# speechcatcher-asr/statecatcher

Measured on AMD Instinct MI355X. Metric: audio-frames/sec (LucyRNN+CTC, 80-d fbank, T=1500), whole job, higher is better.
Workload: dtype bf16

## Files before the change

include/statecatcher.h:

```cpp
#ifndef STATECATCHER_H
#define STATECATCHER_H

#include <stddef.h>
#include <stdint.h>

#ifdef __cplusplus
extern "C" {
#endif

#define SC_EINVAL (-1)

#define SC_F32 0
#define SC_BF16 1
#define SC_F16 2

int sc_abi_version(void);

const char* sc_last_error(void);


int sc_lucy_scan_chunk(void);

int64_t sc_lucy_scan_ckpt_numel(int B, int T, int D);

int sc_lucy_scan_fwd(const void* gates, int gates_dtype, const float* gate_bias,
                     const float* h0, const float* s0,
                     void* out, float* s_out, float* h_out, int B, int T, int D,
                     int64_t stride_g_bt, int64_t stride_g_td, int64_t stride_g_cd,
                     int64_t stride_g_cb, int64_t stride_o_bt, int64_t stride_o_bd, float* ckpt,
                     void* stream);

int sc_lucy_scan_fwd_split(const void* gates, int gates_dtype, const float* gate_bias,
                           const float* h0, const float* s0, void* out, void* out_dup, void* out_lo,
                           float* s_out, float* h_out, int B, int T, int D,
                           int64_t stride_g_bt, int64_t stride_g_td, int64_t stride_g_cd,
                           int64_t stride_g_cb, int64_t stride_o_bt, int64_t stride_o_bd,
                           float* ckpt, void* stream);

int sc_lucy_scan_fwd_ln(const void* gates, int gates_dtype, const float* gate_bias,
                        const float* h0, const float* s0, void* out, void* out_dup, void* out_lo,
                        float* s_out, float* h_out, int B, int T, int D,
                        int64_t stride_g_bt, int64_t stride_g_td, int64_t stride_g_cd,
                        int64_t stride_g_cb, int64_t stride_o_bt, int64_t stride_o_bd,
                        float* ckpt, const float* ln_r, const float* ln_rec_in, float* ln_stat,
                        float* ln_rec_out, float ln_eps, void* stream);

int sc_lucy_scan_bwd(const void* gates, int gates_dtype, const float* gate_bias, const float* ckpt,
                     const void* dout, const float* ds_last,
                     void* dgates, float* dh0, float* ds0, float* dbias, int B, int T, int D,
                     int64_t stride_g_bt, int64_t stride_g_td, int64_t stride_g_cd,
                     int64_t stride_g_cb, int64_t stride_d_bt, int64_t stride_d_bd,
                     int64_t stride_dg_bt, int64_t stride_dg_td, int64_t stride_dg_cd,
                     int64_t stride_dg_cb, void* stream);

int sc_lucy_scan_bwd_ln(const void* gates, int gates_dtype, const float* gate_bias,
                        const float* ckpt, const void* dout, const float* ds_last, void* dgates,
                        float* dh0, float* ds0, float* dbias, int B, int T, int D,
                        int64_t stride_g_bt, int64_t stride_g_td, int64_t stride_g_cd,
                        int64_t stride_g_cb, int64_t stride_d_bt, int64_t stride_d_bd,
                        int64_t stride_dg_bt, int64_t stride_dg_td, int64_t stride_dg_cd,
                        int64_t stride_dg_cb, const float* ln_r, const float* ln_stat,
                        void* stream);


int sc_decay_scan_fwd(const void* kv, const void* decay, void* out, int dtype,
                      const float* init, int B, int T, int D,
                      int64_t stride_b, int64_t stride_t, int64_t stride_d, void* stream);

int sc_decay_scan_bwd(const void* decay, const void* s_all, const void* dout, void* dkv,
                      void* ddecay, int dtype, const float* init, float* dinit,
                      int B, int T, int D, int64_t stride_b, int64_t stride_t, int64_t stride_d,
                      void* stream);


int sc_layernorm_supported(int dtype, int D);
int sc_layernorm_fwd(const void* x, int dtype, const float* gamma, const float* beta, void* y,
                     float* mean, float* rstd, int64_t rows, int D, float eps, void* stream);

int64_t sc_layernorm_bwd_workspace_numel(int64_t rows, int D);

int sc_layernorm_bwd(const void* x, const void* dy, int dtype, const float* gamma,
                     const float* mean, const float* rstd, void* dx, float* dgamma_dbeta,
                     float* workspace, int64_t rows, int D, void* stream);

typedef struct {
  const float* w;
  const float* gamma;
  const float* beta;
  const float* bias;
  float* shift;
  float* bias_out;
  float* rowsum;
  int64_t ld, rows, D;
} sc_ln_fold_job;
int sc_ln_fold_prep(const sc_ln_fold_job* jobs, int njobs, void* stream);

int sc_ln_fold_bwd(const void* g, const void* h, int dtype, const float* stat, void* dh,
                   int64_t rows, int D, void* stream);

int64_t sc_ln_fold_wgrad_workspace_numel(int rows, int D);

int sc_ln_fold_wgrad(const float* M, const float* w, int64_t ld, const float* gamma,
                     const float* beta, const float* dbias, int rows, int D, float* dw,
                     float* dgamma_dbeta, float* workspace, void* stream);


size_t sc_ctc_workspace_bytes(int B, int T, int max_target_len);

int sc_ctc_fwd(const void* x, int x_dtype, int is_logits, int B, int T, int V,
               int64_t stride_b, int64_t stride_t,
               const int64_t* targets, int64_t target_stride, int max_target_len,
               const int64_t* in_lens, const int64_t* tgt_lens, int blank,
               float* nll, void* workspace, size_t workspace_bytes, void* stream);

int sc_ctc_bwd(const void* x, int x_dtype, int is_logits, int B, int T, int V,
               int64_t stride_b, int64_t stride_t,
               const int64_t* targets, int64_t target_stride, int max_target_len,
               const int64_t* in_lens, const int64_t* tgt_lens, int blank,
               const float* nll, const float* scale, void* grad, int grad_dtype,
               const void* workspace, size_t workspace_bytes, void* stream);

int sc_ctc_fwd_ex(const void* x, int x_dtype, int is_logits, int B, int T, int V,
                  int64_t stride_b, int64_t stride_t,
                  const int64_t* targets, int64_t target_stride, int max_target_len,
                  const int64_t* in_lens, const int64_t* tgt_lens, int blank,
                  const float* ex, int64_t ex_stride_b, int64_t ex_stride_t,
                  float* nll, void* workspace, size_t workspace_bytes, void* stream);
int sc_ctc_bwd_ex(const void* x, int x_dtype, int is_logits, int B, int T, int V,
                  int64_t stride_b, int64_t stride_t,
                  const int64_t* targets, int64_t target_stride, int max_target_len,
                  const int64_t* in_lens, const int64_t* tgt_lens, int blank,
                  const float* ex, int64_t ex_stride_b, int64_t ex_stride_t,
                  const float* nll, const float* scale, void* grad, int grad_dtype,
                  const void* workspace, size_t workspace_bytes, void* stream);

int sc_ctc_split_rows(const float* w, int64_t ldw, const float* bias, int V, int K,
                      const int64_t* targets, int64_t target_stride, int max_target_len,
                      int blank, void* out, float* bias_out, int B, void* stream);

int sc_ctc_mean(const float* nll, const int64_t* tgt_lens, int B, float* loss, float* factor,
                void* stream);


int sc_ctc_greedy_decode(const void* log_probs, int dtype, int B, int T, int V,
                         int64_t stride_b, int64_t stride_t, const int64_t* lengths, int blank,
                         int32_t* tokens, int32_t* counts, void* stream);

int sc_ctc_greedy_step(const void* logits, int dtype, int B, int V, int64_t stride_b,
                       const float* mask, int blank, int32_t* prev, int32_t* emit,
                       int64_t emit_stride, void* stream);
int sc_ctc_greedy_frames(const void* logits, int dtype, int F, int B, int V, int64_t stride_f,
                         int64_t stride_b, const float* mask, int64_t mask_f, int blank,
                         int32_t* prev, int32_t* emit, int64_t emit_f, int64_t emit_b,
                         void* stream);


int sc_lucy_step_supported(int dtype, int D);

int sc_lucy_step_ln(const void* x, int dtype, const float* w, const float* b, float eps, void* y,
                    int B, int D, void* stream);

int sc_lucy_step_cell(int mode, const void* g, int dtype, int64_t g_stride, const void* u,
                      const void* hp, const float* lnz_w, const float* lnz_b, const float* lnh_w,
                      const float* lnh_b, float eps, float* h, float* s, void* out,
                      const float* mask, int B, int D, void* stream);

int sc_lucy_frame_gemm(int epi, const float* x, int64_t ldx, int K, const float* ln_w,
                       const float* ln_b, const void* st_in, int nst_in, float eps, const void* w,
                       int w_dtype, int64_t ldw, const float* bias, int B, int N, float* y,
                       int64_t ldy, void* st_out, float* z, void* st_z, float* s,
                       const float* mask, void* stream);
int sc_lucy_frame_cellb(const float* z, const void* st_z, int nst_z, const float* hp,
                        const void* st_h, int nst_h, const float* lnz_w, const float* lnz_b,
                        const float* lnh_w, const float* lnh_b, float eps, float* h, float* out,
                        int64_t ldo, const float* mask, int B, int D, void* stream);

typedef struct sc_frame_gemm_job {
  const float* x;
  int64_t ldx;
  int K;
  const float* ln_w;
  const float* ln_b;
  const void* st_in;
  int nst_in;
  const void* w;
  int64_t ldw;
  const float* bias;
  int B, N;
  float* y;
  int64_t ldy;
  void* st_out;
  float* z;
  void* st_z;
  float* s;
  const float* mask;
} sc_frame_gemm_job;
int sc_lucy_frame_gemm_multi(int epi, int w_dtype, float eps, const sc_frame_gemm_job* jobs,
                             int njobs, void* stream);
typedef struct sc_frame_cell_job {
  const float* z;
  const void* st_z;
  int nst_z;
  const float* hp;
  const void* st_h;
  int nst_h;
  const float *lnz_w, *lnz_b, *lnh_w, *lnh_b;
  float* h;
  float* out;
  int64_t ldo;
  const float* mask;
  int B, D;
} sc_frame_cell_job;
int sc_lucy_frame_cellb_multi(float eps, const sc_frame_cell_job* jobs, int njobs, void* stream);


size_t sc_colsum_workspace_bytes(int64_t M, int64_t N);
int sc_colsum(const void* x, int dtype, int64_t M, int64_t N, int64_t ld, int64_t perm_a,
              int64_t perm_b, float* out, void* workspace, size_t workspace_bytes, void* stream);


int sc_gemm_wgrad_splits(int L, int I, int J);
int sc_gemm_wgrad_bf16(const void* A, int64_t lda, const void* B, int64_t ldb, float* part, int L,
                       int I, int J, int S, void* stream);

int sc_gemm_tn_bf16(const void* A, int64_t lda, const void* B, int64_t ldb, void* C, int64_t ldc,
                    int M, int N, int K, int tile_m, void* stream);

int sc_gemm_tn_ln_bf16(const void* H, int64_t ldh, const void* Wpp, int64_t ldw, void* C,
                       int64_t ldc, int M, int N, int K, const float* r, void* stat, float eps,
                       void* stream);


typedef struct {
  float* p;
  const float* g;
  float* m;
  float* v;
  int64_t n;
} sc_adam_tensor;
int64_t sc_adam_parts(const sc_adam_tensor* t, int nt);
int sc_adam_sumsq(const sc_adam_tensor* t, int nt, float* part, void* stream);
int sc_adam_step(const sc_adam_tensor* t, int nt, const float* part, int64_t nparts,
                 double max_norm, double lr, double beta1, double beta2, double eps,
                 double weight_decay, int decoupled, double step_size, double bc2_sqrt,
                 float* norm_out, void* stream);

typedef struct {
  const float* src;
  void* dst;
  void* dst_t;
  int64_t rows, cols, cols_pad, ld_src, block_d;
  const float* col_scale;
  const float* row_shift;
} sc_image_job;
int sc_weight_images(const sc_image_job* jobs, int njobs, void* stream);


int sc_xlstm_part_rows(int64_t rows);
int sc_rmsnorm_fwd(const void* x, const float* w, void* y, float* rstd, int64_t rows, int D,
                   float eps, void* stream);
int sc_rmsnorm_bwd(const void* x, const void* dy, const float* w, const float* rstd, void* dx,
                   float* part, int64_t rows, int D, void* stream);
int sc_rmsnorm_add_fwd(const void* x, const void* r, void* s, const float* w, void* y, float* rstd,
                       int64_t rows, int D, float eps, void* stream);
int sc_rmsnorm_add_bwd(const void* s, const void* dy, const void* dres, const float* w,
                       const float* rstd, void* dx, float* part, int64_t rows, int D, void* stream);
int sc_mhln_gate_fwd(const void* h, const void* o, int64_t ldo, const float* w, void* out,
                     float* mean, float* rstd, int B, int T, int NH, int DH, float eps,
                     void* stream);
int sc_mhln_gate_bwd(const void* h, const void* o, int64_t ldo, const float* w, const float* mean,
                     const float* rstd, const void* dy, int64_t ldy, void* dh, void* dgo,
                     int64_t lddo, float* part, int B, int T, int NH, int DH, void* stream);
int sc_mhln_gate_fwd_h16(const void* h, const void* o, int64_t ldo, const float* w, void* out,
                         float* mean, float* rstd, int B, int T, int NH, int DH, float eps,
                         void* stream);
int sc_mhln_gate_bwd_h16(const void* h, const void* o, int64_t ldo, const float* w,
                         const float* mean, const float* rstd, const void* dy, int64_t ldy,
                         void* dh, void* dgo, int64_t lddo, float* part, int B, int T, int NH,
                         int DH, void* stream);
int sc_swiglu_fwd(const void* a, void* y, int64_t rows, int F, void* stream);
int sc_swiglu_bwd(const void* a, const void* dy, void* da, int64_t rows, int F, void* stream);


int64_t sc_fbank_frames(int64_t n_samples);
size_t sc_fbank_workspace_bytes(void);

int sc_fbank(const float* audio, int B, int64_t n_samples, int64_t audio_stride, int kind,
             float sample_rate, float* out, void* workspace, size_t workspace_bytes, void* stream);


int sc_mlstm_supported(int dtype, int DQ, int DV);

int64_t sc_mlstm_chunk_state_numel(int BH, int T, int DQ, int DV);

int sc_mlstm_fwd(const void* q, const void* k, const void* v, int dtype, const float* igate,
                 const float* fgate, const float* c0, const float* n0, const float* m0, int BH,
                 int T, int DQ, int DV, float eps, void* h, void* states_C, float* states_n,
                 float* states_m, float* c_last, float* m_rows, float* den_rows,
                 const int64_t* layout, void* stream);

int sc_mlstm_bwd(const void* q, const void* k, const void* v, int dtype, const float* igate,
                 const float* fgate, const void* h, const void* dh, const float* dcT,
                 const float* dnT, const void* states_C, const float* states_n,
                 const float* states_m, const float* m_rows, const float* den_rows, int BH, int T,
                 int DQ, int DV, float eps, float* dstates_C, float* dstates_n, void* dq,
                 void* dk, void* dv, float* qdq, float* kdk, const int64_t* layout,
                 void* stream);

int sc_mlstm_fwd_io(const void* q, const void* k, const void* v, int dtype, int io_dtype,
                    const float* igate, const float* fgate, const float* c0, const float* n0,
                    const float* m0, int BH, int T, int DQ, int DV, float eps, void* h,
                    void* states_C, float* states_n, float* states_m, float* c_last,
                    float* m_rows, float* den_rows, const int64_t* layout, void* stream);
int sc_mlstm_bwd_io(const void* q, const void* k, const void* v, int dtype, int io_dtype,
                    const float* igate, const float* fgate, const void* h, const void* dh,
                    const float* dcT, const float* dnT, const void* states_C,
                    const float* states_n, const float* states_m, const float* m_rows,
                    const float* den_rows, int BH, int T, int DQ, int DV, float eps,
                    float* dstates_C, float* dstates_n, void* dq, void* dk, void* dv,
                    float* qdq, float* kdk, const int64_t* layout, void* stream);

int sc_mlstm_gate_bwd(const float* qdq, const float* kdk, const float* fgate, int BH, int T,
                      float* dfgate, const void* a, void* da, int NH, int64_t ld, int io, int fo,
                      float cap, void* stream);


size_t sc_rnnt_workspace_bytes(int B, int T, int max_labels);

int sc_rnnt_fwd(const void* x, int x_dtype, int is_logits, int B, int T, int max_labels, int V,
                int64_t stride_b, int64_t stride_t, int64_t stride_u, const int64_t* row_offsets,
                const int64_t* labels, int64_t label_stride, const int64_t* frames_lengths,
                const int64_t* labels_lengths, int blank, float* nll, void* workspace,
                size_t workspace_bytes, void* stream);

int sc_rnnt_bwd(const void* x, int x_dtype, int is_logits, int B, int T, int max_labels, int V,
                int64_t stride_b, int64_t stride_t, int64_t stride_u, const int64_t* row_offsets,
                const int64_t* labels, int64_t label_stride, const int64_t* frames_lengths,
                const int64_t* labels_lengths, int blank, const float* scale, void* grad,
                int grad_dtype, const void* workspace, size_t workspace_bytes, void* stream);

int sc_rnnt_joint_geometry(int B, int T, int max_labels, int V, int* t_blocks, int* u_splits,
                           int* slices);
int sc_rnnt_joint_fwd(const float* enc, const float* pred, const void* W, const float* bias, int B,
                      int T, int max_labels, int V, int J, const int64_t* labels,
                      int64_t label_stride, const int64_t* frames_lengths,
                      const int64_t* labels_lengths, int blank, float* nll, void* workspace,
                      size_t workspace_bytes, void* stream);
int sc_rnnt_joint_bwd(const float* enc, const float* pred, const void* W, const float* bias, int B,
                      int T, int max_labels, int V, int J, const int64_t* labels,
                      int64_t label_stride, const int64_t* frames_lengths,
                      const int64_t* labels_lengths, int blank, const float* scale, float* d_enc,
                      float* d_pred, float* dW, float* db, const void* workspace,
                      size_t workspace_bytes, void* stream);

int sc_rnnt_greedy_decode(const void* enc_p, const void* pred_tab, const void* W, int dtype,
                          const float* bias, int B, int T, int V, int J, int64_t stride_b,
                          int64_t stride_t, const int64_t* lengths, const float* mask,
                          int64_t mask_b, int64_t mask_t, int blank, int max_symbols,
                          int32_t* prev, int32_t* tokens, int32_t* frames, int cap,
                          int32_t* counts, void* stream);

#ifdef __cplusplus
}
#endif
#endif
```

statecatcher_amd/_lib.py:

```python
import ctypes
import os

import torch

LIB_NAME = "libstatecatcher_hip.so"
LIB_PATH = os.environ.get("SC_LIB_PATH") or os.path.join(os.path.dirname(os.path.abspath(__file__)),
                                                         LIB_NAME)

SC_F32, SC_BF16, SC_F16 = 0, 1, 2
_DTYPE = {torch.float32: SC_F32, torch.bfloat16: SC_BF16, torch.float16: SC_F16}

_c = ctypes
_i32, _i64, _vp, _fp = _c.c_int, _c.c_int64, _c.c_void_p, _c.c_void_p
ABI_VERSION = 14

_SIGS = {
    "sc_abi_version": (_i32, []),
    "sc_gemm_wgrad_splits": (_i32, [_i32, _i32, _i32]),
    "sc_gemm_wgrad_bf16": (_i32, [_vp, _i64, _vp, _i64, _fp, _i32, _i32, _i32, _i32, _vp]),
    "sc_gemm_tn_bf16": (_i32, [_vp, _i64, _vp, _i64, _vp, _i64, _i32, _i32, _i32, _i32, _vp]),
    "sc_gemm_tn_ln_bf16": (_i32, [_vp, _i64, _vp, _i64, _vp, _i64, _i32, _i32, _i32, _fp, _vp,
                                 _c.c_float, _vp]),
    "sc_last_error": (_c.c_char_p, []),
    "sc_lucy_scan_chunk": (_i32, []),
    "sc_lucy_scan_ckpt_numel": (_i64, [_i32, _i32, _i32]),
    "sc_lucy_scan_fwd": (_i32, [_vp, _i32, _fp, _fp, _fp, _vp, _fp, _fp, _i32, _i32, _i32,
                               _i64, _i64, _i64, _i64, _i64, _i64, _fp, _vp]),
    "sc_lucy_scan_fwd_split": (_i32, [_vp, _i32, _fp, _fp, _fp, _vp, _vp, _vp, _fp, _fp, _i32, _i32,
                                     _i32, _i64, _i64, _i64, _i64, _i64, _i64, _fp, _vp]),
    "sc_lucy_scan_bwd": (_i32, [_vp, _i32, _fp, _fp, _vp, _fp, _vp, _fp, _fp, _fp, _i32, _i32, _i32,
                               _i64, _i64, _i64, _i64, _i64, _i64, _i64, _i64, _i64, _i64,
                               _vp]),
    "sc_lucy_scan_fwd_ln": (_i32, [_vp, _i32, _fp, _fp, _fp, _vp, _vp, _vp, _fp, _fp, _i32, _i32,
                                  _i32, _i64, _i64, _i64, _i64, _i64, _i64, _fp, _fp, _fp, _fp, _fp,
                                  _c.c_float, _vp]),
    "sc_lucy_scan_bwd_ln": (_i32, [_vp, _i32, _fp, _fp, _vp, _fp, _vp, _fp, _fp, _fp, _i32, _i32,
                                  _i32, _i64, _i64, _i64, _i64, _i64, _i64, _i64, _i64, _i64, _i64,
                                  _fp, _fp, _vp]),
    "sc_ln_fold_prep": (_i32, [_vp, _i32, _vp]),
    "sc_ln_fold_bwd": (_i32, [_vp, _vp, _i32, _fp, _vp, _i64, _i32, _vp]),
    "sc_ln_fold_wgrad_workspace_numel": (_i64, [_i32, _i32]),
    "sc_ln_fold_wgrad": (_i32, [_fp, _fp, _i64, _fp, _fp, _fp, _i32, _i32, _fp, _fp, _fp, _vp]),
    "sc_decay_scan_fwd": (_i32, [_vp, _vp, _vp, _i32, _fp, _i32, _i32, _i32, _i64, _i64, _i64, _vp]),
    "sc_decay_scan_bwd": (_i32, [_vp, _vp, _vp, _vp, _vp, _i32, _fp, _fp, _i32, _i32, _i32,
                                _i64, _i64, _i64, _vp]),
    "sc_layernorm_supported": (_i32, [_i32, _i32]),
    "sc_layernorm_fwd": (_i32, [_vp, _i32, _fp, _fp, _vp, _fp, _fp, _i64, _i32, _c.c_float, _vp]),
    "sc_layernorm_bwd_workspace_numel": (_i64, [_i64, _i32]),
    "sc_layernorm_bwd": (_i32, [_vp, _vp, _i32, _fp, _fp, _fp, _vp, _fp, _fp, _i64, _i32, _vp]),
    "sc_ctc_workspace_bytes": (_c.c_size_t, [_i32, _i32, _i32]),
    "sc_ctc_fwd": (_i32, [_vp, _i32, _i32, _i32, _i32, _i32, _i64, _i64, _vp, _i64, _i32, _vp, _vp,
                         _i32, _fp, _vp, _c.c_size_t, _vp]),
    "sc_ctc_bwd": (_i32, [_vp, _i32, _i32, _i32, _i32, _i32, _i64, _i64, _vp, _i64, _i32, _vp, _vp,
                         _i32, _fp, _fp, _vp, _i32, _vp, _c.c_size_t, _vp]),
    "sc_ctc_fwd_ex": (_i32, [_vp, _i32, _i32, _i32, _i32, _i32, _i64, _i64, _vp, _i64, _i32, _vp,
                            _vp, _i32, _fp, _i64, _i64, _fp, _vp, _c.c_size_t, _vp]),
    "sc_ctc_bwd_ex": (_i32, [_vp, _i32, _i32, _i32, _i32, _i32, _i64, _i64, _vp, _i64, _i32, _vp,
                            _vp, _i32, _fp, _i64, _i64, _fp, _fp, _vp, _i32, _vp, _c.c_size_t,
                            _vp]),
    "sc_ctc_split_rows": (_i32, [_fp, _i64, _fp, _i32, _i32, _vp, _i64, _i32, _i32, _vp, _fp,
                                 _i32, _vp]),
    "sc_ctc_greedy_decode": (_i32, [_vp, _i32, _i32, _i32, _i32, _i64, _i64, _vp, _i32, _vp, _vp, _vp]),
    "sc_colsum_workspace_bytes": (_c.c_size_t, [_i64, _i64]),
    "sc_colsum": (_i32, [_vp, _i32, _i64, _i64, _i64, _i64, _i64, _fp, _vp, _c.c_size_t, _vp]),
    "sc_fbank_frames": (_i64, [_i64]),
    "sc_fbank_workspace_bytes": (_c.c_size_t, []),
    "sc_fbank": (_i32, [_vp, _i32, _i64, _i64, _i32, _c.c_float, _fp, _vp, _c.c_size_t, _vp]),
    "sc_ctc_mean": (_i32, [_fp, _vp, _i32, _fp, _fp, _vp]),
    "sc_ctc_greedy_step": (_i32, [_vp, _i32, _i32, _i32, _i64, _fp, _i32, _vp, _vp, _i64, _vp]),
    "sc_lucy_step_supported": (_i32, [_i32, _i32]),
    "sc_lucy_step_ln": (_i32, [_vp, _i32, _fp, _fp, _c.c_float, _vp, _i32, _i32, _vp]),
    "sc_lucy_step_cell": (_i32, [_i32, _vp, _i32, _i64, _vp, _vp, _fp, _fp, _fp, _fp, _c.c_float,
                                 _fp, _fp, _vp, _fp, _i32, _i32, _vp]),
    "sc_lucy_frame_gemm": (_i32, [_i32, _fp, _i64, _i32, _fp, _fp, _vp, _i32, _c.c_float, _vp, _i32,
                                  _i64, _fp, _i32, _i32, _fp, _i64, _vp, _fp, _vp, _fp, _fp, _vp]),
    "sc_lucy_frame_cellb": (_i32, [_fp, _vp, _i32, _fp, _vp, _i32, _fp, _fp, _fp, _fp, _c.c_float,
                                   _fp, _fp, _i64, _fp, _i32, _i32, _vp]),
    "sc_lucy_frame_gemm_multi": (_i32, [_i32, _i32, _c.c_float, _vp, _i32, _vp]),
    "sc_lucy_frame_cellb_multi": (_i32, [_c.c_float, _vp, _i32, _vp]),
    "sc_ctc_greedy_frames": (_i32, [_vp, _i32, _i32, _i32, _i32, _i64, _i64, _fp, _i64, _i32, _vp,
                                    _vp, _i64, _i64, _vp]),
    "sc_mlstm_supported": (_i32, [_i32, _i32, _i32]),
    "sc_mlstm_chunk_state_numel": (_i64, [_i32, _i32, _i32, _i32]),
    "sc_mlstm_fwd": (_i32, [_vp, _vp, _vp, _i32, _fp, _fp, _fp, _fp, _fp, _i32, _i32, _i32, _i32,
                           _c.c_float, _vp, _vp, _fp, _fp, _fp, _fp, _fp, _vp, _vp]),
    "sc_mlstm_bwd": (_i32, [_vp, _vp, _vp, _i32, _fp, _fp, _vp, _vp, _fp, _fp, _vp, _fp, _fp, _fp,
                           _fp, _i32, _i32, _i32, _i32, _c.c_float, _fp, _fp, _vp, _vp, _vp, _fp,
                           _fp, _vp, _vp]),
    "sc_mlstm_fwd_io": (_i32, [_vp, _vp, _vp, _i32, _i32, _fp, _fp, _fp, _fp, _fp, _i32, _i32, _i32,
                              _i32, _c.c_float, _vp, _vp, _fp, _fp, _fp, _fp, _fp, _vp, _vp]),
    "sc_mlstm_bwd_io": (_i32, [_vp, _vp, _vp, _i32, _i32, _fp, _fp, _vp, _vp, _fp, _fp, _vp, _fp, _fp,
                              _fp, _fp, _i32, _i32, _i32, _i32, _c.c_float, _fp, _fp, _vp, _vp, _vp,
                              _fp, _fp, _vp, _vp]),
    "sc_mlstm_gate_bwd": (_i32, [_fp, _fp, _fp, _i32, _i32, _fp, _vp, _vp, _i32, _i64, _i32, _i32,
                                _c.c_float, _vp]),
    "sc_xlstm_part_rows": (_i32, [_i64]),
    "sc_rmsnorm_fwd": (_i32, [_vp, _fp, _vp, _fp, _i64, _i32, _c.c_float, _vp]),
    "sc_rmsnorm_bwd": (_i32, [_vp, _vp, _fp, _fp, _vp, _fp, _i64, _i32, _vp]),
    "sc_rmsnorm_add_fwd": (_i32, [_vp, _vp, _vp, _fp, _vp, _fp, _i64, _i32, _c.c_float, _vp]),
    "sc_rmsnorm_add_bwd": (_i32, [_vp, _vp, _vp, _fp, _fp, _vp, _fp, _i64, _i32, _vp]),
    "sc_mhln_gate_fwd": (_i32, [_vp, _vp, _i64, _fp, _vp, _fp, _fp, _i32, _i32, _i32, _i32,
                                _c.c_float, _vp]),
    "sc_mhln_gate_bwd": (_i32, [_vp, _vp, _i64, _fp, _fp, _fp, _vp, _i64, _vp, _vp, _i64, _fp,
                                _i32, _i32, _i32, _i32, _vp]),
    "sc_mhln_gate_fwd_h16": (_i32, [_vp, _vp, _i64, _fp, _vp, _fp, _fp, _i32, _i32, _i32, _i32,
                                _c.c_float, _vp]),
    "sc_mhln_gate_bwd_h16": (_i32, [_vp, _vp, _i64, _fp, _fp, _fp, _vp, _i64, _vp, _vp, _i64, _fp,
                                _i32, _i32, _i32, _i32, _vp]),
    "sc_swiglu_fwd": (_i32, [_vp, _vp, _i64, _i32, _vp]),
    "sc_swiglu_bwd": (_i32, [_vp, _vp, _vp, _i64, _i32, _vp]),
    "sc_adam_parts": (_i64, [_vp, _i32]),
    "sc_adam_sumsq": (_i32, [_vp, _i32, _fp, _vp]),
    "sc_adam_step": (_i32, [_vp, _i32, _fp, _i64, _c.c_double, _c.c_double, _c.c_double,
                           _c.c_double, _c.c_double, _c.c_double, _i32, _c.c_double, _c.c_double,
                           _fp, _vp]),
    "sc_weight_images": (_i32, [_vp, _i32, _vp]),
    "sc_rnnt_workspace_bytes": (_c.c_size_t, [_i32, _i32, _i32]),
    "sc_rnnt_joint_geometry": (_i32, [_i32, _i32, _i32, _i32, _vp, _vp, _vp]),
    "sc_rnnt_joint_fwd": (_i32, [_fp, _fp, _vp, _fp, _i32, _i32, _i32, _i32, _i32, _vp, _i64, _vp,
                                 _vp, _i32, _fp, _vp, _c.c_size_t, _vp]),
    "sc_rnnt_joint_bwd": (_i32, [_fp, _fp, _vp, _fp, _i32, _i32, _i32, _i32, _i32, _vp, _i64, _vp,
                                 _vp, _i32, _fp, _fp, _fp, _fp, _fp, _vp, _c.c_size_t, _vp]),
    "sc_rnnt_fwd": (_i32, [_vp, _i32, _i32, _i32, _i32, _i32, _i32, _i64, _i64, _i64, _vp, _vp, _i64,
                          _vp, _vp, _i32, _fp, _vp, _c.c_size_t, _vp]),
    "sc_rnnt_bwd": (_i32, [_vp, _i32, _i32, _i32, _i32, _i32, _i32, _i64, _i64, _i64, _vp, _vp, _i64,
                          _vp, _vp, _i32, _fp, _vp, _i32, _vp, _c.c_size_t, _vp]),
    "sc_rnnt_greedy_decode": (_i32, [_vp, _vp, _vp, _i32, _fp, _i32, _i32, _i32, _i32, _i64, _i64,
                                     _vp, _fp, _i64, _i64, _i32, _i32, _vp, _vp, _vp, _i32, _vp,
                                     _vp]),
}
EXPORTED = tuple(_SIGS)


class AdamTensor(ctypes.Structure):
    _fields_ = [("p", _vp), ("g", _vp), ("m", _vp), ("v", _vp), ("n", _i64)]


class ImageJob(ctypes.Structure):
    _fields_ = [("src", _vp), ("dst", _vp), ("dst_t", _vp), ("rows", _i64), ("cols", _i64),
                ("cols_pad", _i64), ("ld_src", _i64), ("block_d", _i64), ("col_scale", _vp),
                ("row_shift", _vp)]


class LnFoldJob(ctypes.Structure):
    _fields_ = [("w", _vp), ("gamma", _vp), ("beta", _vp), ("bias", _vp), ("shift", _vp),
                ("bias_out", _vp), ("rowsum", _vp), ("ld", _i64), ("rows", _i64), ("D", _i64)]


class FrameGemmJob(ctypes.Structure):
    _fields_ = [("x", _vp), ("ldx", _i64), ("K", _i32), ("ln_w", _vp), ("ln_b", _vp),
                ("st_in", _vp), ("nst_in", _i32), ("w", _vp), ("ldw", _i64), ("bias", _vp),
                ("B", _i32), ("N", _i32), ("y", _vp), ("ldy", _i64), ("st_out", _vp), ("z", _vp),
                ("st_z", _vp), ("s", _vp), ("mask", _vp)]


class FrameCellJob(ctypes.Structure):
    _fields_ = [("z", _vp), ("st_z", _vp), ("nst_z", _i32), ("hp", _vp), ("st_h", _vp),
                ("nst_h", _i32), ("lnz_w", _vp), ("lnz_b", _vp), ("lnh_w", _vp), ("lnh_b", _vp),
                ("h", _vp), ("out", _vp), ("ldo", _i64), ("mask", _vp), ("B", _i32), ("D", _i32)]


_LIB = None


def load():
    global _LIB
    if _LIB is None:
        if not os.path.exists(LIB_PATH):
            raise RuntimeError(
                f"statecatcher HIP library not built: {LIB_PATH} missing "
                "(run `python -c 'import __graft_entry__ as g; g.build()'` or "
                "`make -C statecatcher_amd/csrc`)")
        lib = ctypes.CDLL(LIB_PATH)
        for name, (res, args) in _SIGS.items():
            fn = getattr(lib, name)
            fn.restype = res
            fn.argtypes = args
        if lib.sc_abi_version() != ABI_VERSION:
            raise RuntimeError("statecatcher ABI version mismatch")
        _LIB = lib
    return _LIB


def check(rc, what):
    if rc != 0:
        msg = load().sc_last_error().decode(errors="replace")
        if rc < 0:
            raise ValueError(f"{what}: {msg}")
        raise RuntimeError(f"{what}: HIP error {rc}: {msg}")


def dtype_code(t):
    try:
        return _DTYPE[t.dtype]
    except KeyError:
        raise TypeError(f"unsupported dtype {t.dtype}; expected float32, bfloat16 or float16") from None


def require_device(*tensors):
    for t in tensors:
        if t is not None and t.device.type != "cuda":
            raise RuntimeError(
                "statecatcher ops run only on a ROCm GPU (HIP); got a tensor on "
                f"{t.device}. There is no CPU fallback.")


def stream_of(t):
    return ctypes.c_void_p(torch.cuda.current_stream(t.device).cuda_stream)


def ptr(t):
    return ctypes.c_void_p(t.data_ptr()) if t is not None else None
```

statecatcher_amd/csrc/ctc.hip:

```cpp
#include "sc_common.h"

#ifndef SC_CTC_ABL
#define SC_CTC_ABL 0
#endif
#ifndef SC_CTC_KMAX
#define SC_CTC_KMAX 16
#endif
#ifndef SC_CTC_FLAGX
#define SC_CTC_FLAGX 0
#endif
#ifndef SC_CTC_WMV
#define SC_CTC_WMV 0
#endif
#ifndef SC_CTC_FLAG_SLEEP
#define SC_CTC_FLAG_SLEEP 1
#endif

namespace sc {

constexpr float kNegInf = -__builtin_huge_valf();

struct CtcWs {
  float* lse;
  double* lse64;
  float* lpe;
  float* alpha;
  float* beta;
  double* offA;
  double* offB;
  float* cst;
  double* ll2s;
  int* chain;
  int* first;
  float* ylin;
  int* flag;
  int* sharp;
};

static size_t align256(size_t x) { return (x + 255) & ~(size_t)255; }

static int states_per_lane(int S) { return (S + 63) / 64; }

static int lin_ppl(int Umax);

static size_t ws_layout(int B, int T, int Umax, CtcWs* w, void* base) {
  const int S = 2 * Umax + 1;
  const int Sp = 64 * states_per_lane(S);
  const bool lin = lin_ppl(Umax) > 0;
  const size_t ab = 4;
  const int Um = Umax > 0 ? Umax : 1;
  char* p = (char*)base;
  size_t off = 0;
  auto take = [&](size_t bytes) {
    char* r = p + off;
    off += align256(bytes);
    return (void*)r;
  };
  CtcWs t;
  t.lse = (float*)take((size_t)B * T * 4);
  t.lse64 = (double*)take((size_t)B * T * 8);
  t.lpe = (float*)take((size_t)B * T * Sp * 4);
  t.alpha = (float*)take((size_t)B * T * Sp * ab);
  t.beta = (float*)take((size_t)B * T * Sp * ab);
  t.offA = (double*)take((size_t)B * (T + 1) * 8);
  t.offB = (double*)take((size_t)B * (T + 1) * 8);
  t.cst = (float*)take((size_t)B * T * 4);
  t.ll2s = (double*)take((size_t)B * 8);
  t.chain = (int*)take((size_t)B * Um * 4);
  t.first = (int*)take((size_t)B * Um * 4);
  t.ylin = lin ? (float*)take((size_t)B * T * Sp * 4) : nullptr;
  t.flag = lin ? (int*)take((size_t)B * 4) : nullptr;
  t.sharp = (int*)take((size_t)B * 4);
  if (w) *w = t;
  return off;
}

__device__ __forceinline__ float lse2_b2(float a, float b) {
  const float m = fmaxf(a, b);
  if (m == kNegInf) return kNegInf;
  return m + log2_(exp2_(a - m) + exp2_(b - m));
}


struct CtcArgs {
  const void* x;
  int is_logits, B, T, V, S, Sp, Umax, blank;
  int kh;
  int lin;
  int64_t sb, stt;
  const int64_t* tg;
  int64_t tgs;
  const int64_t* in_lens;
  const int64_t* tgt_lens;
  float* nll;
  CtcWs ws;
  const float* scale;
  void* grad;
  const float* ex;
  int64_t exb, ext;
};

__device__ __forceinline__ int clampi(int64_t v, int lo, int hi) {
  return (int)(v < lo ? lo : (v > hi ? hi : v));
}

__device__ __forceinline__ int state_label(const int64_t* tg, int s, int blank, int V) {
  int lab = (s & 1) ? (int)tg[(s - 1) >> 1] : blank;
  return lab < 0 ? 0 : (lab >= V ? V - 1 : lab);
}

constexpr float kTiny = 120.0f;

template <int DT>
__global__ void __launch_bounds__(256) ctc_emit_kernel(CtcArgs a) {
  using E = Elem<DT>;
  using T = typename E::T;
  const int lane = threadIdx.x & 63;
  const int64_t row = (int64_t)blockIdx.x * 4 + (threadIdx.x >> 6);
  if (row >= (int64_t)a.B * a.T) return;
  const int b = (int)(row / a.T), t = (int)(row % a.T);
  if (t >= clampi(a.in_lens[b], 0, a.T)) return;
  const T* p = (const T*)a.x + (int64_t)b * a.sb + (int64_t)t * a.stt;
  const int Sb = 2 * clampi(a.tgt_lens[b], 0, a.Umax) + 1;
  const int64_t* tg = a.tg + (int64_t)b * a.tgs;
  const float* exr = a.ex ? a.ex + (int64_t)b * a.exb + (int64_t)t * a.ext : nullptr;
  constexpr int kGx = 8;
  auto state_logit = [&](int s) {
    return exr ? exr[(s & 1) ? (s + 1) >> 1 : 0] : E::ld(p[state_label(tg, s, a.blank, a.V)]);
  };
  const bool inreg = a.Sp <= 64 * kGx;
  float xs[kGx];
  if (inreg) {
    if (exr) {
#pragma unroll
      for (int j = 0; j < kGx; ++j) {
        const int s = min(lane + 64 * j, Sb - 1);
        xs[j] = exr[(s & 1) ? (s + 1) >> 1 : 0];
      }
    } else {
      int lab[kGx];
#pragma unroll
      for (int j = 0; j < kGx; ++j) lab[j] = state_label(tg, min(lane + 64 * j, Sb - 1), a.blank, a.V);
#pragma unroll
      for (int j = 0; j < kGx; ++j) xs[j] = E::ld(p[lab[j]]);
    }
  }
  float lse = 0.0f;
  if (a.is_logits) {
    float m = kNegInf, l = 0.0f;
    constexpr int N = Vec16<DT>::N;
    if ((a.V % N) == 0 && ((uintptr_t)p & 15) == 0) {
      for (int c = lane; c < a.V / N; c += 64) {
        float xv[N];
        Vec16<DT>::ld(p + N * c, xv);
        float cm = xv[0];
#pragma unroll
        for (int k = 1; k < N; ++k) cm = fmaxf(cm, xv[k]);
        const float mn = fmaxf(m, cm);
        float cs = 0.0f;
#pragma unroll
        for (int k = 0; k < N; ++k) cs += fexp(xv[k] - mn);
        l = l * fexp(m - mn) + cs;
        m = mn;
      }
    } else {
      for (int v = lane; v < a.V; v += 64) {
        const float xv = E::ld(p[v]);
        const float mn = fmaxf(m, xv);
        l = l * fexp(m - mn) + fexp(xv - mn);
        m = mn;
      }
    }
    const float M = wave_max_dpp(m);
    l = wave_sum_dpp(m == kNegInf ? 0.0f : l * fexp(m - M));
    lse = M + flog(l);
    if (lane == 0) {
      a.ws.lse[row] = lse;
      a.ws.lse64[row] = (double)M + (double)flog(l);
    }
  }
  float* out = a.ws.lpe + row * a.Sp;
  auto lp2x = [&](float xl) { return fmaxf((xl - lse) * kLog2e, -1e30f); };
  auto lp2 = [&](int s) { return lp2x(state_logit(s)); };
  float c = -1e30f;
  if (inreg) {
#pragma unroll
    for (int j = 0; j < kGx; ++j)
      if (lane + 64 * j < Sb) c = fmaxf(c, lp2x(xs[j]));
  } else {
    for (int s = lane; s < Sb; s += 64) c = fmaxf(c, lp2(s));
  }
  c = wave_max_dpp(c);
  if (!(c > -1e29f)) c = 0.0f;
  bool tiny = false;
  auto put = [&](int s, float e) {
    out[s] = e;
    if (a.lin) {
      tiny |= e > -1e29f && e < -kTiny;
      a.ws.ylin[row * a.Sp + s] = e > -1e29f ? exp2_(e) : 0.0f;
    }
  };
  if (inreg) {
#pragma unroll
    for (int j = 0; j < kGx; ++j) {
      const int s = lane + 64 * j;
      if (s < a.Sp) put(s, s < Sb ? fmaxf(lp2x(xs[j]) - c, -1e30f) : -1e30f);
    }
  } else {
    for (int s = lane; s < a.Sp; s += 64) put(s, s < Sb ? fmaxf(lp2(s) - c, -1e30f) : -1e30f);
  }
  if (lane == 0) a.ws.cst[row] = c;
  if (a.lin && __ballot(tiny) && lane == 0) a.ws.flag[b] = 1;
}

__global__ void __launch_bounds__(256) ctc_chain_kernel(CtcArgs a) {
  __shared__ int lt[1024];
  const int b = blockIdx.x;
  const int lane = threadIdx.x & 63;
  const int Ub = clampi(a.tgt_lens[b], 0, a.Umax);
  const int64_t* tg = a.tg + (int64_t)b * a.tgs;
  const int Um = a.Umax > 0 ? a.Umax : 1;
  for (int u = threadIdx.x; u < Ub; u += blockDim.x) lt[u] = (int)tg[u];
  __syncthreads();
  if (blockIdx.y == 0 && threadIdx.x == 0) a.ws.sharp[b] = 0;
  const int u = blockIdx.y * 4 + (threadIdx.x >> 6);
  if (u >= Um) return;
  int nxt = -1, first = 0;
  if (u < Ub) {
    const int lab = lt[u];
    for (int q0 = u + 1; q0 < Ub; q0 += 64) {
      const int q = q0 + lane;
      const unsigned long long hit = __ballot(q < Ub && lt[q] == lab);
      if (hit) {
        nxt = q0 + __ffsll(hit) - 1;
        break;
      }
    }
    first = 1;
    for (int q0 = 0; q0 < u; q0 += 64) {
      const int q = q0 + lane;
      if (__ballot(q < u && lt[q] == lab)) {
        first = 0;
        break;
      }
    }
  }
  if (lane == 0) {
    a.ws.chain[(int64_t)b * Um + u] = nxt;
    a.ws.first[(int64_t)b * Um + u] = first;
  }
}

__device__ __forceinline__ float shr1(float v) {
  return __int_as_float(__builtin_amdgcn_update_dpp(__float_as_int(-1e30f), __float_as_int(v),
                                                     0x138, 0xf, 0xf, false));
}
__device__ __forceinline__ float shl1(float v) {
  return __int_as_float(__builtin_amdgcn_update_dpp(__float_as_int(-1e30f), __float_as_int(v),
                                                     0x130, 0xf, 0xf, false));
}

constexpr float kDead = -1e30f;
constexpr float kDrift = 512.0f;
__device__ __forceinline__ float lse3_live(float a, float b, float c) {
  const float m = fmaxf(fmaxf(a, b), c);
  if (SC_CTC_ABL & 4) return m;
  const float md = __builtin_amdgcn_fmed3f(a, b, c);
  const float lo = fminf(fminf(a, b), c);
  return m + log2_(1.0f + exp2_(md - m) + exp2_(lo - m));
}

constexpr int kAbP = 16;

#ifndef SC_CTC_V2
#define SC_CTC_V2 1
#endif
__device__ __forceinline__ float vmin(float a, float b) {
  float r;
  asm("v_min_f32 %0, %1, %2" : "=v"(r) : "v"(a), "v"(b));
  return r;
}
__device__ __forceinline__ float vmax3(float a, float b, float c) {
  float r;
  asm("v_max3_f32 %0, %1, %2, %3" : "=v"(r) : "v"(a), "v"(b), "v"(c));
  return r;
}
__device__ __forceinline__ float vmin3(float a, float b, float c) {
  float r;
  asm("v_min3_f32 %0, %1, %2, %3" : "=v"(r) : "v"(a), "v"(b), "v"(c));
  return r;
}
__device__ __forceinline__ float shr1z(float v) {
  return __int_as_float(__builtin_amdgcn_mov_dpp(__float_as_int(v), 0x138, 0xf, 0xf, true));
}
__device__ __forceinline__ float shl1z(float v) {
  return __int_as_float(__builtin_amdgcn_mov_dpp(__float_as_int(v), 0x130, 0xf, 0xf, true));
}
typedef float f2v __attribute__((ext_vector_type(2)));
__device__ __forceinline__ f2v lse23(float a2, float b2, float a3, float b3, float c3, f2v e) {
  const float m2 = vmax(a2, b2), l2 = vmin(a2, b2);
  const float m3 = vmax3(a3, b3, c3), d3 = __builtin_amdgcn_fmed3f(a3, b3, c3);
  const float l3 = vmin3(a3, b3, c3);
  const f2v me = f2v{m2, m3} + e;
  const f2v s = f2v{1.0f, 1.0f} + f2v{exp2_(l2 - m2), exp2_(d3 - m3)};
  return me + f2v{log2_(s.x), log2_(s.y + exp2_(l3 - m3))};
}


__device__ __forceinline__ float lse2_live(float a, float b) {
  const float m = fmaxf(a, b);
  if (SC_CTC_ABL & 4) return m;
  return m + log2_(1.0f + exp2_(fminf(a, b) - m));
}

template <int K, bool BETA>
__device__ __forceinline__ void ab_run(const CtcArgs& a, int b, int Tb, int Ub) {
  constexpr int OW = 64 - K;
  constexpr int kAbP = K > 16 ? K : 16;
  const int tid = threadIdx.x;
  const int lane = tid & 63;
  const int w = uniform(tid >> 6);
  const int nw = blockDim.x >> 6;
  const int p = BETA ? w * OW + lane : w * OW + lane - K;
  const bool own = BETA ? (lane < OW) : (lane >= K);
  const bool liveB = p >= 0 && p <= Ub;
  const bool liveL = p >= 0 && p < Ub;
  const int64_t* tg = a.tg + (int64_t)b * a.tgs;
  bool skip = false;
  if (liveL) {
    const int lab = (int)tg[p];
    if (!BETA) {
      skip = p >= 1 && lab != a.blank && lab != (int)tg[p - 1];
    } else if (p + 1 < Ub) {
      const int l2 = (int)tg[p + 1];
      skip = l2 != a.blank && l2 != lab;
    }
  }
  extern __shared__ __attribute__((aligned(16))) float2 full2[];
  __shared__ __attribute__((aligned(16))) float wmax[16];
  __shared__ int xflag[16];
  if (SC_CTC_FLAGX) {
    if (tid < 16) xflag[tid] = 0;
    lds_barrier();
  }
  const int nst = nw * OW;
  const int pc = p < 0 ? 0 : (2 * p >= a.Sp ? a.Sp / 2 - 1 : p);
  const float2* lrow = (const float2*)(a.ws.lpe + (int64_t)b * a.T * a.Sp) + pc;
  const int64_t rs = a.Sp / 2;
  constexpr uint32_t kDrop = 0x80000000u;
  const uint32_t rowb = (uint32_t)(a.Sp * 4);
  const __amdgpu_buffer_rsrc_t ors = __builtin_amdgcn_make_buffer_rsrc(
      (BETA ? a.ws.beta : a.ws.alpha) + (int64_t)b * a.T * a.Sp, 0, (int)(rowb * (uint32_t)a.T),
      0x00020000);
  const uint32_t ovo = (own && 2 * p < a.Sp) ? (uint32_t)(8 * pc) : kDrop;
  double* offn = (BETA ? a.ws.offB : a.ws.offA) + (int64_t)b * (a.T + 1);
  if (tid == 0) offn[0] = 0.0;
  auto tstep = [&](int i) { return BETA ? Tb - 1 - i : i; };
  float2 bufA[kAbP], bufB[kAbP];
#if SC_CTC_V2
  const __amdgpu_buffer_rsrc_t ers = __builtin_amdgcn_make_buffer_rsrc(
      a.ws.lpe + (int64_t)b * a.T * a.Sp, 0, (int)(rowb * (uint32_t)a.T), 0x00020000);
  const uint32_t evo = (p >= 0 && 2 * p < a.Sp) ? (uint32_t)(8 * p) : kDrop;
  auto load = [&](float2 (&buf)[kAbP], int i0) {
#pragma unroll
    for (int j = 0; j < kAbP; ++j)
      buf[j] = __builtin_bit_cast(float2, __builtin_amdgcn_raw_buffer_load_b64(
                                              ers, evo, (uint32_t)tstep(min(i0 + j, Tb - 1)) * rowb, 0));
  };
#else
  auto load = [&](float2 (&buf)[kAbP], int i0) {
#pragma unroll
    for (int j = 0; j < kAbP; ++j) buf[j] = lrow[(int64_t)tstep(min(i0 + j, Tb - 1)) * rs];
  };
#endif
  auto emit = [&](int t, float vB, float vL) {
    __builtin_amdgcn_raw_buffer_store_b64(
        __builtin_bit_cast(__attribute__((ext_vector_type(2))) unsigned, make_float2(vB, vL)), ors,
        ovo, (uint32_t)t * rowb, 0);
  };
  float vB = kDead, vL = kDead;
  double off = 0.0;
  int exch = 0;
  auto body = [&](const float2 (&buf)[kAbP], int i0) __attribute__((always_inline)) {
#pragma unroll
    for (int j = 0; j < kAbP; ++j) {
      const int i = i0 + j;
      if (i >= Tb) break;
#if SC_CTC_V2
      if (i == 0) {
        vB = (liveB && p == (BETA ? Ub : 0)) ? buf[j].x : kDead;
        vL = (liveL && p == (BETA ? Ub - 1 : 0)) ? buf[j].y : kDead;
      } else if (!BETA) {
        const float lp = shr1z(vL);
        const f2v r = lse23(vB, lp, vL, vB, skip ? lp : kDead, f2v{buf[j].x, buf[j].y});
        vB = r.x;
        vL = r.y;
      } else {
        const float bn = shl1z(vB);
        const float ln = shl1z(vL);
        const f2v r = lse23(vB, vL, vL, bn, skip ? ln : kDead, f2v{buf[j].x, buf[j].y});
        vB = r.x;
        vL = r.y;
      }
#else
      const float eB = liveB ? buf[j].x : kDead;
      const float eL = liveL ? buf[j].y : kDead;
      if (i == 0) {
        vB = (liveB && p == (BETA ? Ub : 0)) ? eB : kDead;
        vL = (liveL && p == (BETA ? Ub - 1 : 0)) ? eL : kDead;
      } else if (!BETA) {
        const float lp = shr1(vL);
        const float nB = lse2_live(vB, lp) + eB;
        vL = lse3_live(vL, vB, skip ? lp : kDead) + eL;
        vB = nB;
      } else {
        const float bn = shl1(vB);
        const float ln = shl1(vL);
        const float nB = lse2_live(vB, vL) + eB;
        vL = lse3_live(vL, bn, skip ? ln : kDead) + eL;
        vB = nB;
      }
#endif
      if (!(SC_CTC_ABL & 1) && j % K == K - 1) {
        const int par = exch & 1;
        const bool norm = par == 1;
        if (own) full2[par * nst + p] = make_float2(vB, vL);
        if (SC_CTC_FLAGX && !norm) {
          lds_read_wait();
          if (lane == 0)
            __hip_atomic_store(&xflag[w], exch + 1, __ATOMIC_RELEASE, __HIP_MEMORY_SCOPE_WORKGROUP);
          const int nb = BETA ? w + 1 : w - 1;
          if (nb >= 0 && nb < nw) {
            while (__hip_atomic_load(&xflag[nb], __ATOMIC_ACQUIRE, __HIP_MEMORY_SCOPE_WORKGROUP) <= exch)
              if (SC_CTC_FLAG_SLEEP) __builtin_amdgcn_s_sleep(1);
          }
          if (!own) {
            const bool has = p >= 0 && p < nst;
            const float2 q = has ? full2[par * nst + p] : make_float2(kDead, kDead);
            vB = q.x;
            vL = q.y;
          }
          ++exch;
          if (!(SC_CTC_ABL & 2)) emit(tstep(i), vB, vL);
          continue;
        }
        if (norm) {
          float m = own ? fmaxf(vB, vL) : kDead;
#if SC_CTC_V2
          m = wave_max_dpp(m);
#else
#pragma unroll
          for (int o = 32; o > 0; o >>= 1) m = fmaxf(m, __shfl_xor(m, o));
#endif
          if (lane == 0) wmax[w] = m;
        }
        lds_barrier();
        if (!own) {
          const bool has = p >= 0 && p < nst;
          const float2 q = has ? full2[par * nst + p] : make_float2(kDead, kDead);
          vB = q.x;
          vL = q.y;
        }
        if (norm) {
          float m = kDead;
#if SC_CTC_WMV
#pragma unroll
          for (int q4 = 0; q4 < 16; q4 += 4) {
            if (q4 < nw) {
              const float4 wm = *(const float4*)&wmax[q4];
              m = fmaxf(m, q4 + 0 < nw ? wm.x : kDead);
              m = fmaxf(m, q4 + 1 < nw ? wm.y : kDead);
              m = fmaxf(m, q4 + 2 < nw ? wm.z : kDead);
              m = fmaxf(m, q4 + 3 < nw ? wm.w : kDead);
            }
          }
#else
          for (int q = 0; q < nw; ++q) m = fmaxf(m, wmax[q]);
#endif
          if (m > 0.5f * kDead) {
            vB -= m;
            vL -= m;
            off += (double)m;
// ... 94 lines not shown
  const int64_t* tg = a.tg + (int64_t)b * a.tgs;
  const int npairs = a.Sp / 2;
  double skip[PPL];
  uint32_t vo[PPL];
  constexpr uint32_t kDrop = 0x80000000u;
#pragma unroll
  for (int j = 0; j < PPL; ++j) {
    const int p = lane * PPL + j;
    bool sk = false;
    if (p < Ub) {
      const int lab = (int)tg[p];
      if (!BETA) {
        sk = p >= 1 && lab != a.blank && lab != (int)tg[p - 1];
      } else if (p + 1 < Ub) {
        const int l2 = (int)tg[p + 1];
        sk = l2 != a.blank && l2 != lab;
      }
    }
    skip[j] = sk ? 1.0 : 0.0;
    vo[j] = p < npairs ? (uint32_t)(8 * p) : kDrop;
  }
  const uint32_t rowb = (uint32_t)(a.Sp * 4);
  const __amdgpu_buffer_rsrc_t ers = __builtin_amdgcn_make_buffer_rsrc(
      a.ws.ylin + (int64_t)b * a.T * a.Sp, 0, (int)(rowb * (uint32_t)a.T), 0x00020000);
  double* offn = (BETA ? a.ws.offB : a.ws.offA) + (int64_t)b * (a.T + 1);
  if (lane == 0) offn[0] = 0.0;
  auto tstep = [&](int i) { return BETA ? Tb - 1 - i : i; };
  f2v bufA[kLinC][PPL], bufB[kLinC][PPL];
  auto load = [&](f2v (&buf)[kLinC][PPL], int i0) {
#pragma unroll
    for (int s = 0; s < kLinC; ++s) {
      const uint32_t so = (uint32_t)tstep(min(i0 + s, Tb - 1)) * rowb;
#pragma unroll
      for (int j = 0; j < PPL; ++j)
        buf[s][j] = (SC_CTC_ABL & 16) ? f2v{0.5f, 0.25f}
                                      : __builtin_bit_cast(f2v, __builtin_amdgcn_raw_buffer_load_b64(ers, vo[j], so, 0));
    }
  };
  double vB[PPL], vL[PPL];
#pragma unroll
  for (int j = 0; j < PPL; ++j) vB[j] = vL[j] = 0.0;
  double off = 0.0;
  bool fail = false;
  auto body = [&](const f2v (&buf)[kLinC][PPL], int ci) __attribute__((always_inline)) {
    d2v* slot = slots + (size_t)(ci & 1) * kLinC * PPL * 64;
#pragma unroll
    for (int s = 0; s < kLinC; ++s) {
      const int i = ci * kLinC + s;
      if (i >= Tb) break;
      if (i == 0) {
#pragma unroll
        for (int j = 0; j < PPL; ++j) {
          const int p = lane * PPL + j;
          vB[j] = (p <= Ub && p == (BETA ? Ub : 0)) ? (double)buf[s][j].x : 0.0;
          vL[j] = (p < Ub && p == (BETA ? Ub - 1 : 0)) ? (double)buf[s][j].y : 0.0;
        }
      } else if (!BETA) {
        double prevL[PPL];
        prevL[0] = dpp_shr1d(vL[PPL - 1]);
#pragma unroll
        for (int j = 1; j < PPL; ++j) prevL[j] = vL[j - 1];
#pragma unroll
        for (int j = 0; j < PPL; ++j) {
          const double nb = (vB[j] + prevL[j]) * (double)buf[s][j].x;
          const double nl = __builtin_fma(skip[j], prevL[j], vL[j] + vB[j]) * (double)buf[s][j].y;
          vB[j] = nb;
          vL[j] = nl;
        }
      } else {
        double nB[PPL], nL[PPL];
        nB[PPL - 1] = dpp_shl1d(vB[0]);
        nL[PPL - 1] = dpp_shl1d(vL[0]);
#pragma unroll
        for (int j = 0; j + 1 < PPL; ++j) {
          nB[j] = vB[j + 1];
          nL[j] = vL[j + 1];
        }
#pragma unroll
        for (int j = 0; j < PPL; ++j) {
          const double nb = (vB[j] + vL[j]) * (double)buf[s][j].x;
          const double nl = __builtin_fma(skip[j], nL[j], vL[j] + nB[j]) * (double)buf[s][j].y;
          vB[j] = nb;
          vL[j] = nl;
        }
      }
      if (!(SC_CTC_ABL & 8) && (i + 1) % kAb1R == 0) {
        double m = 0.0;
#pragma unroll
        for (int j = 0; j < PPL; ++j) m = fmax(m, fmax(vB[j], vL[j]));
        int e = 0;
        (void)frexp(m, &e);
        const float E = wave_max_dpp(m > 0.0 ? (float)e : -1e9f);
        if (E < -1e8f) {
          fail = true;
          return;
        }
        const int ie = (int)E;
#pragma unroll
        for (int j = 0; j < PPL; ++j) {
          vB[j] = ldexp(vB[j], -ie);
          vL[j] = ldexp(vL[j], -ie);
        }
        off += (double)ie;
        if (lane == 0) offn[(i + 1) / kAb1R] = off;
      }
#pragma unroll
      for (int j = 0; j < PPL; ++j) slot[(s * PPL + j) * 64 + lane] = d2v{vB[j], vL[j]};
    }
  };
  const int nch = (Tb + kLinC - 1) / kLinC;
  load(bufA, 0);
  for (int ci = 0; ci < nch; ++ci) {
    if (!fail) {
      if ((ci & 1) == 0) {
        if (ci + 1 < nch) load(bufB, (ci + 1) * kLinC);
        body(bufA, ci);
      } else {
        if (ci + 1 < nch) load(bufA, (ci + 1) * kLinC);
        body(bufB, ci);
      }
    }
    if (lane == 0) *fail_lds = fail ? 1 : 0;
    __syncthreads();
  }
  if (fail) return false;
  if (!BETA) {
    double c = 0.0;
#pragma unroll
    for (int j = 0; j < PPL; ++j) {
      const int p = lane * PPL + j;
      if (p == Ub) c += vB[j];
      if (p == Ub - 1) c += vL[j];
    }
    double cs = 0.0;
    for (int t = lane; t < Tb; t += 64) cs += (double)a.ws.cst[(int64_t)b * a.T + t];
#pragma unroll
    for (int o = 32; o > 0; o >>= 1) {
      c += __shfl_xor(c, o);
      cs += __shfl_xor(cs, o);
    }
    if (!(c > 0.0)) return false;
    if (lane == 0) {
      const double ll2s = log2(c) + off;
      a.ws.ll2s[b] = ll2s;
      a.nll[b] = (float)(-(ll2s + cs) * 0.6931471805599453);
    }
  }
  return true;
}

template <int PPL, bool BETA>
__device__ __forceinline__ void lin_consume(const CtcArgs& a, int b, int Tb, const d2v* slots,
                                            const int* fail_lds) {
  const int lane = threadIdx.x & 63, half = (threadIdx.x >> 6) - 1;
  const int npairs = a.Sp / 2;
  constexpr uint32_t kDrop = 0x80000000u;
  uint32_t vo[PPL];
#pragma unroll
  for (int j = 0; j < PPL; ++j) {
    const int p = lane * PPL + j;
    vo[j] = p < npairs ? (uint32_t)(8 * p) : kDrop;
  }
  const uint32_t rowb = (uint32_t)(a.Sp * 4);
  const __amdgpu_buffer_rsrc_t ors = __builtin_amdgcn_make_buffer_rsrc(
      (BETA ? a.ws.beta : a.ws.alpha) + (int64_t)b * a.T * a.Sp, 0, (int)(rowb * (uint32_t)a.T),
      0x00020000);
  const int nch = (Tb + kLinC - 1) / kLinC;
  bool stop = false;
  auto consume = [&](int ci) {
    const d2v* slot = slots + (size_t)(ci & 1) * kLinC * PPL * 64;
#pragma unroll
    for (int s2 = 0; s2 < kLinC / 2; ++s2) {
      const int s = half * (kLinC / 2) + s2, i = ci * kLinC + s;
      if (i >= Tb) break;
      const uint32_t so = (uint32_t)(BETA ? Tb - 1 - i : i) * rowb;
#pragma unroll
      for (int j = 0; j < PPL; ++j) {
        const d2v v = slot[(s * PPL + j) * 64 + lane];
        if (!(SC_CTC_ABL & 2))
          __builtin_amdgcn_raw_buffer_store_b64(
              __builtin_bit_cast(__attribute__((ext_vector_type(2))) unsigned, f2v{log2d(v.x), log2d(v.y)}),
              ors, vo[j], so, 0);
      }
    }
  };
  for (int ci = 0; ci < nch; ++ci) {
    __syncthreads();
    if (!stop) stop = *fail_lds != 0;
    if (!stop) consume(ci);
  }
}

template <int PPL>
__global__ void __launch_bounds__(192) ctc_lin_kernel(CtcArgs a) {
  __shared__ d2v slots[2 * kLinC * PPL * 64];
  __shared__ int fail_lds;
  const bool is_beta = blockIdx.x >= a.B;
  const int b = is_beta ? blockIdx.x - a.B : blockIdx.x;
  const int Tb = clampi(a.in_lens[b], 0, a.T);
  const int Ub = clampi(a.tgt_lens[b], 0, a.Umax);
  const int w = uniform(threadIdx.x >> 6);
  if (Tb == 0) {
    if (!is_beta && threadIdx.x == 0) {
      a.nll[b] = (Ub == 0) ? 0.0f : __builtin_huge_valf();
      a.ws.ll2s[b] = (Ub == 0) ? 0.0 : -__builtin_huge_val();
    }
    return;
  }
  const bool tiny = a.ws.flag[b] != 0;
  bool lin = !tiny;
  if (lin) {
    if (w == 0) {
      lin = is_beta ? lin_produce<PPL, true>(a, b, Tb, Ub, slots, &fail_lds)
                    : lin_produce<PPL, false>(a, b, Tb, Ub, slots, &fail_lds);
    } else {
      if (is_beta) lin_consume<PPL, true>(a, b, Tb, slots, &fail_lds);
      else lin_consume<PPL, false>(a, b, Tb, slots, &fail_lds);
      __builtin_amdgcn_s_waitcnt(0);
    }
    __syncthreads();
  }
  if (!lin && threadIdx.x == 0) a.ws.sharp[b] = 1;
}


constexpr int kXDeadE = -(1 << 29);
constexpr int kX64P = 16;
constexpr double kLog2eD = 1.4426950408889634;

struct Xv {
  double m;
  int e;
};
__device__ __forceinline__ Xv xnorm(double m, int e) {
  int x;
  const double mm = frexp(m, &x);
  return m > 0.0 ? Xv{mm, e + x} : Xv{0.0, kXDeadE};
}
__device__ __forceinline__ Xv xadd2(Xv a, Xv b) {
  const int E = max(a.e, b.e);
  return Xv{ldexp(a.m, a.e - E) + ldexp(b.m, b.e - E), E};
}
__device__ __forceinline__ Xv xadd3(Xv a, Xv b, Xv c) {
  const int E = max(max(a.e, b.e), c.e);
  return Xv{ldexp(a.m, a.e - E) + ldexp(b.m, b.e - E) + ldexp(c.m, c.e - E), E};
}
template <bool RIGHT>
__device__ __forceinline__ Xv xdpp(Xv v) {
  constexpr int ctl = RIGHT ? 0x138 : 0x130;
  const int lo = __builtin_amdgcn_update_dpp(0, __double2loint(v.m), ctl, 0xf, 0xf, false);
  const int hi = __builtin_amdgcn_update_dpp(0, __double2hiint(v.m), ctl, 0xf, 0xf, false);
  const int e = __builtin_amdgcn_update_dpp(kXDeadE, v.e, ctl, 0xf, 0xf, false);
  return Xv{__hiloint2double(hi, lo), e};
}
__device__ __forceinline__ Xv xemit(float x, double q, bool live) {
  const double e2 = (double)x * kLog2eD - q;
  if (!live || !(e2 > -1e300)) return Xv{0.0, kXDeadE};
  const double k = floor(e2);
  return xnorm((double)exp2_((float)(e2 - k)), (int)k);
}

template <int PPL, int DT, bool BETA>
__device__ __forceinline__ void x64_run(const CtcArgs& a, int b, int Tb, int Ub) {
  using E = Elem<DT>;
  const int lane = threadIdx.x;
  const int64_t* tg = a.tg + (int64_t)b * a.tgs;
  const int npairs = a.Sp / 2;
  bool skip[PPL], liveB[PPL], liveL[PPL];
  uint32_t cB[PPL], cL[PPL];
  uint32_t vo[PPL];
  constexpr uint32_t kDrop = 0x80000000u;
  const bool ex = a.ex != nullptr;
  const uint32_t esz = ex ? 4u : (uint32_t)sizeof(typename E::T);
#pragma unroll
  for (int j = 0; j < PPL; ++j) {
    const int p = lane * PPL + j;
    skip[j] = false;
    liveB[j] = p <= Ub;
    liveL[j] = p < Ub;
    int lab = a.blank;
    if (p < Ub) {
      lab = (int)tg[p];
      if (!BETA) {
        skip[j] = p >= 1 && lab != a.blank && lab != (int)tg[p - 1];
      } else if (p + 1 < Ub) {
        const int l2 = (int)tg[p + 1];
        skip[j] = l2 != a.blank && l2 != lab;
      }
    }
    lab = lab < 0 ? 0 : (lab >= a.V ? a.V - 1 : lab);
    cB[j] = ex ? 0u : (uint32_t)a.blank * esz;
    cL[j] = ex ? (uint32_t)(p < Ub ? 1 + p : 0) * 4u : (uint32_t)lab * esz;
    vo[j] = p < npairs ? (uint32_t)(8 * p) : kDrop;
  }
  const void* xb = ex ? (const void*)(a.ex + (int64_t)b * a.exb)
                      : (const void*)((const typename E::T*)a.x + (int64_t)b * a.sb);
  const uint32_t xrow = ex ? (uint32_t)a.ext * 4u : (uint32_t)a.stt * esz;
  const Buf<float> xf(xb);
  const Buf<typename E::T> xe(xb);
  auto ldx = [&](uint32_t col, uint32_t so) -> uint32_t {
    return ex ? __float_as_uint(xf.ld(col, so)) : xe.ldw(col, so);
  };
  auto cvt = [&](uint32_t w) { return ex ? __uint_as_float(w) : E::ldw(w); };
  const uint32_t rowb = (uint32_t)(a.Sp * 4);
  const __amdgpu_buffer_rsrc_t ors = __builtin_amdgcn_make_buffer_rsrc(
      (BETA ? a.ws.beta : a.ws.alpha) + (int64_t)b * a.T * a.Sp, 0, (int)(rowb * (uint32_t)a.T),
      0x00020000);
  double* offn = (BETA ? a.ws.offB : a.ws.offA) + (int64_t)b * (a.T + 1);
  const double* lse64 = a.ws.lse64 + (int64_t)b * a.T;
  const float* cst = a.ws.cst + (int64_t)b * a.T;
  if (lane == 0) offn[0] = 0.0;
  auto tstep = [&](int i) { return BETA ? Tb - 1 - i : i; };
  uint32_t wA[kX64P][PPL][2], wB[kX64P][PPL][2];
  double qA, qB;
  auto load = [&](uint32_t (&w)[kX64P][PPL][2], double& q, int i0) {
#pragma unroll
    for (int s = 0; s < kX64P; ++s) {
      const uint32_t so = (uint32_t)tstep(min(i0 + s, Tb - 1)) * xrow;
#pragma unroll
      for (int j = 0; j < PPL; ++j) {
        w[s][j][0] = ldx(cB[j], so);
        w[s][j][1] = ldx(cL[j], so);
      }
    }
    const int t = tstep(min(i0 + (lane & (kX64P - 1)), Tb - 1));
    q = (a.is_logits ? lse64[t] * kLog2eD : 0.0) + (double)cst[t];
  };
  Xv vB[PPL], vL[PPL];
#pragma unroll
  for (int j = 0; j < PPL; ++j) vB[j] = vL[j] = Xv{0.0, kXDeadE};
  const Xv dead{0.0, kXDeadE};
  auto body = [&](const uint32_t (&w)[kX64P][PPL][2], double qv, int i0) __attribute__((always_inline)) {
#pragma unroll
    for (int s = 0; s < kX64P; ++s) {
      const int i = i0 + s;
      if (i >= Tb) break;
      const double q = __hiloint2double(__builtin_amdgcn_readlane(__double2hiint(qv), s),
                                        __builtin_amdgcn_readlane(__double2loint(qv), s));
      Xv eB[PPL], eL[PPL];
#pragma unroll
      for (int j = 0; j < PPL; ++j) {
        eB[j] = xemit(cvt(w[s][j][0]), q, liveB[j]);
        eL[j] = xemit(cvt(w[s][j][1]), q, liveL[j]);
      }
      if (i == 0) {
#pragma unroll
        for (int j = 0; j < PPL; ++j) {
          const int p = lane * PPL + j;
          vB[j] = p == (BETA ? Ub : 0) ? eB[j] : dead;
          vL[j] = p == (BETA ? Ub - 1 : 0) ? eL[j] : dead;
        }
      } else if (!BETA) {
        Xv prevL[PPL];
        prevL[0] = xdpp<true>(vL[PPL - 1]);
#pragma unroll
        for (int j = 1; j < PPL; ++j) prevL[j] = vL[j - 1];
#pragma unroll
        for (int j = 0; j < PPL; ++j) {
          const Xv nb = xadd2(vB[j], prevL[j]);
          const Xv nl = xadd3(vL[j], vB[j], skip[j] ? prevL[j] : dead);
          vB[j] = xnorm(nb.m * eB[j].m, nb.e + eB[j].e);
          vL[j] = xnorm(nl.m * eL[j].m, nl.e + eL[j].e);
        }
      } else {
        Xv nB[PPL], nL[PPL];
        nB[PPL - 1] = xdpp<false>(vB[0]);
        nL[PPL - 1] = xdpp<false>(vL[0]);
#pragma unroll
        for (int j = 0; j + 1 < PPL; ++j) {
          nB[j] = vB[j + 1];
          nL[j] = vL[j + 1];
        }
#pragma unroll
        for (int j = 0; j < PPL; ++j) {
          const Xv nb = xadd2(vB[j], vL[j]);
          const Xv nl = xadd3(vL[j], nB[j], skip[j] ? nL[j] : dead);
          vB[j] = xnorm(nb.m * eB[j].m, nb.e + eB[j].e);
          vL[j] = xnorm(nl.m * eL[j].m, nl.e + eL[j].e);
        }
      }
      int mx = kXDeadE;
#pragma unroll
      for (int j = 0; j < PPL; ++j) mx = max(mx, max(vB[j].e, vL[j].e));
      const int O = (int)wave_max_dpp((float)mx);
      const bool alive = O > kXDeadE / 2;
      if (lane == 0) offn[i + 1] = alive ? (double)O : 0.0;
      const uint32_t so = (uint32_t)tstep(i) * rowb;
#pragma unroll
      for (int j = 0; j < PPL; ++j) {
        const float rb = vB[j].m > 0.0 ? (float)(vB[j].e - O) + log2_((float)vB[j].m) : kDead;
        const float rl = vL[j].m > 0.0 ? (float)(vL[j].e - O) + log2_((float)vL[j].m) : kDead;
        __builtin_amdgcn_raw_buffer_store_b64(
            __builtin_bit_cast(__attribute__((ext_vector_type(2))) unsigned, f2v{rb, rl}), ors,
            vo[j], so, 0);
      }
    }
  };
  load(wA, qA, 0);
  for (int i0 = 0; i0 < Tb; i0 += 2 * kX64P) {
    load(wB, qB, i0 + kX64P);
    body(wA, qA, i0);
    if (i0 + kX64P >= Tb) break;
    load(wA, qA, i0 + 2 * kX64P);
    body(wB, qB, i0 + kX64P);
  }
  if (!BETA) {
    Xv c = dead;
#pragma unroll
    for (int j = 0; j < PPL; ++j) {
      const int p = lane * PPL + j;
      if (p == Ub) c = xadd2(c, vB[j]);
      if (p == Ub - 1) c = xadd2(c, vL[j]);
    }
    double cs = 0.0;
    for (int t = lane; t < Tb; t += 64) cs += (double)cst[t];
#pragma unroll
    for (int o = 32; o > 0; o >>= 1) {
      const Xv co{__shfl_xor(c.m, o), __shfl_xor(c.e, o)};
      c = xadd2(c, co);
      cs += __shfl_xor(cs, o);
    }
    if (lane == 0) {
      const bool deadP = !(c.m > 0.0);
      const double ll2s = (double)c.e + log2(c.m);
      a.ws.ll2s[b] = deadP ? -__builtin_huge_val() : ll2s;
      a.nll[b] = deadP ? __builtin_huge_valf() : (float)(-(ll2s + cs) * 0.6931471805599453);
    }
  }
}

template <int PPL, int DT>
__global__ void __launch_bounds__(64) ctc_x64_kernel(CtcArgs a) {
  const bool is_beta = blockIdx.x >= a.B;
  const int b = is_beta ? blockIdx.x - a.B : blockIdx.x;
  if (a.ws.sharp[b] == 0) return;
  const int Tb = clampi(a.in_lens[b], 0, a.T);
  const int Ub = clampi(a.tgt_lens[b], 0, a.Umax);
  if (Tb == 0) return;
  if (threadIdx.x == 0) a.ws.sharp[b] = 2;
  if (is_beta) x64_run<PPL, DT, true>(a, b, Tb, Ub);
  else x64_run<PPL, DT, false>(a, b, Tb, Ub);
}

static int x64_ppl(int Umax) {
  const int ppl = (Umax + 1 + 63) / 64;
  return ppl <= 4 ? ppl : 0;
}

static int lin_ppl(int Umax) {
  static const bool on = [] {
    const char* e = getenv("SC_CTC_LIN");
    return e && e[0] == '1';
  }();
  const int ppl = (Umax + 1 + 63) / 64;
  return (on && ppl <= 4) ? ppl : 0;
}

static int ab_halo_k(int Umax) {
  auto waves = [&](int K) { return (Umax + 1 + (64 - K) - 1) / (64 - K); };
  for (int K : {SC_CTC_KMAX, 4, 2, 1})
    if (waves(K) <= 16) {
      if (SC_CTC_KMAX == 16 && K == 16 && waves(24) == waves(16)) return 24;
      return K;
    }
  return 0;
}

__device__ __forceinline__ void wave_lds_sync() {
  __builtin_amdgcn_fence(__ATOMIC_RELEASE, "wavefront");
  __builtin_amdgcn_wave_barrier();
  __builtin_amdgcn_fence(__ATOMIC_ACQUIRE, "wavefront");
}

template <int DT, int GT>
__global__ void __launch_bounds__(256) ctc_grad_kernel(CtcArgs a) {
  using E = Elem<DT>;
  using G = Elem<GT>;
  extern __shared__ __attribute__((aligned(16))) float lcab_all[];
  const int lane = threadIdx.x & 63, w = threadIdx.x >> 6;
  const int64_t row = (int64_t)blockIdx.x * (blockDim.x >> 6) + w;
  if (row >= (int64_t)a.B * a.T) return;
  float* lcab = lcab_all + w * (a.V + 4);
  const int b = (int)(row / a.T), t = (int)(row % a.T);
  const int Tb = clampi(a.in_lens[b], 0, a.T);
  typename G::T* g = (typename G::T*)a.grad + row * a.V;
  const float sc = a.scale[b];
  const bool gvec = (a.V & 7) == 0 && ((uintptr_t)g & 15) == 0;
  if (t >= Tb || sc == 0.0f) {
    if (gvec) {
      const float z[8] = {0.f, 0.f, 0.f, 0.f, 0.f, 0.f, 0.f, 0.f};
      for (int c = lane; c < (a.V >> 3); c += 64) {
        if constexpr (Vec16<GT>::N == 8) {
          Vec16<GT>::st(g + 8 * c, z);
        } else {
          Vec16<GT>::st(g + 8 * c, *(const float(*)[4])&z[0]);
          Vec16<GT>::st(g + 8 * c + 4, *(const float(*)[4])&z[4]);
        }
      }
    } else {
      for (int v = lane; v < a.V; v += 64) g[v] = G::st(0.0f);
    }
    return;
  }
  const int Ub = clampi(a.tgt_lens[b], 0, a.Umax);
  const int Sb = 2 * Ub + 1;
  const int Um = a.Umax > 0 ? a.Umax : 1;
  const int64_t* tg = a.tg + (int64_t)b * a.tgs;
  for (int v = lane; v < a.V; v += 64) lcab[v] = kNegInf;
  wave_lds_sync();
  const float* exr = a.ex ? a.ex + (int64_t)b * a.exb + (int64_t)t * a.ext : nullptr;
  const float* al = a.ws.alpha + ((int64_t)b * a.T + t) * a.Sp;
  const float* be = a.ws.beta + ((int64_t)b * a.T + t) * a.Sp;
  const int per = a.ws.sharp[b] == 2 ? 1 : 2 * a.kh;
  const float koff = (float)(a.ws.offA[(int64_t)b * (a.T + 1) + (t + 1) / per] +
                             a.ws.offB[(int64_t)b * (a.T + 1) + (Tb - t) / per] +
                             (double)a.ws.cst[(int64_t)b * a.T + t] - a.ws.ll2s[b]);
  const int* chain = a.ws.chain + (int64_t)b * Um;
  const int* first = a.ws.first + (int64_t)b * Um;
  const float lse = a.is_logits ? a.ws.lse[(int64_t)b * a.T + t] : 0.0f;
  const float lse_lo = a.is_logits ? (float)(a.ws.lse64[(int64_t)b * a.T + t] - (double)lse) : 0.0f;
  auto exact_grad = [&](float logit, float occ2) {
    const float lp2 = ((logit - lse) - lse_lo) * kLog2e;
    return (exp2_(lp2) - exp2_(occ2 + koff - lp2)) * sc;
  };
  float m = kNegInf, l = 0.0f;
  for (int s = lane; s < Sb; s += 64) {
    const int lab = (s & 1) ? (int)tg[(s - 1) >> 1] : a.blank;
    const float val = al[s] + be[s];
    if (lab == a.blank) {
      const float mn = fmaxf(m, val);
      if (mn != kNegInf) {
        l = l * exp2_(m - mn) + exp2_(val - mn);
        m = mn;
      }
    } else {
      const int u = (s - 1) >> 1;
      if (first[u]) {
        float acc = val;
        for (int q = chain[u]; q >= 0; q = chain[q])
          acc = lse2_b2(acc, al[2 * q + 1] + be[2 * q + 1]);
        if (lab >= 0 && lab < a.V) lcab[lab] = exr ? exact_grad(exr[1 + u], acc) : acc;
      }
    }
  }
  {
    const float M = wave_max_dpp(m);
    l = wave_sum_dpp(m == kNegInf ? 0.0f : l * exp2_(m - M));
    m = M;
  }
  if (lane == 0 && a.blank >= 0 && a.blank < a.V) {
    const float ob = (m == kNegInf) ? kNegInf : m + log2_(l);
    lcab[a.blank] = exr ? exact_grad(exr[0], ob) : ob;
  }
  wave_lds_sync();
  const typename E::T* xr = (const typename E::T*)a.x + (int64_t)b * a.sb + (int64_t)t * a.stt;
  if (gvec && ((uintptr_t)xr & 15) == 0) {
    for (int c = lane; c < (a.V >> 3); c += 64) {
      float xv[8], gv[8];
      if constexpr (Vec16<DT>::N == 8) {
        Vec16<DT>::ld(xr + 8 * c, xv);
      } else {
        Vec16<DT>::ld(xr + 8 * c, *(float(*)[4])&xv[0]);
        Vec16<DT>::ld(xr + 8 * c + 4, *(float(*)[4])&xv[4]);
      }
      const float4 l0 = *(const float4*)&lcab[8 * c], l1 = *(const float4*)&lcab[8 * c + 4];
      const float lc[8] = {l0.x, l0.y, l0.z, l0.w, l1.x, l1.y, l1.z, l1.w};
#pragma unroll
      for (int k = 0; k < 8; ++k) {
        const float lp2 = ((xv[k] - lse) - lse_lo) * kLog2e;
        gv[k] = (exp2_(lp2) - exp2_(lc[k] + koff - lp2)) * sc;
        if (a.ex && lc[k] != kNegInf) gv[k] = lc[k];
      }
      if constexpr (Vec16<GT>::N == 8) {
        Vec16<GT>::st(g + 8 * c, gv);
      } else {
        Vec16<GT>::st(g + 8 * c, *(float(*)[4])&gv[0]);
        Vec16<GT>::st(g + 8 * c + 4, *(float(*)[4])&gv[4]);
      }
    }
    return;
  }
  for (int v = lane; v < a.V; v += 64) {
    const float lp2 = ((E::ld(xr[v]) - lse) - lse_lo) * kLog2e;
    const float lc = lcab[v];
    const float gv = (a.ex && lc != kNegInf) ? lc : (exp2_(lp2) - exp2_(lc + koff - lp2)) * sc;
    g[v] = G::st(gv);
  }
}

static void launch_ab(const CtcArgs& a, hipStream_t st);

template <int DT>
static void launch_fwd(const CtcArgs& a, hipStream_t st) {
  const int64_t rows = (int64_t)a.B * a.T;
  if (a.lin) zero_async(a.ws.flag, (size_t)a.B * sizeof(int), st);
  hipLaunchKernelGGL((ctc_emit_kernel<DT>), dim3((unsigned)((rows + 3) / 4)), dim3(256), 0, st, a);
  hipLaunchKernelGGL(ctc_chain_kernel, dim3(a.B, ((a.Umax > 0 ? a.Umax : 1) + 3) / 4), dim3(256), 0,
                     st, a);
  switch (a.lin ? lin_ppl(a.Umax) : 0) {
    case 1: hipLaunchKernelGGL((ctc_lin_kernel<1>), dim3(2 * a.B), dim3(192), 0, st, a); break;
    case 2: hipLaunchKernelGGL((ctc_lin_kernel<2>), dim3(2 * a.B), dim3(192), 0, st, a); break;
    case 3: hipLaunchKernelGGL((ctc_lin_kernel<3>), dim3(2 * a.B), dim3(192), 0, st, a); break;
    case 4: hipLaunchKernelGGL((ctc_lin_kernel<4>), dim3(2 * a.B), dim3(192), 0, st, a); break;
    default: launch_ab(a, st); break;
  }
  switch (x64_ppl(a.Umax)) {
    case 1: hipLaunchKernelGGL((ctc_x64_kernel<1, DT>), dim3(2 * a.B), dim3(64), 0, st, a); break;
    case 2: hipLaunchKernelGGL((ctc_x64_kernel<2, DT>), dim3(2 * a.B), dim3(64), 0, st, a); break;
    case 3: hipLaunchKernelGGL((ctc_x64_kernel<3, DT>), dim3(2 * a.B), dim3(64), 0, st, a); break;
    case 4: hipLaunchKernelGGL((ctc_x64_kernel<4, DT>), dim3(2 * a.B), dim3(64), 0, st, a); break;
    default: break;
  }
}

static void launch_ab(const CtcArgs& a, hipStream_t st) {
  const int K = a.kh;
  const int nw = (a.Umax + 1 + (64 - K) - 1) / (64 - K);
  const size_t sh = 2 * (size_t)nw * (64 - K) * sizeof(float2);
  switch (K) {
#if SC_CTC_KMAX == 16
    case 24: hipLaunchKernelGGL((ctc_ab_kernel<24>), dim3(2 * a.B), dim3(64 * nw), sh, st, a); break;
    case 16: hipLaunchKernelGGL((ctc_ab_kernel<16>), dim3(2 * a.B), dim3(64 * nw), sh, st, a); break;
#endif
    case 8: hipLaunchKernelGGL((ctc_ab_kernel<8>), dim3(2 * a.B), dim3(64 * nw), sh, st, a); break;
    case 4: hipLaunchKernelGGL((ctc_ab_kernel<4>), dim3(2 * a.B), dim3(64 * nw), sh, st, a); break;
    case 2: hipLaunchKernelGGL((ctc_ab_kernel<2>), dim3(2 * a.B), dim3(64 * nw), sh, st, a); break;
    default: hipLaunchKernelGGL((ctc_ab_kernel<1>), dim3(2 * a.B), dim3(64 * nw), sh, st, a); break;
  }
}

template <int DT, int GT>
static void launch_bwd(const CtcArgs& a, hipStream_t st) {
  const int R = 4 * (a.V + 4) * (int)sizeof(float) <= 65536 ? 4 : 1;
  hipLaunchKernelGGL((ctc_grad_kernel<DT, GT>), dim3((unsigned)(((int64_t)a.B * a.T + R - 1) / R)),
                     dim3(64 * R), R * (a.V + 4) * sizeof(float), st, a);
}

__global__ void __launch_bounds__(256) ctc_mean_kernel(const float* nll, const int64_t* tgt_lens,
                                                       int B, float* loss, float* factor) {
  __shared__ float part[256];
  float acc = 0.0f;
  for (int b = threadIdx.x; b < B; b += 256) {
    const float u = (float)(tgt_lens[b] > 1 ? tgt_lens[b] : 1);
    const float v = nll[b];
    const bool fin = !__builtin_isinf(v);
    acc += fin ? v / u : 0.0f;
    factor[b] = fin ? 1.0f / ((float)B * u) : 0.0f;
  }
  part[threadIdx.x] = acc;
  __syncthreads();
  for (int o = 128; o > 0; o >>= 1) {
    if ((int)threadIdx.x < o) part[threadIdx.x] += part[threadIdx.x + o];
    __syncthreads();
  }
  if (threadIdx.x == 0) *loss = part[0] / (float)B;
}

__global__ void __launch_bounds__(256) ctc_split_rows_kernel(const float* w, int64_t ldw,
                                                             const float* bias, int V, int K,
                                                             const int64_t* tg, int64_t tgs, int U1,
                                                             int blank, __bf16* out, float* bout,
                                                             int B) {
  const int lane = threadIdx.x & 63;
  const int64_t row = (int64_t)blockIdx.x * 4 + (threadIdx.x >> 6);
  if (row >= (int64_t)B * U1) return;
  const int b = (int)(row / U1), c = (int)(row % U1);
  int r = c == 0 ? blank : (int)tg[(int64_t)b * tgs + c - 1];
  r = r < 0 ? 0 : (r >= V ? V - 1 : r);
  const float* wr = w + (int64_t)r * ldw;
  __bf16* o = out + row * 3 * (int64_t)K;
  typedef __bf16 bf4 __attribute__((ext_vector_type(4)));
  for (int k = 4 * lane; k < K; k += 256) {
    const float4 v = *(const float4*)(wr + k);
    const bf4 hi = {(__bf16)v.x, (__bf16)v.y, (__bf16)v.z, (__bf16)v.w};
    const bf4 lo = {(__bf16)(v.x - (float)hi[0]), (__bf16)(v.y - (float)hi[1]),
                    (__bf16)(v.z - (float)hi[2]), (__bf16)(v.w - (float)hi[3])};
    *(bf4*)(o + k) = hi;
    *(bf4*)(o + K + k) = lo;
    *(bf4*)(o + 2 * K + k) = hi;
  }
  if (lane == 0) bout[row] = bias ? bias[r] : 0.0f;
}

}

using namespace sc;

extern "C" int sc_ctc_split_rows(const float* w, int64_t ldw, const float* bias, int V, int K,
                                 const int64_t* targets, int64_t target_stride, int max_target_len,
                                 int blank, void* out, float* bias_out, int B, void* stream) {
  clear_error();
  SC_REQUIRE(B >= 0 && V > 0 && K > 0 && max_target_len >= 0, "sc_ctc_split_rows: bad shape");
  if (B == 0) return 0;
  SC_REQUIRE(w && out && bias_out && (max_target_len == 0 || targets),
             "sc_ctc_split_rows: null pointer");
  SC_REQUIRE(K % 4 == 0 && ldw % 4 == 0 && (uintptr_t)w % 16 == 0 && (uintptr_t)out % 8 == 0,
             "sc_ctc_split_rows: rows must be 16-byte aligned (K %% 4, ldw %% 4)");
  SC_REQUIRE(blank >= 0 && blank < V, "sc_ctc_split_rows: blank outside [0, V)");
  const int U1 = max_target_len + 1;
  const int64_t rows = (int64_t)B * U1;
  hipLaunchKernelGGL(ctc_split_rows_kernel, dim3((unsigned)((rows + 3) / 4)), dim3(256), 0,
                     (hipStream_t)stream, w, ldw, bias, V, K, targets, target_stride, U1, blank,
                     (__bf16*)out, bias_out, B);
  return launch_status("sc_ctc_split_rows");
}

extern "C" size_t sc_ctc_workspace_bytes(int B, int T, int max_target_len) {
  if (B <= 0 || T <= 0 || max_target_len < 0) return 256;
  return ws_layout(B, T, max_target_len, nullptr, nullptr);
}

static int ctc_check(const void* x, int x_dtype, int B, int T, int V, int max_target_len,
                     const int64_t* targets, const int64_t* in_lens, const int64_t* tgt_lens,
                     int blank, const void* ws, size_t wsb, const char* who) {
  SC_REQUIRE(x_dtype == SC_F32 || x_dtype == SC_BF16 || x_dtype == SC_F16,
             "%s: unsupported dtype %d", who, x_dtype);
  SC_REQUIRE(B >= 0 && T >= 0 && V > 0 && max_target_len >= 0, "%s: bad shape", who);
  SC_REQUIRE(ab_halo_k(max_target_len) > 0,
             "%s: max target length %d exceeds %d", who, max_target_len, 16 * 63 - 1);
  SC_REQUIRE(blank >= 0 && blank < V, "%s: blank %d outside [0, %d)", who, blank, V);
  SC_REQUIRE((int64_t)B * T <= 0x7fffffff, "%s: B*T too large", who);
  if (B == 0 || T == 0) return 0;
  SC_REQUIRE(x && in_lens && tgt_lens && ws, "%s: null pointer", who);
  SC_REQUIRE(max_target_len == 0 || targets, "%s: null targets", who);
  const size_t need = ws_layout(B, T, max_target_len, nullptr, nullptr);
  SC_REQUIRE(wsb >= need, "%s: workspace %zu < %zu bytes", who, wsb, need);
  return 0;
}

static CtcArgs make_args(const void* x, int is_logits, int B, int T, int V, int64_t sb, int64_t st,
                         const int64_t* targets, int64_t tgs, int umax, const int64_t* in_lens,
                         const int64_t* tgt_lens, int blank, float* nll, const void* ws,
                         const float* scale, void* grad) {
  CtcArgs a;
  a.x = x;
  a.is_logits = is_logits;
  a.B = B;
  a.T = T;
  a.V = V;
  a.S = 2 * umax + 1;
  a.Sp = 64 * states_per_lane(a.S);
  a.Umax = umax;
  a.lin = lin_ppl(umax) > 0;
  a.kh = a.lin ? kAb1R / 2 : ab_halo_k(umax);
  a.blank = blank;
  a.sb = sb;
  a.stt = st;
  a.tg = targets;
  a.tgs = tgs;
  a.in_lens = in_lens;
  a.tgt_lens = tgt_lens;
  a.nll = nll;
  ws_layout(B, T, umax, &a.ws, (void*)ws);
  a.scale = scale;
  a.grad = grad;
  a.ex = nullptr;
  a.exb = a.ext = 0;
  return a;
}

static int ex_check(const float* ex, int64_t ex_stride_b, int64_t ex_stride_t, int is_logits,
                    int T, int max_target_len, const char* who) {
  if (!ex) return 0;
  SC_REQUIRE(is_logits, "%s: emission logits need is_logits = 1", who);
  SC_REQUIRE(ex_stride_t >= max_target_len + 1 && ex_stride_b >= (int64_t)T * ex_stride_t,
             "%s: emission logits rows of max_target_len + 1 = %d", who, max_target_len + 1);
  return 0;
}

extern "C" int sc_ctc_fwd_ex(const void* x, int x_dtype, int is_logits, int B, int T, int V,
                             int64_t stride_b, int64_t stride_t, const int64_t* targets,
                             int64_t target_stride, int max_target_len, const int64_t* in_lens,
                             const int64_t* tgt_lens, int blank, const float* ex,
                             int64_t ex_stride_b, int64_t ex_stride_t, float* nll, void* workspace,
                             size_t workspace_bytes, void* stream) {
  clear_error();
  int rc = ctc_check(x, x_dtype, B, T, V, max_target_len, targets, in_lens, tgt_lens, blank,
                     workspace, workspace_bytes, "sc_ctc_fwd");
  if (rc) return rc;
  if (B == 0) return 0;
  SC_REQUIRE(nll, "sc_ctc_fwd: null nll");
  SC_REQUIRE(T > 0, "sc_ctc_fwd: T == 0 is handled by the caller");
  if ((rc = ex_check(ex, ex_stride_b, ex_stride_t, is_logits, T, max_target_len, "sc_ctc_fwd_ex")))
    return rc;
  CtcArgs a = make_args(x, is_logits, B, T, V, stride_b, stride_t, targets, target_stride,
                        max_target_len, in_lens, tgt_lens, blank, nll, workspace, nullptr, nullptr);
  a.ex = ex;
  a.exb = ex_stride_b;
  a.ext = ex_stride_t;
  hipStream_t st = (hipStream_t)stream;
  switch (x_dtype) {
    case SC_F32: launch_fwd<SC_F32>(a, st); break;
    case SC_BF16: launch_fwd<SC_BF16>(a, st); break;
    default: launch_fwd<SC_F16>(a, st); break;
  }
  return launch_status("sc_ctc_fwd");
}

extern "C" int sc_ctc_fwd(const void* x, int x_dtype, int is_logits, int B, int T, int V,
                          int64_t stride_b, int64_t stride_t, const int64_t* targets,
                          int64_t target_stride, int max_target_len, const int64_t* in_lens,
                          const int64_t* tgt_lens, int blank, float* nll, void* workspace,
                          size_t workspace_bytes, void* stream) {
  return sc_ctc_fwd_ex(x, x_dtype, is_logits, B, T, V, stride_b, stride_t, targets, target_stride,
                       max_target_len, in_lens, tgt_lens, blank, nullptr, 0, 0, nll, workspace,
                       workspace_bytes, stream);
}

extern "C" int sc_ctc_bwd_ex(const void* x, int x_dtype, int is_logits, int B, int T, int V,
                             int64_t stride_b, int64_t stride_t, const int64_t* targets,
                             int64_t target_stride, int max_target_len, const int64_t* in_lens,
                             const int64_t* tgt_lens, int blank, const float* ex,
                             int64_t ex_stride_b, int64_t ex_stride_t, const float* nll,
                             const float* scale, void* grad, int grad_dtype, const void* workspace,
                             size_t workspace_bytes, void* stream) {
  clear_error();
  int rc = ctc_check(x, x_dtype, B, T, V, max_target_len, targets, in_lens, tgt_lens, blank,
                     workspace, workspace_bytes, "sc_ctc_bwd");
  if (rc) return rc;
  if (B == 0 || T == 0) return 0;
  SC_REQUIRE(grad_dtype == SC_F32 || grad_dtype == SC_BF16 || grad_dtype == SC_F16,
             "sc_ctc_bwd: unsupported grad dtype %d", grad_dtype);
  SC_REQUIRE(nll && scale && grad, "sc_ctc_bwd: null pointer");
  if ((rc = ex_check(ex, ex_stride_b, ex_stride_t, is_logits, T, max_target_len, "sc_ctc_bwd_ex")))
    return rc;
  CtcArgs a = make_args(x, is_logits, B, T, V, stride_b, stride_t, targets, target_stride,
                        max_target_len, in_lens, tgt_lens, blank, (float*)nll, workspace, scale,
                        grad);
  a.ex = ex;
  a.exb = ex_stride_b;
  a.ext = ex_stride_t;
  hipStream_t st = (hipStream_t)stream;
#define SC_CTC_BWD(DT)                                               \
  switch (grad_dtype) {                                              \
    case SC_F32: launch_bwd<DT, SC_F32>(a, st); break;               \
    case SC_BF16: launch_bwd<DT, SC_BF16>(a, st); break;             \
    default: launch_bwd<DT, SC_F16>(a, st); break;                   \
  }
  switch (x_dtype) {
    case SC_F32: SC_CTC_BWD(SC_F32) break;
    case SC_BF16: SC_CTC_BWD(SC_BF16) break;
    default: SC_CTC_BWD(SC_F16) break;
  }
#undef SC_CTC_BWD
  return launch_status("sc_ctc_bwd");
}

extern "C" int sc_ctc_bwd(const void* x, int x_dtype, int is_logits, int B, int T, int V,
                          int64_t stride_b, int64_t stride_t, const int64_t* targets,
                          int64_t target_stride, int max_target_len, const int64_t* in_lens,
                          const int64_t* tgt_lens, int blank, const float* nll,
                          const float* scale, void* grad, int grad_dtype, const void* workspace,
                          size_t workspace_bytes, void* stream) {
  return sc_ctc_bwd_ex(x, x_dtype, is_logits, B, T, V, stride_b, stride_t, targets, target_stride,
                       max_target_len, in_lens, tgt_lens, blank, nullptr, 0, 0, nll, scale, grad,
                       grad_dtype, workspace, workspace_bytes, stream);
}

extern "C" int sc_ctc_mean(const float* nll, const int64_t* tgt_lens, int B, float* loss,
                           float* factor, void* stream) {
  clear_error();
  SC_REQUIRE(B > 0, "sc_ctc_mean: B must be positive");
  SC_REQUIRE(nll && tgt_lens && loss && factor, "sc_ctc_mean: null pointer");
  hipLaunchKernelGGL(ctc_mean_kernel, dim3(1), dim3(256), 0, (hipStream_t)stream, nll, tgt_lens, B,
                     loss, factor);
  return launch_status("sc_ctc_mean");
}
```

statecatcher_amd/csrc/tn_gemm.hip:

```cpp

#include "sc_common.h"

namespace sc {
namespace {

typedef __bf16 b8v __attribute__((ext_vector_type(8)));
typedef __bf16 b2v __attribute__((ext_vector_type(2)));
typedef float f4v __attribute__((ext_vector_type(4)));
typedef int i4v __attribute__((ext_vector_type(4)));

#ifndef SC_TN_ABL
#define SC_TN_ABL 0
#endif
#ifndef SC_TNW_FENCE
#define SC_TNW_FENCE 1
#endif
#ifndef SC_TNW_IL
#define SC_TNW_IL 0
#endif
#ifndef SC_TNW_EPI
#define SC_TNW_EPI 1
#endif
#ifndef SC_TNW_AB
#define SC_TNW_AB 0
#endif

constexpr int kBK = 64;
constexpr int kRowB = 128;
constexpr int kTN = 256;
constexpr int kSlots = 2;

struct TnArgs {
  const __bf16* A;
  const __bf16* B;
  __bf16* C;
  int M, N, K, ntn, tiles;
  uint32_t lda, ldb, ldc;
  uint32_t cbytes;
  int gm;
};

__device__ __forceinline__ int swz(int r) { return (r ^ (r >> 2) ^ (r >> 4)) & 7; }

__device__ __forceinline__ i4v lds_read16(uint32_t byte) {
  return *(const __attribute__((address_space(3))) i4v*)(size_t)byte;
}

template <int MF, int SPI>
__global__ void __launch_bounds__(512) tn_kernel(TnArgs a) {
  constexpr int TM = 32 * MF;
  constexpr int NP = (TM + kTN) / 8;
  constexpr int NPW = NP / 8;
  static_assert(NP % 8 == 0, "pieces must split evenly over the 8 waves");
  constexpr int kSlotB = (TM + kTN) * kRowB;
  constexpr int NST = 2 * MF;
  extern __shared__ __attribute__((aligned(16))) unsigned char lds[];
  const int lane = threadIdx.x & 63;
  const int w = uniform(threadIdx.x >> 6);
  const int wm = w >> 2, wn = w & 3;
  const int fr = lane & 15, fq = lane >> 4;

  const int G = gridDim.x, bid = blockIdx.x;
  const int xcd = bid % 8, qq = G / 8, rr = G % 8;
  const int lid = (xcd < rr ? xcd * (qq + 1) : rr * (qq + 1) + (xcd - rr) * qq) + bid / 8;
  const int nks = a.K / kBK;
  const int ntw = lid < a.tiles ? (a.tiles - lid + G - 1) / G : 0;
  const int NH = ntw * nks;
  const uint32_t lds0 = lds_addr(lds);

  int prow[NPW];
  uint32_t pcol[NPW];
#pragma unroll
  for (int q = 0; q < NPW; ++q) {
    const int R = 8 * (NPW * w + q) + (lane >> 3);
    prow[q] = R < TM ? R : R - TM;
    pcol[q] = 8u * (uint32_t)((lane & 7) ^ swz(prow[q]));
  }
  int st_h = 0, st_ks = 0, st_tile = lid;
  int st_m0 = (st_tile / a.ntn) * TM, st_n0 = (st_tile % a.ntn) * kTN;
  auto stage = [&]() __attribute__((always_inline)) {
    const uint32_t sb = lds0 + (st_h % kSlots) * kSlotB;
    const uint32_t k0 = (uint32_t)st_ks * kBK;
#pragma unroll
    for (int q = 0; q < NPW; ++q) {
      const int g = NPW * w + q;
      if (8 * g < TM) {
        const uint32_t row = (uint32_t)min(st_m0 + prow[q], a.M - 1);
        dma_to_lds_s<16>(a.A, (row * a.lda + k0 + pcol[q]) * 2u, sb + g * 1024);
      } else {
        const uint32_t row = (uint32_t)(st_n0 + prow[q]);
        dma_to_lds_s<16>(a.B, (row * a.ldb + k0 + pcol[q]) * 2u, sb + g * 1024);
      }
    }
    ++st_h;
    if (++st_ks == nks) {
      st_ks = 0;
      st_tile += G;
      st_m0 = (st_tile / a.ntn) * TM;
      st_n0 = (st_tile % a.ntn) * kTN;
    }
  };

  uint32_t offB[4];
#pragma unroll
  for (int nf = 0; nf < 4; ++nf) {
    const int r = wn * 64 + (fr >> 2) * 16 + nf * 4 + (fr & 3);
    offB[nf] = (uint32_t)(TM * kRowB + r * kRowB + 16 * (fq ^ swz(r)));
  }
  uint32_t offA[MF];
#pragma unroll
  for (int mf = 0; mf < MF; ++mf) {
    const int r = wm * (TM / 2) + mf * 16 + fr;
    offA[mf] = (uint32_t)(r * kRowB + 16 * (fq ^ swz(r)));
  }
  auto load_frags = [&](uint32_t sb, int kk, i4v (&bf)[4], i4v (&af)[MF]) __attribute__((always_inline)) {
    const uint32_t x = 64u * kk;
#pragma unroll
    for (int nf = 0; nf < 4; ++nf) bf[nf] = lds_read16(sb + (offB[nf] ^ x));
#pragma unroll
    for (int mf = 0; mf < MF; ++mf) af[mf] = lds_read16(sb + (offA[mf] ^ x));
  };

  f4v acc[MF][4];
#pragma unroll
  for (int mf = 0; mf < MF; ++mf)
#pragma unroll
    for (int nf = 0; nf < 4; ++nf) acc[mf][nf] = f4v{0.f, 0.f, 0.f, 0.f};
  auto mfmas = [&](const i4v (&bf)[4], const i4v (&af)[MF]) __attribute__((always_inline)) {
#pragma unroll
    for (int mf = 0; mf < MF; ++mf)
#pragma unroll
      for (int nf = 0; nf < 4; ++nf)
        acc[mf][nf] = __builtin_amdgcn_mfma_f32_16x16x32_bf16(
            __builtin_bit_cast(b8v, bf[nf]), __builtin_bit_cast(b8v, af[mf]), acc[mf][nf], 0, 0, 0);
  };

  const __amdgpu_buffer_rsrc_t crs = __builtin_amdgcn_make_buffer_rsrc(a.C, 0, a.cbytes, 0x00020000);
  i4v outv[NST];
  int st_done = NST;
  uint32_t obase = 0;
  auto pack = [&](int tile) __attribute__((always_inline)) {
    const int m0 = (tile / a.ntn) * TM, n0 = (tile % a.ntn) * kTN;
    const uint32_t row = (uint32_t)(m0 + wm * (TM / 2) + fr);
    obase = (row * a.ldc + (uint32_t)(n0 + wn * 64 + fq * 16)) * 2u;
#pragma unroll
    for (int mf = 0; mf < MF; ++mf)
#pragma unroll
      for (int hlf = 0; hlf < 2; ++hlf) {
        i4v v;
#pragma unroll
        for (int d = 0; d < 4; ++d) {
          const int nf = 2 * hlf + (d >> 1), j = 2 * (d & 1);
          const b2v p = {(__bf16)acc[mf][nf][j], (__bf16)acc[mf][nf][j + 1]};
          v[d] = __builtin_bit_cast(int, p);
        }
        outv[2 * mf + hlf] = v;
      }
#pragma unroll
    for (int mf = 0; mf < MF; ++mf)
#pragma unroll
      for (int nf = 0; nf < 4; ++nf) acc[mf][nf] = f4v{0.f, 0.f, 0.f, 0.f};
    st_done = 0;
  };
  auto store_some = [&](int n) __attribute__((always_inline)) {
    const int lo = st_done, hi = min(NST, st_done + n);
#pragma unroll
    for (int s = 0; s < NST; ++s)
      if (s >= lo && s < hi) {
        const uint32_t off = obase + (uint32_t)((s >> 1) * 16) * a.ldc * 2u + (uint32_t)((s & 1) * 16);
        __builtin_amdgcn_raw_buffer_store_b128(outv[s], crs, off, 0, 0);
      }
    st_done = hi;
  };

  if (NH > 0) {
    stage();
    dma_wait();
    lds_barrier();
  }
  int cur_ks = 0, cur_tile = lid;
  i4v bf0[4], af0[MF], bf1[4], af1[MF];
  for (int h = 0; h < NH; ++h) {
    if (st_done < NST) store_some(SPI);
    if (st_h < NH && !(SC_TN_ABL & 2)) stage();
    const uint32_t sb = lds0 + (h % kSlots) * kSlotB;
    load_frags(sb, 0, bf0, af0);
    load_frags(sb, 1, bf1, af1);
    if (SC_TN_ABL & 1) {
#pragma unroll
      for (int mf = 0; mf < MF; ++mf)
        acc[mf][0][0] += (float)(bf0[mf & 3][0] ^ af1[mf][1]) + (float)(bf1[mf & 3][2] ^ af0[mf][3]);
    } else {
      mfmas(bf0, af0);
      mfmas(bf1, af1);
    }
    if (++cur_ks == nks) {
      pack(cur_tile);
      cur_ks = 0;
      cur_tile += G;
    }
    dma_wait();
    lds_barrier();
  }
  if (st_done < NST) store_some(NST);
}

constexpr int kHalfB = 128 * kRowB;

#ifndef SC_TN_WL
#define SC_TN_WL 0
#endif
constexpr int kTnWN = SC_TN_WL ? 2 : 4;
constexpr int kTnMF = 128 / (8 / kTnWN) / 16;
constexpr int kTnNF = 128 / kTnWN / 16;
struct FragA { i4v v[kTnMF][2]; };
struct FragB { i4v v[kTnNF][2]; };

__global__ void __launch_bounds__(512, 1) tn256_kernel(TnArgs a) {
  extern __shared__ __attribute__((aligned(16))) unsigned char lds[];
  const int lane = threadIdx.x & 63;
  const int w = uniform(threadIdx.x >> 6);
  const int wm = w / kTnWN, wn = w % kTnWN;
  const int l15 = lane & 15, l4 = lane >> 4;

  const int G = gridDim.x, bid = blockIdx.x;
  const int xcd = bid % 8, qq = G / 8, rr = G % 8;
  const int lid = (xcd < rr ? xcd * (qq + 1) : rr * (qq + 1) + (xcd - rr) * qq) + bid / 8;
  const int nkt = a.K / kBK;
  const int ntw = lid < a.tiles ? (a.tiles - lid + G - 1) / G : 0;
  const int NG = ntw * nkt;
  const uint32_t lds0 = lds_addr(lds);

  int drow[2];
  uint32_t dcol[2];
#pragma unroll
  for (int q = 0; q < 2; ++q) {
    const int r = 8 * (2 * w + q) + (lane >> 3);
    drow[q] = r;
    dcol[q] = 8u * (uint32_t)((lane & 7) ^ swz(r));
  }
  int dg = 0, dkt = 0, dtile = lid;
  int dm0 = (dtile / a.ntn) * 256, dn0 = (dtile % a.ntn) * 256;
  auto dma_half = [&](int h) __attribute__((always_inline)) {
    const uint32_t dst = lds0 + (uint32_t)(((dg & 1) * 4 + h) * kHalfB + 2 * w * 1024);
    const uint32_t k0 = (uint32_t)dkt * kBK;
#pragma unroll
    for (int q = 0; q < 2; ++q) {
      if (h < 2) {
        const uint32_t row = (uint32_t)min(dm0 + h * 128 + drow[q], a.M - 1);
        dma_to_lds_s<16>(a.A, (row * a.lda + k0 + dcol[q]) * 2u, dst + q * 1024);
      } else {
        const uint32_t row = (uint32_t)(dn0 + (h - 2) * 128 + drow[q]);
        dma_to_lds_s<16>(a.B, (row * a.ldb + k0 + dcol[q]) * 2u, dst + q * 1024);
      }
    }
  };
  auto dma_next = [&]() __attribute__((always_inline)) {
    ++dg;
    if (++dkt == nkt) {
      dkt = 0;
      dtile += G;
      dm0 = (dtile / a.ntn) * 256;
      dn0 = (dtile % a.ntn) * 256;
    }
  };

  uint32_t offA[kTnMF], offB[kTnNF];
#pragma unroll
  for (int mf = 0; mf < kTnMF; ++mf) {
    const int r = wm * 16 * kTnMF + mf * 16 + l15;
    offA[mf] = (uint32_t)(r * kRowB + 16 * (l4 ^ swz(r)));
  }
#pragma unroll
  for (int nf = 0; nf < kTnNF; ++nf) {
    const int r = wn * 16 * kTnNF + (l15 >> 2) * 4 * kTnNF + nf * 4 + (l15 & 3);
    offB[nf] = (uint32_t)(r * kRowB + 16 * (l4 ^ swz(r)));
  }
  auto half_base = [&](int buf, int h) __attribute__((always_inline)) {
    return lds0 + (uint32_t)((buf * 4 + h) * kHalfB);
  };
  auto read_A = [&](int buf, int qm, FragA& f) __attribute__((always_inline)) {
    const uint32_t hb = half_base(buf, qm);
#pragma unroll
    for (int kk = 0; kk < 2; ++kk)
#pragma unroll
      for (int mf = 0; mf < kTnMF; ++mf) f.v[mf][kk] = lds_read16(hb + (offA[mf] ^ (64u * kk)));
  };
  auto read_B = [&](int buf, int qn, FragB& f) __attribute__((always_inline)) {
    const uint32_t hb = half_base(buf, 2 + qn);
#pragma unroll
    for (int kk = 0; kk < 2; ++kk)
#pragma unroll
      for (int nf = 0; nf < kTnNF; ++nf) f.v[nf][kk] = lds_read16(hb + (offB[nf] ^ (64u * kk)));
  };

  f4v acc[4][kTnMF][kTnNF];
#pragma unroll
  for (int q = 0; q < 4; ++q)
#pragma unroll
    for (int mf = 0; mf < kTnMF; ++mf)
#pragma unroll
      for (int nf = 0; nf < kTnNF; ++nf) acc[q][mf][nf] = f4v{0.f, 0.f, 0.f, 0.f};
  auto quad = [&](f4v (&c)[kTnMF][kTnNF], const FragA& fa, const FragB& fb) __attribute__((always_inline)) {
    __builtin_amdgcn_s_setprio(1);
#pragma unroll
    for (int kk = 0; kk < 2; ++kk)
#pragma unroll
      for (int mf = 0; mf < kTnMF; ++mf)
#pragma unroll
        for (int nf = 0; nf < kTnNF; ++nf) {
          if (SC_TN_ABL & 1)
            c[mf][nf][0] += (float)(fb.v[nf][kk][0] ^ fa.v[mf][kk][1]);
          else
            c[mf][nf] = __builtin_amdgcn_mfma_f32_16x16x32_bf16(
                __builtin_bit_cast(b8v, fb.v[nf][kk]), __builtin_bit_cast(b8v, fa.v[mf][kk]),
                c[mf][nf], 0, 0, 0);
        }
    __builtin_amdgcn_s_setprio(0);
  };

  const __amdgpu_buffer_rsrc_t crs = __builtin_amdgcn_make_buffer_rsrc(a.C, 0, a.cbytes, 0x00020000);
  auto store_quad = [&](f4v (&c)[kTnMF][kTnNF], int m0, int n0, int qm, int qn) __attribute__((always_inline)) {
    if (SC_TN_ABL & 4) return;
    const uint32_t row = (uint32_t)(m0 + qm * 128 + wm * 16 * kTnMF + l15);
    const uint32_t col = (uint32_t)(n0 + qn * 128 + wn * 16 * kTnNF + l4 * 4 * kTnNF);
#pragma unroll
    for (int mf = 0; mf < kTnMF; ++mf) {
#pragma unroll
      for (int s2 = 0; s2 < kTnNF / 2; ++s2) {
        i4v v;
#pragma unroll
        for (int d = 0; d < 4; ++d) {
          const int nf = 2 * s2 + (d >> 1), j = 2 * (d & 1);
          const b2v p = {(__bf16)c[mf][nf][j], (__bf16)c[mf][nf][j + 1]};
          v[d] = __builtin_bit_cast(int, p);
        }
        __builtin_amdgcn_raw_buffer_store_b128(v, crs, ((row + 16u * mf) * a.ldc + col + 8u * s2) * 2u,
                                               0, 0);
      }
#pragma unroll
      for (int nf = 0; nf < kTnNF; ++nf) c[mf][nf] = f4v{0.f, 0.f, 0.f, 0.f};
    }
  };

  if (NG == 0) return;
#pragma unroll
  for (int g0 = 0; g0 < 2; ++g0)
    if (dg < NG) {
// ... 586 lines not shown
    for (int i = 0; i < 8; ++i)
#pragma unroll
      for (int j = 0; j < 8; ++j) asm volatile("" ::"a"(acc[i][j]));
    return;
  }
  const __amdgpu_buffer_rsrc_t crs = __builtin_amdgcn_make_buffer_rsrc(a.C, 0, a.cbytes, 0x00020000);
  const uint32_t col = (uint32_t)(n0 + wn * 128 + l4 * 32);
  float rr[32];
  if constexpr (LN) {
    const float inv = 1.0f / (float)a.K;
    const float m1 = (ls1a + ls1b) * inv;
    const float var = fmaxf((ls2a + ls2b) * inv - m1 * m1, 0.0f);
    const float2 sr = make_float2(rsq(var + ln.eps), lsh + m1);
    typedef float f2 __attribute__((ext_vector_type(2)));
    *(__attribute__((address_space(3))) f2*)(size_t)(lds0 + kStat + (uint32_t)t * 8u) = f2{sr.x, sr.y};
    if (n0 == 0 && m0 + t < a.M) ln.stat[m0 + t] = sr;
    lds_barrier();
    const uint32_t rb = lds0 + kR + (uint32_t)(wn * 128 + l4 * 32) * 4u;
#pragma unroll
    for (int q = 0; q < 8; ++q) {
      const i4v v = lds_read16(rb + 16u * q);
#pragma unroll
      for (int e = 0; e < 4; ++e) rr[4 * q + e] = __int_as_float(v[e]);
    }
  }
  const uint32_t blk = lds0 + (uint32_t)w * 32768u;
  if (SC_TNW_EPI && !LN) lds_barrier();
#pragma unroll
  for (int i = 0; i < 8; ++i) {
    const uint32_t row = (uint32_t)(m0 + wm * 128 + i * 16 + l15);
    typedef float f2 __attribute__((ext_vector_type(2)));
    f2 sr = {1.f, 0.f};
    if constexpr (LN)
      sr = *(const __attribute__((address_space(3))) f2*)(size_t)(
          lds0 + kStat + (uint32_t)(wm * 128 + i * 16 + l15) * 8u);
#pragma unroll
    for (int s4 = 0; s4 < 4; ++s4) {
      i4v v;
#pragma unroll
      for (int d = 0; d < 4; ++d) {
        const int j = 2 * s4 + (d >> 1), e = 2 * (d & 1);
        float c0 = acc[i][j][e], c1 = acc[i][j][e + 1];
        if constexpr (LN) {
          c0 = (c0 - sr.y * rr[4 * j + e]) * sr.x;
          c1 = (c1 - sr.y * rr[4 * j + e + 1]) * sr.x;
        }
        const b2v p = {(__bf16)c0, (__bf16)c1};
        v[d] = __builtin_bit_cast(int, p);
      }
      if (SC_TNW_EPI) {
        const uint32_t rl = (uint32_t)(i * 16 + l15), c = (uint32_t)(l4 * 4 + s4);
        *(__attribute__((address_space(3))) i4v*)(size_t)(blk + rl * 256u + 16u * (c ^ (rl & 15u))) = v;
      } else {
        __builtin_amdgcn_raw_buffer_store_b128(v, crs, (row * a.ldc + col + 8u * s4) * 2u, 0, 0);
      }
    }
  }
  if (SC_TNW_EPI) {
    lds_read_wait();
    const uint32_t ch = (uint32_t)(lane & 15);
#pragma unroll
    for (int it = 0; it < 32; ++it) {
      const uint32_t rl = (uint32_t)(4 * it + (lane >> 4));
      const i4v v = lds_read16(blk + rl * 256u + 16u * (ch ^ (rl & 15u)));
      const uint32_t row = (uint32_t)(m0 + wm * 128) + rl;
      __builtin_amdgcn_raw_buffer_store_b128(
          v, crs, (row * a.ldc + (uint32_t)(n0 + wn * 128) + 8u * ch) * 2u, 0, 0);
    }
  }
}

template <int NS, bool LN>
int launch_tnw32(const TnArgs& a, const TnLn& ln, hipStream_t st) {
  constexpr size_t lds = (size_t)NS * tnw32::kSlot + (LN ? 3072 : 0);
  static_assert(!LN || lds <= 160 * 1024, "LN needs a spare 3 KiB of LDS");
  static const bool ok = hipFuncSetAttribute((const void*)tnw32_kernel<NS, LN>,
                                             hipFuncAttributeMaxDynamicSharedMemorySize,
                                             (int)lds) == hipSuccess;
  (void)ok;
  const int npan = (a.M + 255) / 256;
  const int grid = 8 * ((npan + 7) / 8) * a.ntn;
  hipLaunchKernelGGL((tnw32_kernel<NS, LN>), dim3(grid), dim3(256), lds, st, a, ln);
  return 0;
}

#ifndef SC_TNR
#define SC_TNR 0
#endif
#if SC_TNR
template <bool LN>
__global__ void __launch_bounds__(256, 1) tnr_kernel(TnArgs a, TnLn ln) {
  using namespace tnw32;
  using tnw::Frag;
  extern __shared__ __attribute__((aligned(16))) unsigned char lds[];
  const int lane = threadIdx.x & 63;
  const int w = uniform(threadIdx.x >> 6);
  const int wm = w >> 1, wn = w & 1;
  const int l15 = lane & 15, l4 = lane >> 4;
  const int bid = blockIdx.x;
  const int npan = (a.M + 255) / 256;
  const int xcd = bid % 8, k = bid / 8;
  const int pq = npan / 8, pr = npan % 8;
  const int np = pq + (xcd < pr), p0 = xcd * pq + min(xcd, pr);
  if (k >= np * a.ntn) return;
  const int grp = k / (a.gm * a.ntn), first = grp * a.gm;
  const int gsz = min(a.gm, np - first), within = k - grp * a.gm * a.ntn;
  const int m0 = (p0 + first + within % gsz) * 256, n0 = (within / gsz) * 256;
  const int nst = a.K / 32;
  const uint32_t lds0 = lds_addr(lds);

  const int r0 = 64 * w + (lane >> 2);
  uint32_t voA[4], chq[4];
#pragma unroll
  for (int q = 0; q < 4; ++q) {
    chq[q] = 16u * (uint32_t)((lane & 3) ^ f64(r0 + 16 * q));
    voA[q] = (uint32_t)min(m0 + r0 + 16 * q, a.M - 1) * a.lda * 2u + chq[q];
  }
  const uint32_t voB0 = ((uint32_t)(n0 + r0) * a.ldb) * 2u;
  const __amdgpu_buffer_rsrc_t ra =
      __builtin_amdgcn_make_buffer_rsrc((void*)a.A, 0, (int)(a.M * a.lda * 2u), 0x00020000);
  const __amdgpu_buffer_rsrc_t rb =
      __builtin_amdgcn_make_buffer_rsrc((void*)a.B, 0, (int)((uint32_t)a.N * a.ldb * 2u), 0x00020000);
  struct Stg { i4v a[4], b[4]; };
  auto gload = [&](int st, Stg& g) __attribute__((always_inline)) {
    const uint32_t so = (uint32_t)st * 64u;
#pragma unroll
    for (int q = 0; q < 4; ++q)
      g.a[q] = __builtin_amdgcn_raw_buffer_load_b128(ra, voA[q], so, 0);
#pragma unroll
    for (int q = 0; q < 4; ++q)
      g.b[q] = __builtin_amdgcn_raw_buffer_load_b128(rb, voB0 + chq[q], so + 32u * q * a.ldb, 0);
  };
  const uint32_t wlane = (uint32_t)(w * 4 * 1024 + lane * 16);
  auto dswrite = [&](int st, const Stg& g) __attribute__((always_inline)) {
    const uint32_t sb = lds0 + (uint32_t)((st & 1) * kSlot) + wlane;
#pragma unroll
    for (int q = 0; q < 4; ++q)
      *(__attribute__((address_space(3))) i4v*)(size_t)(sb + q * 1024) = g.a[q];
#pragma unroll
    for (int q = 0; q < 4; ++q)
      *(__attribute__((address_space(3))) i4v*)(size_t)(sb + kHalf + q * 1024) = g.b[q];
  };
  uint32_t ox4[4], ow4[4];
  {
    const uint32_t bx = (uint32_t)((wm * 128 + l15) * kRow + 16 * ((l4 ^ (2 * ((l15 >> 3) & 1))) & 3));
    const int rw0 = wn * 128 + (l15 >> 2) * 32 + (l15 & 3);
    const uint32_t bw = (uint32_t)(kHalf + rw0 * kRow + 16 * ((l4 ^ (2 * ((l15 >> 2) & 1))) & 3));
#pragma unroll
    for (int g = 0; g < 4; ++g) {
      ox4[g] = bx ^ (16u * g);
      ow4[g] = bw ^ (16u * g);
    }
  }
  auto read = [&](int st, Frag& fx, Frag& fw) __attribute__((always_inline)) {
    const uint32_t sb = lds0 + (uint32_t)((st & 1) * kSlot);
#pragma unroll
    for (int f = 0; f < 8; ++f) fw.v[f] = lds_read16(sb + ow4[(2 * ((f >> 1) & 1)) ^ (f >> 2)] + 256u * f);
#pragma unroll
    for (int f = 0; f < 8; ++f) fx.v[f] = lds_read16(sb + ox4[f & 3] + 1024u * f);
  };
  f4v acc[8][8];
#pragma unroll
  for (int i = 0; i < 8; ++i)
#pragma unroll
    for (int j = 0; j < 8; ++j) acc[i][j] = f4v{0.f, 0.f, 0.f, 0.f};
  auto mfmas = [&](const Frag& fx, const Frag& fw, int i0, int i1) __attribute__((always_inline)) {
#pragma unroll
    for (int i = 0; i < 8; ++i) {
      if (i < i0 || i >= i1) continue;
#pragma unroll
      for (int j = 0; j < 8; ++j)
        acc[i][j] = __builtin_amdgcn_mfma_f32_16x16x32_bf16(
            __builtin_bit_cast(b8v, fw.v[j]), __builtin_bit_cast(b8v, fx.v[i]), acc[i][j], 0, 0, 0);
    }
  };
  constexpr uint32_t kR = 2u * kSlot, kStat = kR + 1024;
  const int t = threadIdx.x;
  float lsh = 0.f, ls1a = 0.f, ls1b = 0.f, ls2a = 0.f, ls2b = 0.f;
  const uint32_t statoff = (uint32_t)(t * kRow + 16 * f64(t));
  if constexpr (LN) {
    if (w == 0) {
      const i4v rv = __builtin_amdgcn_raw_buffer_load_b128(
          __builtin_amdgcn_make_buffer_rsrc((void*)ln.r, 0, (int)(a.N * 4), 0x00020000),
          (uint32_t)(n0 + 4 * lane) * 4u, 0, 0);
      *(__attribute__((address_space(3))) i4v*)(size_t)(lds0 + kR + (uint32_t)lane * 16u) = rv;
    }
  }
  auto stat_read = [&](int st, i4v (&rv)[4]) __attribute__((always_inline)) {
    if constexpr (LN) {
      const uint32_t sb = lds0 + (uint32_t)((st & 1) * kSlot);
#pragma unroll
      for (int c = 0; c < 4; ++c) rv[c] = lds_read16(sb + (statoff ^ (16u * c)));
    }
  };
  auto stat_acc = [&](int st, const i4v (&rv)[4]) __attribute__((always_inline)) {
    if constexpr (LN) {
      if (st == 0) lsh = __uint_as_float((uint32_t)rv[0][0] << 16);
#pragma unroll
      for (int c = 0; c < 4; ++c)
#pragma unroll
        for (int d = 0; d < 4; ++d) {
          const uint32_t u = (uint32_t)rv[c][d];
          const float x0 = __uint_as_float(u << 16) - lsh, x1 = __uint_as_float(u & 0xffff0000u) - lsh;
          ls1a += x0;
          ls1b += x1;
          ls2a = fmaf(x0, x0, ls2a);
          ls2b = fmaf(x1, x1, ls2b);
        }
    }
  };
  i4v sv[4];
  Stg S0, S1;
  Frag X, Xw, Y, Yw;
  gload(0, S0);
  gload(1, S1);
  dswrite(0, S0);
  if (2 < nst) gload(2, S0);
  dswrite(1, S1);
  if (3 < nst) gload(3, S1);
  lds_barrier();
  read(0, X, Xw);
  stat_read(0, sv);
  stat_acc(0, sv);
  auto step = [&](int s, Frag& F, Frag& Fw, Frag& N, Frag& Nw, Stg& G) __attribute__((always_inline)) {
    if (s + 1 < nst) {
      read(s + 1, N, Nw);
      stat_read(s + 1, sv);
    }
    __builtin_amdgcn_sched_barrier(0);
    mfmas(F, Fw, 0, 2);
    if (s + 1 < nst) stat_acc(s + 1, sv);
    __builtin_amdgcn_sched_barrier(0);
    if (s + 2 < nst) dswrite(s + 2, G);
    if (s + 4 < nst) gload(s + 4, G);
    __builtin_amdgcn_sched_barrier(0);
    mfmas(F, Fw, 2, 8);
    lds_barrier();
  };
  for (int s = 0; s < nst; s += 2) {
    step(s, X, Xw, Y, Yw, S0);
    step(s + 1, Y, Yw, X, Xw, S1);
  }
  const __amdgpu_buffer_rsrc_t crs = __builtin_amdgcn_make_buffer_rsrc(a.C, 0, a.cbytes, 0x00020000);
  const uint32_t col = (uint32_t)(n0 + wn * 128 + l4 * 32);
  float rr[32];
  if constexpr (LN) {
    const float inv = 1.0f / (float)a.K;
    const float m1 = (ls1a + ls1b) * inv;
    const float var = fmaxf((ls2a + ls2b) * inv - m1 * m1, 0.0f);
    const float2 sr = make_float2(rsq(var + ln.eps), lsh + m1);
    typedef float f2 __attribute__((ext_vector_type(2)));
    *(__attribute__((address_space(3))) f2*)(size_t)(lds0 + kStat + (uint32_t)t * 8u) = f2{sr.x, sr.y};
    if (n0 == 0 && m0 + t < a.M) ln.stat[m0 + t] = sr;
    lds_barrier();
    const uint32_t rb2 = lds0 + kR + (uint32_t)(wn * 128 + l4 * 32) * 4u;
#pragma unroll
    for (int q = 0; q < 8; ++q) {
      const i4v v = lds_read16(rb2 + 16u * q);
#pragma unroll
      for (int e = 0; e < 4; ++e) rr[4 * q + e] = __int_as_float(v[e]);
    }
  }
#pragma unroll
  for (int i = 0; i < 8; ++i) {
    const uint32_t row = (uint32_t)(m0 + wm * 128 + i * 16 + l15);
    typedef float f2 __attribute__((ext_vector_type(2)));
    f2 sr = {1.f, 0.f};
    if constexpr (LN)
      sr = *(const __attribute__((address_space(3))) f2*)(size_t)(
          lds0 + kStat + (uint32_t)(wm * 128 + i * 16 + l15) * 8u);
#pragma unroll
    for (int s4 = 0; s4 < 4; ++s4) {
      i4v v;
#pragma unroll
      for (int d = 0; d < 4; ++d) {
        const int j = 2 * s4 + (d >> 1), e = 2 * (d & 1);
        float c0 = acc[i][j][e], c1 = acc[i][j][e + 1];
        if constexpr (LN) {
          c0 = (c0 - sr.y * rr[4 * j + e]) * sr.x;
          c1 = (c1 - sr.y * rr[4 * j + e + 1]) * sr.x;
        }
        const b2v p = {(__bf16)c0, (__bf16)c1};
        v[d] = __builtin_bit_cast(int, p);
      }
      __builtin_amdgcn_raw_buffer_store_b128(v, crs, (row * a.ldc + col + 8u * s4) * 2u, 0, 0);
    }
  }
}

template <bool LN>
int launch_tnr(const TnArgs& a, const TnLn& ln, hipStream_t st) {
  constexpr size_t lds = 2 * (size_t)tnw32::kSlot + (LN ? 3072 : 0);
  static const bool ok = hipFuncSetAttribute((const void*)tnr_kernel<LN>,
                                             hipFuncAttributeMaxDynamicSharedMemorySize,
                                             (int)lds) == hipSuccess;
  (void)ok;
  const int npan = (a.M + 255) / 256;
  const int grid = 8 * ((npan + 7) / 8) * a.ntn;
  hipLaunchKernelGGL((tnr_kernel<LN>), dim3(grid), dim3(256), lds, st, a, ln);
  return 0;
}
#endif

int launch_tn256(const TnArgs& a, hipStream_t st) {
  constexpr size_t lds = 2 * 4 * (size_t)kHalfB;
  static const bool ok = hipFuncSetAttribute((const void*)tn256_kernel,
                                             hipFuncAttributeMaxDynamicSharedMemorySize,
                                             (int)lds) == hipSuccess;
  (void)ok;
  const int grid = a.tiles < 256 ? a.tiles : 256;
  hipLaunchKernelGGL(tn256_kernel, dim3(grid), dim3(512), lds, st, a);
  return 0;
}

int launch_tnpp(const TnArgs& a, hipStream_t st) {
  constexpr size_t lds = 2 * 4 * (size_t)kHalfB;
  static const bool ok = hipFuncSetAttribute((const void*)tnpp_kernel,
                                             hipFuncAttributeMaxDynamicSharedMemorySize,
                                             (int)lds) == hipSuccess;
  (void)ok;
  const int grid = a.tiles < 256 ? a.tiles : 256;
  hipLaunchKernelGGL(tnpp_kernel, dim3(grid), dim3(512), lds, st, a);
  return 0;
}

template <int MF, int SPI>
int launch_tn(const TnArgs& a, hipStream_t st) {
  auto kern = tn_kernel<MF, SPI>;
  constexpr size_t lds = (size_t)kSlots * (32 * MF + kTN) * kRowB;
  static const bool ok = hipFuncSetAttribute((const void*)kern,
                                             hipFuncAttributeMaxDynamicSharedMemorySize,
                                             (int)lds) == hipSuccess;
  (void)ok;
  const int grid = a.tiles < 256 ? a.tiles : 256;
  hipLaunchKernelGGL(kern, dim3(grid), dim3(512), lds, st, a);
  return 0;
}

}
}

using namespace sc;

extern "C" int sc_gemm_tn_bf16(const void* A, int64_t lda, const void* B, int64_t ldb, void* C,
                               int64_t ldc, int M, int N, int K, int tile_m, void* stream) {
  clear_error();
  SC_REQUIRE(A && B && C, "sc_gemm_tn_bf16: null pointer");
  SC_REQUIRE(M > 0 && N > 0 && K > 0, "sc_gemm_tn_bf16: empty shape M=%d N=%d K=%d", M, N, K);
  SC_REQUIRE(K % kBK == 0, "sc_gemm_tn_bf16: K=%d must be a multiple of 64 (zero-pad it)", K);
  SC_REQUIRE(N % kTN == 0, "sc_gemm_tn_bf16: N=%d must be a multiple of 256", N);
  SC_REQUIRE(tile_m == 0 || (SC_TNW_AB && tile_m >= 1 && tile_m <= 3) || tile_m == 128 ||
                 tile_m == 192 || tile_m == 256 || tile_m == 257,
             "sc_gemm_tn_bf16: tile_m=%d must be 0 (default 192), 128, 192, 256 or 257 (256, "
             "ping-pong schedule); 1 / 2 / 3 (one wave per SIMD) in SC_TNW_AB builds only",
             tile_m);
  SC_REQUIRE(lda >= K && ldb >= K && ldc >= N && lda % 8 == 0 && ldb % 8 == 0 && ldc % 8 == 0,
             "sc_gemm_tn_bf16: leading dimensions must cover the rows in 16-byte pieces");
  SC_REQUIRE((uintptr_t)A % 16 == 0 && (uintptr_t)B % 16 == 0 && (uintptr_t)C % 16 == 0,
             "sc_gemm_tn_bf16: operands must be 16-byte aligned");
  SC_REQUIRE((int64_t)M * lda * 2 < (1ll << 32) && (int64_t)N * ldb * 2 < (1ll << 32) &&
                 ((int64_t)M + 256) * ldc * 2 < (1ll << 32),
             "sc_gemm_tn_bf16: operands must be smaller than 4 GiB");
  const int tm = (tile_m == 257 || (tile_m >= 1 && tile_m <= 3)) ? 256 : tile_m ? tile_m : 192;
  const int ntn = N / kTN;
  const int64_t tiles = (int64_t)((M + tm - 1) / tm) * ntn;
  SC_REQUIRE(tiles < (1 << 30), "sc_gemm_tn_bf16: too many tiles");
  static const int gm = [] {
    const char* e = getenv("SC_TN_GM");
    const int v = e ? atoi(e) : 8;
    return v >= 1 ? v : 8;
  }();
  TnArgs a{(const __bf16*)A, (const __bf16*)B, (__bf16*)C, M, N, K, ntn, (int)tiles,
           (uint32_t)lda, (uint32_t)ldb, (uint32_t)ldc, (uint32_t)((int64_t)M * ldc * 2), gm};
  hipStream_t st = (hipStream_t)stream;
#if SC_TNW_AB
  if (tile_m == 1) {
    launch_tnw(a, st);
    return launch_status("sc_gemm_tn_bf16");
  }
  if (tile_m == 2 || tile_m == 3) {
#if SC_TNR
    launch_tnr<false>(a, TnLn{}, st);
#else
    if (tile_m == 2) launch_tnw32<5, false>(a, TnLn{}, st);
    else launch_tnw32<4, false>(a, TnLn{}, st);
#endif
    return launch_status("sc_gemm_tn_bf16");
  }
#endif
  if (tile_m == 257) {
    launch_tnpp(a, st);
    return launch_status("sc_gemm_tn_bf16");
  }
  if (tm == 256) {
    launch_tn256(a, st);
    return launch_status("sc_gemm_tn_bf16");
  }
  const int nks = K / kBK, nst = 2 * (tm / 32);
  const int spi = (nst + nks - 1) / nks;
  if (tm == 128) {
    if (spi <= 1) launch_tn<4, 1>(a, st);
    else if (spi <= 2) launch_tn<4, 2>(a, st);
    else if (spi <= 4) launch_tn<4, 4>(a, st);
    else launch_tn<4, 8>(a, st);
  } else {
    if (spi <= 1) launch_tn<6, 1>(a, st);
    else if (spi <= 2) launch_tn<6, 2>(a, st);
    else if (spi <= 4) launch_tn<6, 4>(a, st);
    else if (spi <= 6) launch_tn<6, 6>(a, st);
    else launch_tn<6, 12>(a, st);
  }
  return launch_status("sc_gemm_tn_bf16");
}

extern "C" int sc_gemm_tn_ln_bf16(const void* H, int64_t ldh, const void* Wpp, int64_t ldw, void* C,
                                  int64_t ldc, int M, int N, int K, const float* r, void* stat,
                                  float eps, void* stream) {
  clear_error();
  SC_REQUIRE(H && Wpp && C && r && stat, "sc_gemm_tn_ln_bf16: null pointer");
  SC_REQUIRE(M > 0 && N > 0 && K > 0 && K % 64 == 0 && N % 256 == 0,
             "sc_gemm_tn_ln_bf16: shape M=%d N=%d K=%d (K %% 64, N %% 256)", M, N, K);
  SC_REQUIRE(ldh >= K && ldw >= K && ldc >= N && ldh % 8 == 0 && ldw % 8 == 0 && ldc % 8 == 0,
             "sc_gemm_tn_ln_bf16: leading dimensions must cover the rows in 16-byte pieces");
  SC_REQUIRE(((uintptr_t)H | (uintptr_t)Wpp | (uintptr_t)C | (uintptr_t)r) % 16 == 0 &&
                 (uintptr_t)stat % 8 == 0,
             "sc_gemm_tn_ln_bf16: misaligned operand");
  SC_REQUIRE((int64_t)M * ldh * 2 < (1ll << 32) && (int64_t)N * ldw * 2 < (1ll << 32) &&
                 ((int64_t)M + 256) * ldc * 2 < (1ll << 32),
             "sc_gemm_tn_ln_bf16: operands must be smaller than 4 GiB");
  const int ntn = N / 256;
  const int64_t tiles = (int64_t)((M + 255) / 256) * ntn;
  TnArgs a{(const __bf16*)H, (const __bf16*)Wpp, (__bf16*)C, M, N, K, ntn, (int)tiles,
           (uint32_t)ldh, (uint32_t)ldw, (uint32_t)ldc, (uint32_t)((int64_t)M * ldc * 2), 8};
#if SC_TNR
  launch_tnr<true>(a, TnLn{r, (float2*)stat, eps}, (hipStream_t)stream);
#else
  launch_tnw32<4, true>(a, TnLn{r, (float2*)stat, eps}, (hipStream_t)stream);
#endif
  return launch_status("sc_gemm_tn_ln_bf16");
}
```

statecatcher_amd/ops.py:

```python
import ctypes
import os

import torch

from . import _lib
from ._lib import check, dtype_code, ptr, require_device, stream_of

LAUNCH_EVENTS = None


class _timed:

    def __init__(self, name, t, nbytes, flops=0):
        self.rec = LAUNCH_EVENTS is not None
        if self.rec:
            self.name, self.nbytes, self.flops = name, nbytes, flops
            self.stream = torch.cuda.current_stream(t.device)
            self.e0 = torch.cuda.Event(enable_timing=True)
            self.e1 = torch.cuda.Event(enable_timing=True)

    def __enter__(self):
        if self.rec:
            self.e0.record(self.stream)
        return self
# ... 400 lines not shown
        part = None
        if (USE_WGRAD_STREAM and ctx.needs_input_grad[0] and ctx.needs_input_grad[1]
                and dg2.is_cuda and dg2.dtype == torch.bfloat16 and xc.dtype == torch.bfloat16):
            main = torch.cuda.current_stream(dg2.device)
            side = _side_stream(dg2.device)
            side.wait_stream(main)
            with torch.cuda.stream(side):
                with _timed("gate_gemm_wgrad", dg2, 0):
                    part = wgrad_mfma_slabs(dg2, xc)
            if part is not None:
                dg2.record_stream(side)
                xc.record_stream(side)
        dx = None
        if ctx.needs_input_grad[0]:
            with _timed("gate_gemm_dgrad", dg2, 0):
                dx = torch.matmul(dg2, wt.t()) if wt is not None else proj_dgrad(dg2, wc)
            dx = dx.to(xdt)
        dw = None
        if part is not None:
            main.wait_stream(side)
            part.record_stream(main)
            dw = wgrad_slab_sum(part, bd)
            if dw.shape[1] != ctx.din:
                dw = dw[:, :ctx.din].contiguous()
            dw = dw.to(wdt)
        elif ctx.needs_input_grad[1]:
            with _timed("gate_gemm_wgrad", dg2, 0):
                dw = wgrad_splitk(dg2, xc, blocked_d=bd)
            if dw.shape[1] != ctx.din:
                dw = dw[:, :ctx.din].contiguous()
            dw = dw.to(wdt)
        db = colsum(dbias.view(dbias.shape[0], -1)).to(wdt) if dbias is not None else None
        return dx, dw, db, dh0.to(hdt), ds0.to(sdt), None, None, None, None, None, None


def lucy_cell(x, w, b, h0, s0, cdt=None, imgs=None, split_sink=None, rec_sink=None):
    B, T, Din = x.shape
    if cdt is None:
        cdt = torch.promote_types(x.dtype, w.dtype)
    return LucyCellFn.apply(x.reshape(B * T, Din), w, b, h0, s0, B, T, cdt, imgs, split_sink,
                            rec_sink)


LN_FOLD_MODE = int(os.environ.get("SC_LN_FOLD", "0") or 0)
USE_LN_FOLD = LN_FOLD_MODE in (1, 2)
_FOLD = WeakIdKeyDictionary()


def ln_fold_ok(D):
    return USE_LN_FOLD and D in (512, 1024)


def gemm_tn_ln(h2d, wpp, r_img, eps):
    M, K = h2d.shape
    N = wpp.shape[0]
    c = torch.empty(M, N, dtype=torch.bfloat16, device=h2d.device)
    stat = torch.empty(M, 2, dtype=torch.float32, device=h2d.device)
    rc = _lib.load().sc_gemm_tn_ln_bf16(ptr(h2d), h2d.stride(0), ptr(wpp), wpp.stride(0), ptr(c),
                                        c.stride(0), M, N, K, ptr(r_img), ptr(stat), float(eps),
                                        stream_of(h2d))
    check(rc, "sc_gemm_tn_ln_bf16")
    return c, stat


def fold_images(specs):
    out, preps, jobs, keep = [None] * len(specs), [], [], []
    for i, (w, b, g, be, bd, kp, want_t) in enumerate(specs):
        key = (w._version, w.data_ptr(), b._version, b.data_ptr(), g._version, g.data_ptr(),
               be._version, be.data_ptr(), bd, kp, bool(want_t))
        hit = _FOLD.get(w)
        if hit is not None and hit[0] == key:
            out[i] = hit[1]
            continue
        rows, cols = w.shape
        f32 = dict(dtype=torch.float32, device=w.device)
        shift, bprime, rowsum = (torch.empty(rows, **f32) for _ in range(3))
        preps.append(_lib.LnFoldJob(w.data_ptr(), g.data_ptr(), be.data_ptr(), b.data_ptr(),
                                    shift.data_ptr(), bprime.data_ptr(), rowsum.data_ptr(),
                                    w.stride(0), rows, cols))
        img = torch.empty(rows, kp, dtype=torch.bfloat16, device=w.device)
        img_t = torch.empty(cols, rows, dtype=torch.bfloat16, device=w.device) if want_t else None
        jobs.append(_lib.ImageJob(w.data_ptr(), img.data_ptr(),
                                  img_t.data_ptr() if img_t is not None else None, rows, cols, kp,
                                  w.stride(0), bd, g.data_ptr(), shift.data_ptr()))
        keep += [w, b, g, be, shift]
        r_img = torch.empty_like(rowsum) if bd and rows % (7 * 64) == 0 else None
        out[i] = (img, img_t, bprime, rowsum, r_img if r_img is not None else rowsum)
        _FOLD[w] = (key, out[i])
    if preps:
        require_device(*keep)
        lib = _lib.load()
        for k in range(0, len(preps), 16):
            part = preps[k:k + 16]
            check(lib.sc_ln_fold_prep((_lib.LnFoldJob * len(part))(*part), len(part),
                                      stream_of(keep[0])), "sc_ln_fold_prep")
        _image_jobs(jobs, keep)
        for o in out:
            if o is not None and o[4] is not o[3]:
                rows = o[3].numel()
                o[4].copy_(o[3].view(7, rows // (7 * 64), 64).transpose(0, 1).reshape(-1))
    return out


def ln_fold_bwd(g, h, stat):
    M, D = h.shape
    g = g.contiguous()
    dh = torch.empty_like(h)
    check(_lib.load().sc_ln_fold_bwd(ptr(g), ptr(h), dtype_code(h), ptr(stat), ptr(dh), M, D,
                                     stream_of(h)), "sc_ln_fold_bwd")
    return dh


def ln_fold_wgrad(Mw, w, gamma, beta, dbp):
    rows, D = Mw.shape
    lib = _lib.load()
    dw = torch.empty(rows, D, dtype=torch.float32, device=Mw.device)
    dgb = torch.empty(2, D, dtype=torch.float32, device=Mw.device)
    ws = torch.empty(lib.sc_ln_fold_wgrad_workspace_numel(rows, D), dtype=torch.float32,
                     device=Mw.device)
    g = gamma.detach().contiguous()
    be = beta.detach().contiguous()
    wd = w.detach()
    check(lib.sc_ln_fold_wgrad(ptr(Mw.contiguous()), ptr(wd), wd.stride(0), ptr(g), ptr(be),
                               ptr(dbp.contiguous()), rows, D, ptr(dw), ptr(dgb), ptr(ws),
                               stream_of(Mw)), "sc_ln_fold_wgrad")
    return dw, dgb[0], dgb[1]


class LucyCellLNFn(torch.autograd.Function):

    @staticmethod
    def forward(ctx, h2d, w, b, gamma, beta, h0, s0, B, T, fimgs, rec_in, eps, split_sink=None,
                rec_sink=None):
        ctx.set_materialize_grads(False)
        D = w.shape[0] // 7
        wg, wt, bprime, rowsum, r_img = fimgs
        need = any(ctx.needs_input_grad)
        if LN_FOLD_MODE == 2:
            with _timed("gate_gemm_fwd", h2d, 0):
                gates, stat = gemm_tn_ln(h2d, wg, r_img, eps)
            gates = gates.view(B, T, D // 64, 7, 64)
            stat = stat.view(B, T, 2)
            res = _scan_fwd(gates, h0, s0, need, bprime, want_h=True, split=split_sink is not None)
            rowsum = None
        else:
            with _timed("gate_gemm_fwd", h2d, 0):
                gates = proj_fwd(h2d, wg)
            gates = gates.view(B, T, D // 64, 7, 64)
            stat = torch.empty(B, T, 2, dtype=torch.float32, device=h2d.device)
            rec = None
            if rec_sink is not None:
                rec = torch.empty(B, T, D // 64, 2, dtype=torch.float32, device=h2d.device)
                rec_sink.append(rec)
            res = _scan_fwd(gates, h0, s0, need, bprime, want_h=True, split=split_sink is not None,
                            ln=(rowsum, rec_in, stat, rec, eps))
        gates, out, s_out, ckpt, h_out = res[:5]
        if len(res) > 5:
            split_sink.append(res[5])
        if need:
            ctx.save_for_backward(h2d, wt, gates, ckpt, bprime, rowsum, stat, w, gamma, beta)
            ctx.dtypes = (h2d.dtype, w.dtype, h0.dtype, s0.dtype, gamma.dtype, beta.dtype)
        return out, s_out, h_out

    @staticmethod
    def backward(ctx, dout, ds_last, dh_last):
        h2d, wt, gates, ckpt, bprime, rowsum, stat, w, gamma, beta = ctx.saved_tensors
        xdt, wdt, hdt, sdt, gdt, bdt = ctx.dtypes
        if dh_last is not None:
            B, T = gates.shape[:2]
            if dout is None:
                dout = torch.zeros(B, T, dh_last.shape[-1], dtype=gates.dtype, device=gates.device)
            else:
                dout = dout.clone()
            dout[:, -1] += dh_last.to(dout.dtype)
        need_w = any(ctx.needs_input_grad[1:5])
        dgates, dh0, ds0, dbias = _scan_bwd(gates, ckpt, dout, ds_last, need_w, bprime,
                                            ln=(rowsum, stat))
        dg2 = dgates.view(h2d.shape[0], -1)
        D = h2d.shape[1]
        dh = None
        if ctx.needs_input_grad[0]:
            with _timed("gate_gemm_dgrad", dg2, 0):
                g = torch.matmul(dg2, wt.t())
            dh = ln_fold_bwd(g, h2d, stat.view(-1, 2)).to(xdt)
        dw = db = dgam = dbet = None
        if need_w:
            with _timed("gate_gemm_wgrad", dg2, 0):
                Mw = wgrad_splitk(dg2, h2d, blocked_d=D)
            dbp = colsum(dbias.view(dbias.shape[0], -1))
            dw, dgam, dbet = ln_fold_wgrad(Mw, w, gamma, beta, dbp)
            dw, db, dgam, dbet = dw.to(wdt), dbp.to(wdt), dgam.to(gdt), dbet.to(bdt)
        return (dh, dw, db, dgam, dbet, dh0.to(hdt), ds0.to(sdt), None, None, None, None, None,
                None, None)


def lucy_cell_ln(h, w, b, gamma, beta, h0, s0, fimgs, rec_in, eps, split_sink=None, rec_sink=None):
    B, T, D = h.shape
    h2 = h.reshape(B * T, D)
    if not h2.is_contiguous() or h2.data_ptr() % 16:
        h2 = h2.contiguous()
    return LucyCellLNFn.apply(h2, w, b, gamma, beta, h0, s0, B, T, fimgs, rec_in, eps,
                              split_sink, rec_sink)


class LayerNormFn(torch.autograd.Function):

    @staticmethod
    def forward(ctx, x, gamma, beta, eps):
        require_device(x)
        D = x.shape[-1]
        x2 = x.reshape(-1, D)
        if not x2.is_contiguous() or x2.data_ptr() % 16:
            x2 = x2.contiguous()
        rows = x2.shape[0]
        g = gamma.detach().to(torch.float32).contiguous()
        b = beta.detach().to(torch.float32).contiguous()
        y = torch.empty_like(x2)
        mean = torch.empty(rows, dtype=torch.float32, device=x.device)
        rstd = torch.empty(rows, dtype=torch.float32, device=x.device)
        rc = _lib.load().sc_layernorm_fwd(ptr(x2), dtype_code(x2), ptr(g), ptr(b), ptr(y), ptr(mean),
                                          ptr(rstd), rows, D, float(eps), stream_of(x2))
        check(rc, "sc_layernorm_fwd")
        ctx.save_for_backward(x2, g, mean, rstd)
        ctx.pdtypes = (gamma.dtype, beta.dtype)
        return y.view(x.shape)

    @staticmethod
    def backward(ctx, dy):
        x2, g, mean, rstd = ctx.saved_tensors
        rows, D = x2.shape
        dy2 = dy.reshape(rows, D).to(x2.dtype)
        if not dy2.is_contiguous() or dy2.data_ptr() % 16:
            dy2 = dy2.contiguous()
        lib = _lib.load()
        dx = torch.empty_like(x2)
        dgb = torch.empty(2, D, dtype=torch.float32, device=x2.device)
        ws = torch.empty(lib.sc_layernorm_bwd_workspace_numel(rows, D), dtype=torch.float32,
                         device=x2.device)
        rc = lib.sc_layernorm_bwd(ptr(x2), ptr(dy2), dtype_code(x2), ptr(g), ptr(mean), ptr(rstd),
                                  ptr(dx), ptr(dgb), ptr(ws), rows, D, stream_of(x2))
        check(rc, "sc_layernorm_bwd")
        gd, bd = ctx.pdtypes
        return dx.view(dy.shape), dgb[0].to(gd), dgb[1].to(bd), None


def layer_norm(x, gamma, beta, eps=1e-5):
    return LayerNormFn.apply(x, gamma, beta, eps)


def layer_norm_supported(x):
    return x.dtype in _lib._DTYPE and bool(_lib.load().sc_layernorm_supported(dtype_code(x), x.shape[-1]))


class DecayScanFn(torch.autograd.Function):

    @staticmethod
    def forward(ctx, kv, decay, init):
        require_device(kv, decay, init)
        if kv.shape != decay.shape or kv.dim() != 3:
            raise ValueError(f"kv/decay must be equal [B,T,D]; got {tuple(kv.shape)}, {tuple(decay.shape)}")
        decay = decay.to(kv.dtype)
        kv = kv.contiguous()
        decay = decay.contiguous()
        B, T, D = kv.shape
        initc = None if init is None else init.detach().to(torch.float32).contiguous()
        out = torch.empty_like(kv)
        rc = _lib.load().sc_decay_scan_fwd(ptr(kv), ptr(decay), ptr(out), dtype_code(kv), ptr(initc),
                                           B, T, D, kv.stride(0), kv.stride(1), 1, stream_of(kv))
        check(rc, "sc_decay_scan_fwd")
        ctx.save_for_backward(decay, out, initc)
        ctx.has_init = init is not None
        ctx.init_dtype = None if init is None else init.dtype
        return out

    @staticmethod
    def backward(ctx, dout):
        decay, s_all, initc = ctx.saved_tensors
        B, T, D = decay.shape
        dout = dout.to(decay.dtype).contiguous()
        dkv = torch.empty_like(decay)
        ddec = torch.empty_like(decay)
        dinit = torch.zeros(B, D, dtype=torch.float32, device=decay.device) if ctx.has_init else None
        rc = _lib.load().sc_decay_scan_bwd(ptr(decay), ptr(s_all), ptr(dout), ptr(dkv), ptr(ddec),
                                           dtype_code(decay), ptr(initc),
                                           ptr(dinit) if T > 0 else None, B, T, D,
                                           decay.stride(0), decay.stride(1), 1, stream_of(decay))
        check(rc, "sc_decay_scan_bwd")
        return dkv, ddec, (dinit.to(ctx.init_dtype) if ctx.has_init else None)


def decay_scan(kv, decay, init=None):
    return DecayScanFn.apply(kv, decay, init)


def _as_len_tensor(x, device):
    if isinstance(x, torch.Tensor):
        return x.to(device=device, dtype=torch.int64).contiguous()
    return torch.as_tensor(list(x), dtype=torch.int64).to(device, non_blocking=True)


class CTCFn(torch.autograd.Function):

    @staticmethod
    def forward(ctx, x, targets, in_lens, tgt_lens, blank, is_logits, ex=None):
        require_device(x, targets, in_lens, tgt_lens)
        if x.dim() != 3:
            raise ValueError(f"x must be [B,T,V], got {tuple(x.shape)}")
        B, T, V = x.shape
        if x.stride(2) != 1:
            x = x.contiguous()
        if targets.dim() != 2 or targets.shape[0] != B:
            raise ValueError("targets must be padded [B, U_max] (the layout train.py:208 builds); "
                             f"got {tuple(targets.shape)}")
        targets = targets.to(torch.int64).contiguous()
        umax = targets.shape[1]
        nll = torch.empty(B, dtype=torch.float32, device=x.device)
        lib = _lib.load()
        wsb = lib.sc_ctc_workspace_bytes(B, max(T, 1), umax)
        ws = torch.empty(wsb, dtype=torch.uint8, device=x.device)
        if ex is not None:
            require_device(x, ex)
            if (ex.dtype != torch.float32 or ex.shape != (B, T, umax + 1) or ex.stride(2) != 1):
                raise ValueError(f"ex must be fp32 [B, T, U_max + 1] = {(B, T, umax + 1)} with unit "
                                 f"column stride; got {ex.dtype} {tuple(ex.shape)}")
        if T == 0:
            nll = torch.where(tgt_lens == 0, 0.0, float("inf")).to(torch.float32)
        else:
            rc = lib.sc_ctc_fwd_ex(ptr(x), dtype_code(x), int(is_logits), B, T, V, x.stride(0),
                                   x.stride(1), ptr(targets), targets.stride(0) if umax else 0, umax,
                                   ptr(in_lens), ptr(tgt_lens), blank, ptr(ex),
                                   ex.stride(0) if ex is not None else 0,
                                   ex.stride(1) if ex is not None else 0, ptr(nll), ptr(ws), wsb,
                                   stream_of(x))
            check(rc, "sc_ctc_fwd_ex")
        ctx.save_for_backward(x, targets, in_lens, tgt_lens, nll, ws)
        ctx.meta = (blank, int(is_logits), umax, wsb)
        ctx.ex = ex
        return nll

    @staticmethod
    def _bwd(ctx, x, targets, in_lens, tgt_lens, nll, ws, scale, grad):
        blank, is_logits, umax, wsb = ctx.meta
        B, T, V = x.shape
        ex = ctx.ex
        rc = _lib.load().sc_ctc_bwd_ex(ptr(x), dtype_code(x), is_logits, B, T, V, x.stride(0),
                                       x.stride(1), ptr(targets), targets.stride(0) if umax else 0,
                                       umax, ptr(in_lens), ptr(tgt_lens), blank, ptr(ex),
                                       ex.stride(0) if ex is not None else 0,
                                       ex.stride(1) if ex is not None else 0, ptr(nll), ptr(scale),
                                       ptr(grad), dtype_code(grad), ptr(ws), wsb, stream_of(x))
        check(rc, "sc_ctc_bwd_ex")

    @staticmethod
    def backward(ctx, grad_nll):
        x, targets, in_lens, tgt_lens, nll, ws = ctx.saved_tensors
        blank, is_logits, umax, wsb = ctx.meta
        B, T, V = x.shape
        grad = torch.empty(B, T, V, dtype=x.dtype, device=x.device)
        if T > 0:
            scale = grad_nll.to(torch.float32).contiguous()
            CTCFn._bwd(ctx, x, targets, in_lens, tgt_lens, nll, ws, scale, grad)
        return grad, None, None, None, None, None, None


class CTCMeanFn(torch.autograd.Function):

    @staticmethod
    def forward(ctx, x, targets, in_lens, tgt_lens, blank, is_logits, ex=None):
        nll = CTCFn.forward(ctx, x, targets, in_lens, tgt_lens, blank, is_logits, ex)
        B = nll.shape[0]
        loss = torch.empty((), dtype=torch.float32, device=x.device)
        factor = torch.empty(B, dtype=torch.float32, device=x.device)
        if B:
            rc = _lib.load().sc_ctc_mean(ptr(nll), ptr(tgt_lens), B, ptr(loss), ptr(factor),
                                         stream_of(x))
            check(rc, "sc_ctc_mean")
        else:
            loss.fill_(float("nan"))
        ctx.factor = factor
        return loss

    @staticmethod
    def backward(ctx, grad_loss):
        return CTCFn.backward(ctx, ctx.factor * grad_loss)


def _logits_fp32(x2, wc, b):
    return torch.addmm(b, x2, wc.t(), out_dtype=torch.float32)


_SPLIT_W = WeakIdKeyDictionary()

HEAD_SPLIT = os.environ.get("SC_HEAD_SPLIT", "emis")
if HEAD_SPLIT not in ("emis", "labels", "full"):
    raise ValueError(f"SC_HEAD_SPLIT={HEAD_SPLIT!r}: expected 'emis', 'labels' or 'full'")


def _emission_logits(wide, w, b, targets, blank, V):
    B, T, K3 = wide.shape
    K = K3 // 3
    U1 = targets.shape[1] + 1
    wg = torch.empty(B, U1, K3, dtype=torch.bfloat16, device=wide.device)
    bg = torch.empty(B, U1, dtype=torch.float32, device=wide.device)
    tgc = targets.to(torch.int64).contiguous()
    wc_ = w.detach().contiguous()
    rc = _lib.load().sc_ctc_split_rows(ptr(wc_), wc_.stride(0), ptr(b.detach().contiguous()), V, K,
                                       ptr(tgc), tgc.stride(0) if U1 > 1 else 0, U1 - 1, blank,
                                       ptr(wg), ptr(bg), B, stream_of(wide))
    check(rc, "sc_ctc_split_rows")
    ex = torch.bmm(wide, wg.transpose(1, 2), out_dtype=torch.float32)
    ex += bg.unsqueeze(1)
    return ex


def _emission_columns(targets, blank, V):
    B = targets.shape[0]
    return torch.cat([torch.full((B, 1), blank, dtype=torch.int64, device=targets.device),
                      targets.clamp(0, V - 1)], 1)


def _exact_emission_columns(logits, wide, w, b, targets, blank):
    B, T, V = logits.shape
    ex = _emission_logits(wide, w, b, targets, blank, V)
    lab = _emission_columns(targets, blank, V)
    logits.scatter_(2, lab.unsqueeze(1).expand(B, T, lab.shape[1]), ex)


def split_weight_image(w):
    key = (w._version, w.data_ptr(), tuple(w.shape))
    hit = _SPLIT_W.get(w)
    if hit is not None and hit[0] == key:
        return hit[1]
    with torch.no_grad():
        wd = w.detach()
        hi = wd.to(torch.bfloat16)
        lo = (wd - hi.float()).to(torch.bfloat16)
        img = torch.cat([hi, lo, hi], 1)
    _SPLIT_W[w] = (key, img)
    return img


class CTCHeadFn(torch.autograd.Function):

    @staticmethod
    def forward(ctx, x, w, b, wc, wt, targets, in_lens, tgt_lens, blank, wide=None):
        ctx.set_materialize_grads(False)
        B, T, K = x.shape
        V = w.shape[0]
        x2 = x.reshape(-1, K)
        ex = None
        if wide is not None and HEAD_SPLIT == "full":
            logits = _logits_fp32(wide.view(-1, 3 * K), split_weight_image(w), b).view(B, T, V)
        elif wide is not None and HEAD_SPLIT == "emis":
            logits = torch.addmm(b.to(torch.bfloat16), x2, wc.t()).view(B, T, V)
            ex = _emission_logits(wide.view(B, T, 3 * K), w, b, targets, blank, V)
        else:
            logits = _logits_fp32(x2, wc, b).view(B, T, V)
            if wide is not None:
                _exact_emission_columns(logits, wide, w, b, targets, blank)
        loss = CTCMeanFn.forward(ctx, logits, targets, in_lens, tgt_lens, blank, True, ex)
        ctx.head = (x2, wt, x.shape, x.dtype)
        return loss, logits

    @staticmethod
    def backward(ctx, g_loss, g_logits):
        logits, targets, in_lens, tgt_lens, nll, ws = ctx.saved_tensors
        blank, is_logits, umax, wsb = ctx.meta
        x2, wt, xshape, xdt = ctx.head
        B, T, V = logits.shape
        dy = torch.empty(B, T, V, dtype=torch.bfloat16, device=logits.device)
        if g_loss is None:
            dy.zero_()
        elif T > 0:
            scale = (ctx.factor * g_loss).to(torch.float32).contiguous()
            CTCFn._bwd(ctx, logits, targets, in_lens, tgt_lens, nll, ws, scale, dy)
        if g_logits is not None:
            dy = (dy.float() + g_logits).to(torch.bfloat16)
        dy2 = dy.view(-1, V)
        dx = torch.matmul(dy2, wt.t()).view(xshape).to(xdt) if ctx.needs_input_grad[0] else None
        dw = wgrad_splitk(dy2, x2) if ctx.needs_input_grad[1] else None
        db = colsum(dy2) if ctx.needs_input_grad[2] else None
        return dx, dw, db, None, None, None, None, None, None, None


def ctc_head_supported(x, w, b, imgs):
    return (imgs is not None and imgs[1] is not None and x.is_cuda and x.dtype == torch.bfloat16
            and x.dim() == 3 and b is not None and w.dtype == torch.float32
            and b.dtype == torch.float32)


def ctc_head_loss(x, w, b, imgs, targets, in_lens, tgt_lens, blank=0, wide=None):
    dev = x.device
    if wide is not None and not (wide.is_contiguous() and wide.shape[:2] == x.shape[:2]
                                 and wide.shape[2] == 3 * x.shape[2]
                                 and x.data_ptr() == wide.data_ptr()):
        raise ValueError("ctc_head_loss: wide must be the [B,T,3D] buffer x is the head of")
    if wide is None:
        x = x.contiguous()
    return CTCHeadFn.apply(x, w, b, imgs[0], imgs[1], targets.to(dev),
                           _as_len_tensor(in_lens, dev), _as_len_tensor(tgt_lens, dev), int(blank),
                           wide)


def ctc_nll(x, targets, in_lens, tgt_lens, blank=0, is_logits=True):
    dev = x.device
    return CTCFn.apply(x, targets.to(dev), _as_len_tensor(in_lens, dev), _as_len_tensor(tgt_lens, dev),
                       int(blank), bool(is_logits))


def ctc_loss(x, targets, in_lens, tgt_lens, blank=0, reduction="mean", zero_infinity=True,
             is_logits=True):
    dev = x.device
    tl = _as_len_tensor(tgt_lens, dev)
    if reduction == "mean" and zero_infinity:
        return CTCMeanFn.apply(x, targets.to(dev), _as_len_tensor(in_lens, dev), tl, int(blank),
                               bool(is_logits))
    nll = CTCFn.apply(x, targets.to(dev), _as_len_tensor(in_lens, dev), tl, int(blank), bool(is_logits))
    if zero_infinity:
        nll = torch.where(torch.isinf(nll), torch.zeros_like(nll), nll)
    if reduction == "none":
        return nll
    if reduction == "sum":
        return nll.sum()
    if reduction == "mean":
        return (nll / tl.clamp_min(1).to(nll.dtype)).mean()
    raise ValueError(f"unknown reduction {reduction!r}")


def ctc_greedy_decode(log_probs, lengths, blank=0):
    require_device(log_probs)
    B, T, V = log_probs.shape
    if log_probs.stride(2) != 1:
        log_probs = log_probs.contiguous()
    lens = _as_len_tensor(lengths, log_probs.device)
    tokens = torch.empty(B, T, dtype=torch.int32, device=log_probs.device)
    counts = torch.empty(B, dtype=torch.int32, device=log_probs.device)
    rc = _lib.load().sc_ctc_greedy_decode(ptr(log_probs), dtype_code(log_probs), B, T, V,
                                          log_probs.stride(0), log_probs.stride(1), ptr(lens),
                                          int(blank), ptr(tokens), ptr(counts), stream_of(log_probs))
    check(rc, "sc_ctc_greedy_decode")
    return tokens, counts


def ctc_greedy_step(logits, prev, emit, mask=None, blank=0):
    require_device(logits, prev, emit)
    B, V = logits.shape
    if logits.stride(1) != 1 or prev.dtype != torch.int32 or emit.dtype != torch.int32:
        raise ValueError("ctc_greedy_step: logits need unit inner stride, prev/emit int32")
    if prev.numel() != B or emit.numel() != B or not prev.is_contiguous():
        raise ValueError("ctc_greedy_step: prev/emit must hold B entries (prev contiguous)")
    if mask is not None and (mask.dtype != torch.float32 or mask.numel() != B or mask.stride(0) != 1):
        raise ValueError("ctc_greedy_step: mask must be contiguous fp32 [B]")
    rc = _lib.load().sc_ctc_greedy_step(ptr(logits), dtype_code(logits), B, V, logits.stride(0),
                                        ptr(mask), int(blank), ptr(prev), ptr(emit),
                                        emit.stride(0), stream_of(logits))
    check(rc, "sc_ctc_greedy_step")


STEP_FUSED, STEP_UNFUSED_A, STEP_UNFUSED_B = 0, 1, 2


def lucy_step_ln(x, w, b, out, eps=1e-5):
    B, D = x.shape
    rc = _lib.load().sc_lucy_step_ln(ptr(x), dtype_code(x), ptr(w), ptr(b), float(eps), ptr(out),
                                     B, D, stream_of(x))
    check(rc, "sc_lucy_step_ln")


def lucy_step_cell(mode, g, h, s, out, lnz=None, lnh=None, u=None, hp=None, mask=None, eps=1e-5):
    B, D = h.shape
    lzw, lzb = lnz if lnz is not None else (None, None)
    lhw, lhb = lnh if lnh is not None else (None, None)
    rc = _lib.load().sc_lucy_step_cell(int(mode), ptr(g), dtype_code(g), g.stride(0), ptr(u),
                                       ptr(hp), ptr(lzw), ptr(lzb), ptr(lhw), ptr(lhb), float(eps),
                                       ptr(h), ptr(s), ptr(out), ptr(mask), B, D, stream_of(g))
    check(rc, "sc_lucy_step_cell")


FRAME_PLAIN, FRAME_STATS, FRAME_CELL_UNFUSED, FRAME_CELL_FUSED = 0, 1, 2, 3


def lucy_frame_gemm(epi, x, w, bias, y, st_out=None, ln=None, st_in=None, z=None, st_z=None,
                    s=None, mask=None, eps=1e-5):
    B, K = x.shape
    N = w.shape[0]
    lw, lb = ln if ln is not None else (None, None)
    rc = _lib.load().sc_lucy_frame_gemm(
        int(epi), ptr(x), x.stride(0), K, ptr(lw), ptr(lb), ptr(st_in),
        st_in.shape[0] if st_in is not None else 0, float(eps), ptr(w), dtype_code(w), w.stride(0),
        ptr(bias), B, N, ptr(y), y.stride(0), ptr(st_out), ptr(z), ptr(st_z), ptr(s), ptr(mask),
        stream_of(x))
    check(rc, "sc_lucy_frame_gemm")


def lucy_frame_cellb(z, hp, h, out, st_z=None, st_h=None, lnz=None, lnh=None, mask=None, eps=1e-5):
    B, D = h.shape
    zw, zb = lnz if lnz is not None else (None, None)
    hw, hb = lnh if lnh is not None else (None, None)
    rc = _lib.load().sc_lucy_frame_cellb(
        ptr(z), ptr(st_z), st_z.shape[0] if st_z is not None else 0, ptr(hp), ptr(st_h),
        st_h.shape[0] if st_h is not None else 0, ptr(zw), ptr(zb), ptr(hw), ptr(hb), float(eps),
        ptr(h), ptr(out), out.stride(0), ptr(mask), B, D, stream_of(h))
    check(rc, "sc_lucy_frame_cellb")


def frame_gemm_job(x, w, bias, y, st_out=None, ln=None, st_in=None, z=None, st_z=None, s=None,
                   mask=None):
    B, K = x.shape
    lw, lb = ln if ln is not None else (None, None)
    return _lib.FrameGemmJob(ptr(x), x.stride(0), K, ptr(lw), ptr(lb), ptr(st_in),
                             st_in.shape[0] if st_in is not None else 0, ptr(w), w.stride(0),
                             ptr(bias), B, w.shape[0], ptr(y), y.stride(0), ptr(st_out), ptr(z),
                             ptr(st_z), ptr(s), ptr(mask))


def lucy_frame_gemm_multi(epi, w_dtype, jobs, stream, eps=1e-5):
    lib = _lib.load()
    code = dtype_code(torch.empty(0, dtype=w_dtype))
    for k in range(0, len(jobs), 8):
        part = jobs[k:k + 8]
        check(lib.sc_lucy_frame_gemm_multi(int(epi), code, float(eps),
                                           (_lib.FrameGemmJob * len(part))(*part), len(part),
                                           stream), "sc_lucy_frame_gemm_multi")


def frame_cell_job(z, hp, h, out, st_z=None, st_h=None, lnz=None, lnh=None, mask=None):
    B, D = h.shape
    zw, zb = lnz if lnz is not None else (None, None)
    hw, hb = lnh if lnh is not None else (None, None)
    return _lib.FrameCellJob(ptr(z), ptr(st_z), st_z.shape[0] if st_z is not None else 0, ptr(hp),
                             ptr(st_h), st_h.shape[0] if st_h is not None else 0, ptr(zw), ptr(zb),
                             ptr(hw), ptr(hb), ptr(h), ptr(out), out.stride(0), ptr(mask), B, D)


def lucy_frame_cellb_multi(jobs, stream, eps=1e-5):
    lib = _lib.load()
    for k in range(0, len(jobs), 8):
        part = jobs[k:k + 8]
        check(lib.sc_lucy_frame_cellb_multi(float(eps), (_lib.FrameCellJob * len(part))(*part),
                                            len(part), stream), "sc_lucy_frame_cellb_multi")


def ctc_greedy_frames(logits, prev, emit, mask=None, blank=0):
    require_device(logits, prev, emit)
    F, B, V = logits.shape
    if logits.stride(2) != 1 or prev.dtype != torch.int32 or emit.dtype != torch.int32:
        raise ValueError("ctc_greedy_frames: logits need unit inner stride, prev/emit int32")
    if prev.numel() != B or not prev.is_contiguous() or tuple(emit.shape) != (F, B):
        raise ValueError("ctc_greedy_frames: prev [B] contiguous, emit [F, B]")
    if mask is not None and (mask.dtype != torch.float32 or tuple(mask.shape) != (F, B)
                             or mask.stride(1) != 1):
        raise ValueError("ctc_greedy_frames: mask must be fp32 [F, B] with unit inner stride")
    rc = _lib.load().sc_ctc_greedy_frames(
        ptr(logits), dtype_code(logits), F, B, V, logits.stride(0), logits.stride(1), ptr(mask),
        mask.stride(0) if mask is not None else 0, int(blank), ptr(prev), ptr(emit),
        emit.stride(0), emit.stride(1), stream_of(logits))
    check(rc, "sc_ctc_greedy_frames")


def rnnt_greedy_decode(enc_p, pred_tab, W, bias, lengths=None, mask=None, blank=0, max_symbols=4,
                       prev=None, cap=None, return_frames=False, out=None):
    require_device(enc_p, pred_tab, W, bias, prev, mask)
    if enc_p.dim() != 3 or pred_tab.dim() != 2 or W.dim() != 2 or bias.dim() != 1:
        raise ValueError("rnnt_greedy_decode: enc_p [B,T,J], pred_tab [V,J], W [V,J], bias [V]")
    B, T, J = enc_p.shape
    V = W.shape[0]
    if tuple(W.shape) != (V, J) or tuple(pred_tab.shape) != (V, J) or bias.numel() != V:
        raise ValueError(f"rnnt_greedy_decode: pred_tab / W must be [V,J]=[{V},{J}] and bias [V], "
                         f"got {tuple(pred_tab.shape)}, {tuple(W.shape)}, {tuple(bias.shape)}")
    if pred_tab.dtype != enc_p.dtype or W.dtype != enc_p.dtype:
        raise ValueError("rnnt_greedy_decode: enc_p, pred_tab and W must share one dtype")
    if bias.dtype != torch.float32 or not bias.is_contiguous():
        raise ValueError("rnnt_greedy_decode: bias must be contiguous fp32 [V]")
    if (T > 0 and B > 0 and enc_p.stride(2) != 1) or not pred_tab.is_contiguous() \
            or not W.is_contiguous():
        raise ValueError("rnnt_greedy_decode: enc_p needs unit inner stride, pred_tab / W contiguous")
    if prev is not None and (prev.dtype != torch.int32 or prev.numel() != B
                             or not prev.is_contiguous()):
        raise ValueError("rnnt_greedy_decode: prev must be contiguous int32 [B]")
    if mask is not None and (mask.dtype != torch.float32 or tuple(mask.shape) != (B, T)):
        raise ValueError("rnnt_greedy_decode: mask must be fp32 [B, T]")
    lens = None if lengths is None else _as_len_tensor(lengths, enc_p.device)
    if lens is not None and lens.numel() != B:
        raise ValueError("rnnt_greedy_decode: lengths must have B entries")
    if out is not None:
        tokens, counts, frames = out
        cap = tokens.shape[1]
        ok = tokens.dtype == torch.int32 and tokens.is_contiguous() and tokens.shape[0] == B \
            and counts.dtype == torch.int32 and counts.is_contiguous() and counts.numel() == B \
            and (frames is None or (frames.dtype == torch.int32 and frames.is_contiguous()
                                    and frames.shape == tokens.shape))
        if not ok:
            raise ValueError("rnnt_greedy_decode: out = (tokens int32 [B,cap], counts int32 [B], "
                             "frames int32 [B,cap] or None), contiguous")
        require_device(tokens, counts, frames)
    else:
        cap = T * int(max_symbols) if cap is None else int(cap)
        if cap < 0:
            raise ValueError(f"rnnt_greedy_decode: cap={cap} is negative")
        tokens = torch.empty(B, cap, dtype=torch.int32, device=enc_p.device)
        counts = torch.empty(B, dtype=torch.int32, device=enc_p.device)
        frames = torch.empty(B, cap, dtype=torch.int32, device=enc_p.device) \
            if return_frames else None
    rc = _lib.load().sc_rnnt_greedy_decode(
        ptr(enc_p), ptr(pred_tab), ptr(W), dtype_code(enc_p), ptr(bias), B, T, V, J,
        enc_p.stride(0), enc_p.stride(1), ptr(lens), ptr(mask),
        mask.stride(0) if mask is not None else 0, mask.stride(1) if mask is not None else 0,
        int(blank), int(max_symbols), ptr(prev), ptr(tokens), ptr(frames), cap, ptr(counts),
        stream_of(enc_p))
    check(rc, "sc_rnnt_greedy_decode")
    return (tokens, counts, frames) if return_frames else (tokens, counts)


def fbank(audio, kind="mfcc", sample_rate=16000):
    require_device(audio)
    if audio.dim() != 2:
        raise ValueError(f"fbank: audio must be [B, N], got {tuple(audio.shape)}")
    codes = {"mfcc": 0, "mel": 1}
    if kind not in codes:
        raise ValueError(f"Unsupported frontend: {kind}")
    a = audio.to(torch.float32)
    if a.stride(1) != 1:
        a = a.contiguous()
    lib = _lib.load()
    B, N = a.shape
    F = lib.sc_fbank_frames(N)
    out = torch.empty(B, F, 80, dtype=torch.float32, device=a.device)
    wsb = lib.sc_fbank_workspace_bytes()
    ws = torch.empty(wsb, dtype=torch.uint8, device=a.device)
    rc = lib.sc_fbank(ptr(a), B, N, a.stride(0), codes[kind], float(sample_rate), ptr(out), ptr(ws),
                      wsb, stream_of(a))
    check(rc, "sc_fbank")
    return out


class RNNTFn(torch.autograd.Function):

    @staticmethod
    def forward(ctx, x, labels, flen, llen, blank, is_logits, row_off, T):
        require_device(x, labels, flen, llen)
        compact = row_off is not None
        if x.stride(-1) != 1:
            x = x.contiguous()
        if compact:
            if x.dim() != 2:
                raise ValueError(f"compact log_probs must be [rows, V], got {tuple(x.shape)}")
            B = flen.shape[0]
            V = x.shape[1]
            sb, st, su = 0, 0, x.stride(0)
        else:
            if x.dim() != 4:
                raise ValueError(f"log_probs must be [B,T,U+1,V], got {tuple(x.shape)}")
            B, T, U1, V = x.shape
            sb, st, su = x.stride(0), x.stride(1), x.stride(2)
        labels = labels.to(torch.int64).contiguous()
        if labels.dim() != 2 or labels.shape[0] != B:
            raise ValueError(f"labels must be padded [B, U_max], got {tuple(labels.shape)}")
        umax = labels.shape[1] if compact else x.shape[2] - 1
        if not compact and labels.shape[1] < umax:
            labels = torch.nn.functional.pad(labels, (0, umax - labels.shape[1]))
        nll = torch.empty(B, dtype=torch.float32, device=x.device)
        lib = _lib.load()
        wsb = lib.sc_rnnt_workspace_bytes(B, max(T, 1), umax)
# ... 669 lines not shown
```

Measured before the change: 9.333 million.

## Fuse emission bias into CTC kernels and prefetch rows in gradient kernel

The per-target emission bias is now passed into the CTC forward and backward kernels and added at load time, so the separate broadcast add over the [B,T,U+1] emission tensor goes away. The CTC gradient kernel is split into a preload stage and a per-row stage that software-pipelines alpha/beta, target and logit loads for the next row, and it gains a compile-time path for the emission case. A small-K GEMM dispatch and a new tile_m option are also added. The cost is more registers in the gradient kernel and extra bias loads inside the inner kernels.

New measurement: 9.406 million, median of 6. Within noise of the previous version (+0.8%).

```diff
diff --git a/include/statecatcher.h b/include/statecatcher.h
--- a/include/statecatcher.h
+++ b/include/statecatcher.h
@@ -133,6 +133,21 @@
                   const float* ex, int64_t ex_stride_b, int64_t ex_stride_t,
                   const float* nll, const float* scale, void* grad, int grad_dtype,
                   const void* workspace, size_t workspace_bytes, void* stream);
+int sc_ctc_fwd_exb(const void* x, int x_dtype, int is_logits, int B, int T, int V,
+                   int64_t stride_b, int64_t stride_t,
+                   const int64_t* targets, int64_t target_stride, int max_target_len,
+                   const int64_t* in_lens, const int64_t* tgt_lens, int blank,
+                   const float* ex, int64_t ex_stride_b, int64_t ex_stride_t,
+                   const float* ex_bias,
+                   float* nll, void* workspace, size_t workspace_bytes, void* stream);
+int sc_ctc_bwd_exb(const void* x, int x_dtype, int is_logits, int B, int T, int V,
+                   int64_t stride_b, int64_t stride_t,
+                   const int64_t* targets, int64_t target_stride, int max_target_len,
+                   const int64_t* in_lens, const int64_t* tgt_lens, int blank,
+                   const float* ex, int64_t ex_stride_b, int64_t ex_stride_t,
+                   const float* ex_bias,
+                   const float* nll, const float* scale, void* grad, int grad_dtype,
+                   const void* workspace, size_t workspace_bytes, void* stream);
 
 int sc_ctc_split_rows(const float* w, int64_t ldw, const float* bias, int V, int K,
                       const int64_t* targets, int64_t target_stride, int max_target_len,
diff --git a/statecatcher_amd/_lib.py b/statecatcher_amd/_lib.py
--- a/statecatcher_amd/_lib.py
+++ b/statecatcher_amd/_lib.py
@@ -58,6 +58,11 @@
     "sc_ctc_bwd_ex": (_i32, [_vp, _i32, _i32, _i32, _i32, _i32, _i64, _i64, _vp, _i64, _i32, _vp,
                             _vp, _i32, _fp, _i64, _i64, _fp, _fp, _vp, _i32, _vp, _c.c_size_t,
                             _vp]),
+    "sc_ctc_fwd_exb": (_i32, [_vp, _i32, _i32, _i32, _i32, _i32, _i64, _i64, _vp, _i64, _i32, _vp,
+                             _vp, _i32, _fp, _i64, _i64, _fp, _fp, _vp, _c.c_size_t, _vp]),
+    "sc_ctc_bwd_exb": (_i32, [_vp, _i32, _i32, _i32, _i32, _i32, _i64, _i64, _vp, _i64, _i32, _vp,
+                             _vp, _i32, _fp, _i64, _i64, _fp, _fp, _fp, _vp, _i32, _vp,
+                             _c.c_size_t, _vp]),
     "sc_ctc_split_rows": (_i32, [_fp, _i64, _fp, _i32, _i32, _vp, _i64, _i32, _i32, _vp, _fp,
                                  _i32, _vp]),
     "sc_ctc_greedy_decode": (_i32, [_vp, _i32, _i32, _i32, _i32, _i64, _i64, _vp, _i32, _vp, _vp, _vp]),
diff --git a/statecatcher_amd/csrc/ctc.hip b/statecatcher_amd/csrc/ctc.hip
--- a/statecatcher_amd/csrc/ctc.hip
+++ b/statecatcher_amd/csrc/ctc.hip
@@ -1,3 +1,5 @@
+#include <type_traits>
+
 #include "sc_common.h"
 
 #ifndef SC_CTC_ABL
@@ -98,7 +100,13 @@
   void* grad;
   const float* ex;
   int64_t exb, ext;
+  const float* exbias;
 };
+
+__device__ __forceinline__ float ex_ld(const CtcArgs& a, const float* exr, int b, int c) {
+  const float v = exr[c];
+  return a.exbias ? v + a.exbias[(int64_t)b * (a.Umax + 1) + c] : v;
+}
 
 __device__ __forceinline__ int clampi(int64_t v, int lo, int hi) {
   return (int)(v < lo ? lo : (v > hi ? hi : v));
@@ -126,16 +134,27 @@
   const float* exr = a.ex ? a.ex + (int64_t)b * a.exb + (int64_t)t * a.ext : nullptr;
   constexpr int kGx = 8;
   auto state_logit = [&](int s) {
-    return exr ? exr[(s & 1) ? (s + 1) >> 1 : 0] : E::ld(p[state_label(tg, s, a.blank, a.V)]);
+    return exr ? ex_ld(a, exr, b, (s & 1) ? (s + 1) >> 1 : 0)
+               : E::ld(p[state_label(tg, s, a.blank, a.V)]);
   };
   const bool inreg = a.Sp <= 64 * kGx;
-  float xs[kGx];
+  float xs[kGx], bs[kGx];
+#pragma unroll
+  for (int j = 0; j < kGx; ++j) bs[j] = 0.0f;
   if (inreg) {
     if (exr) {
 #pragma unroll
       for (int j = 0; j < kGx; ++j) {
         const int s = min(lane + 64 * j, Sb - 1);
         xs[j] = exr[(s & 1) ? (s + 1) >> 1 : 0];
+      }
+      if (a.exbias) {
+        const float* eb = a.exbias + (int64_t)b * (a.Umax + 1);
+#pragma unroll
+        for (int j = 0; j < kGx; ++j) {
+          const int s = min(lane + 64 * j, Sb - 1);
+          bs[j] = eb[(s & 1) ? (s + 1) >> 1 : 0];
+        }
       }
     } else {
       int lab[kGx];
@@ -178,6 +197,10 @@
       a.ws.lse[row] = lse;
       a.ws.lse64[row] = (double)M + (double)flog(l);
     }
+  }
+  if (inreg && exr && a.exbias) {
+#pragma unroll
+    for (int j = 0; j < kGx; ++j) xs[j] += bs[j];
   }
   float* out = a.ws.lpe + row * a.Sp;
   auto lp2x = [&](float xl) { return fmaxf((xl - lse) * kLog2e, -1e30f); };
@@ -878,6 +901,17 @@
     return ex ? __float_as_uint(xf.ld(col, so)) : xe.ldw(col, so);
   };
   auto cvt = [&](uint32_t w) { return ex ? __uint_as_float(w) : E::ldw(w); };
+  const bool exb = ex && a.exbias != nullptr;
+  float bB = 0.0f, bL[PPL];
+#pragma unroll
+  for (int j = 0; j < PPL; ++j) bL[j] = 0.0f;
+  if (exb) {
+    const float* eb = a.exbias + (int64_t)b * (a.Umax + 1);
+    bB = eb[0];
+#pragma unroll
+    for (int j = 0; j < PPL; ++j) bL[j] = eb[cL[j] >> 2];
+  }
+  auto cvtb = [&](uint32_t w, float bias) { return exb ? cvt(w) + bias : cvt(w); };
   const uint32_t rowb = (uint32_t)(a.Sp * 4);
   const __amdgpu_buffer_rsrc_t ors = __builtin_amdgcn_make_buffer_rsrc(
       (BETA ? a.ws.beta : a.ws.alpha) + (int64_t)b * a.T * a.Sp, 0, (int)(rowb * (uint32_t)a.T),
@@ -916,8 +950,8 @@
       Xv eB[PPL], eL[PPL];
 #pragma unroll
       for (int j = 0; j < PPL; ++j) {
-        eB[j] = xemit(cvt(w[s][j][0]), q, liveB[j]);
-        eL[j] = xemit(cvt(w[s][j][1]), q, liveL[j]);
+        eB[j] = xemit(cvtb(w[s][j][0], bB), q, liveB[j]);
+        eL[j] = xemit(cvtb(w[s][j][1], bL[j]), q, liveL[j]);
       }
       if (i == 0) {
 #pragma unroll
@@ -1048,19 +1082,101 @@
   __builtin_amdgcn_fence(__ATOMIC_ACQUIRE, "wavefront");
 }
 
+#ifndef SC_CTC_GROWS
+#define SC_CTC_GROWS 1
+#endif
+constexpr int kGradRows = SC_CTC_GROWS;
+constexpr int kGradXC = 2;
+constexpr int kGradSP = 4;
+
+template <int DT>
+struct GradPre {
+  typedef uint32_t raw_t __attribute__((ext_vector_type(4)));
+  static constexpr int NR = Vec16<DT>::N == 8 ? 1 : 2;
+  int64_t in_len, tgt_len;
+  float sc, cst, lse;
+  double lse64, ll2s;
+  int sharp;
+  float al[kGradSP], be[kGradSP], exv[kGradSP], exvb[kGradSP];
+  int tgv[kGradSP], firstv[kGradSP], chainv[kGradSP];
+  float ex0, ex0b;
+  raw_t x[kGradXC][NR];
+  bool xvec;
+};
+
 template <int DT, int GT>
-__global__ void __launch_bounds__(256) ctc_grad_kernel(CtcArgs a) {
+__device__ __forceinline__ void grad_preload(const CtcArgs& a, int64_t row, int lane, GradPre<DT>& p) {
   using E = Elem<DT>;
   using G = Elem<GT>;
-  extern __shared__ __attribute__((aligned(16))) float lcab_all[];
-  const int lane = threadIdx.x & 63, w = threadIdx.x >> 6;
-  const int64_t row = (int64_t)blockIdx.x * (blockDim.x >> 6) + w;
-  if (row >= (int64_t)a.B * a.T) return;
-  float* lcab = lcab_all + w * (a.V + 4);
   const int b = (int)(row / a.T), t = (int)(row % a.T);
-  const int Tb = clampi(a.in_lens[b], 0, a.T);
+  p.in_len = a.in_lens[b];
+  p.tgt_len = a.tgt_lens[b];
+  p.sc = a.scale[b];
+  p.sharp = a.ws.sharp[b];
+  p.ll2s = a.ws.ll2s[b];
+  p.cst = a.ws.cst[row];
+  p.lse = a.is_logits ? a.ws.lse[row] : 0.0f;
+  p.lse64 = a.is_logits ? a.ws.lse64[row] : 0.0;
+  const float* exr = a.ex ? a.ex + (int64_t)b * a.exb + (int64_t)t * a.ext : nullptr;
+  const float* eb = (exr && a.exbias) ? a.exbias + (int64_t)b * (a.Umax + 1) : nullptr;
+#pragma unroll
+  for (int k = 0; k < kGradSP; ++k) {
+    const int s = lane + 64 * k;
+    const bool in = s < a.Sp;
+    p.al[k] = in ? a.ws.alpha[row * a.Sp + s] : kNegInf;
+    p.be[k] = in ? a.ws.beta[row * a.Sp + s] : kNegInf;
+    const int u = (s - 1) >> 1;
+    const bool lab = (s & 1) && u < a.Umax;
+    p.tgv[k] = lab ? ((const int*)(a.tg + (int64_t)b * a.tgs))[2 * u] : 0;
+    p.firstv[k] = lab ? a.ws.first[(int64_t)b * a.Umax + u] : 0;
+    p.chainv[k] = lab ? a.ws.chain[(int64_t)b * a.Umax + u] : -1;
+    p.exv[k] = (lab && exr) ? exr[1 + u] : 0.0f;
+    p.exvb[k] = (lab && eb) ? eb[1 + u] : 0.0f;
+  }
+  p.ex0 = exr ? exr[0] : 0.0f;
+  p.ex0b = eb ? eb[0] : 0.0f;
+  const typename G::T* g = (const typename G::T*)a.grad + row * a.V;
+  const typename E::T* xr = (const typename E::T*)a.x + (int64_t)b * a.sb + (int64_t)t * a.stt;
+  p.xvec = (a.V & 7) == 0 && ((uintptr_t)g & 15) == 0 && ((uintptr_t)xr & 15) == 0;
+#pragma unroll
+  for (int j = 0; j < kGradXC; ++j) {
+    const int c = lane + 64 * j;
+#pragma unroll
+    for (int r = 0; r < GradPre<DT>::NR; ++r) {
+      p.x[j][r] = typename GradPre<DT>::raw_t{0u, 0u, 0u, 0u};
+      if (p.xvec && c < (a.V >> 3))
+        p.x[j][r] = *(const typename GradPre<DT>::raw_t*)(xr + 8 * c + r * Vec16<DT>::N);
+    }
+  }
+}
+
+template <int DT>
+__device__ __forceinline__ void grad_x8(const typename GradPre<DT>::raw_t (&r)[GradPre<DT>::NR],
+                                        float (&f)[8]) {
+  if constexpr (Vec16<DT>::N == 4) {
+#pragma unroll
+    for (int i = 0; i < 4; ++i) {
+      f[i] = __uint_as_float(r[0][i]);
+      f[4 + i] = __uint_as_float(r[1][i]);
+    }
+  } else {
+#pragma unroll
+    for (int i = 0; i < 4; ++i) {
+      f[2 * i] = Elem<DT>::ldw(r[0][i] & 0xffffu);
+      f[2 * i + 1] = Elem<DT>::ldw(r[0][i] >> 16);
+    }
+  }
+}
+
+template <int DT, int GT>
+__device__ __forceinline__ void grad_row(const CtcArgs& a, int64_t row, int lane, float* lcab,
+                                         const GradPre<DT>& p) {
+  using E = Elem<DT>;
+  using G = Elem<GT>;
+  const int b = (int)(row / a.T), t = (int)(row % a.T);
+  const int Tb = clampi(p.in_len, 0, a.T);
   typename G::T* g = (typename G::T*)a.grad + row * a.V;
-  const float sc = a.scale[b];
+  const float sc = p.sc;
   const bool gvec = (a.V & 7) == 0 && ((uintptr_t)g & 15) == 0;
   if (t >= Tb || sc == 0.0f) {
     if (gvec) {
@@ -1078,46 +1194,56 @@
     }
     return;
   }
-  const int Ub = clampi(a.tgt_lens[b], 0, a.Umax);
+  const int Ub = clampi(p.tgt_len, 0, a.Umax);
   const int Sb = 2 * Ub + 1;
   const int Um = a.Umax > 0 ? a.Umax : 1;
   const int64_t* tg = a.tg + (int64_t)b * a.tgs;
+  wave_lds_sync();
   for (int v = lane; v < a.V; v += 64) lcab[v] = kNegInf;
   wave_lds_sync();
   const float* exr = a.ex ? a.ex + (int64_t)b * a.exb + (int64_t)t * a.ext : nullptr;
   const float* al = a.ws.alpha + ((int64_t)b * a.T + t) * a.Sp;
   const float* be = a.ws.beta + ((int64_t)b * a.T + t) * a.Sp;
-  const int per = a.ws.sharp[b] == 2 ? 1 : 2 * a.kh;
+  const int per = p.sharp == 2 ? 1 : 2 * a.kh;
   const float koff = (float)(a.ws.offA[(int64_t)b * (a.T + 1) + (t + 1) / per] +
                              a.ws.offB[(int64_t)b * (a.T + 1) + (Tb - t) / per] +
-                             (double)a.ws.cst[(int64_t)b * a.T + t] - a.ws.ll2s[b]);
+                             (double)p.cst - p.ll2s);
   const int* chain = a.ws.chain + (int64_t)b * Um;
   const int* first = a.ws.first + (int64_t)b * Um;
-  const float lse = a.is_logits ? a.ws.lse[(int64_t)b * a.T + t] : 0.0f;
-  const float lse_lo = a.is_logits ? (float)(a.ws.lse64[(int64_t)b * a.T + t] - (double)lse) : 0.0f;
+  const float lse = p.lse;
+  const float lse_lo = a.is_logits ? (float)(p.lse64 - (double)lse) : 0.0f;
   auto exact_grad = [&](float logit, float occ2) {
     const float lp2 = ((logit - lse) - lse_lo) * kLog2e;
     return (exp2_(lp2) - exp2_(occ2 + koff - lp2)) * sc;
   };
   float m = kNegInf, l = 0.0f;
-  for (int s = lane; s < Sb; s += 64) {
-    const int lab = (s & 1) ? (int)tg[(s - 1) >> 1] : a.blank;
-    const float val = al[s] + be[s];
+  auto state = [&](int s, int tgl, float val, int isfirst, int q0, float exl) __attribute__((always_inline)) {
+    const int lab = (s & 1) ? tgl : a.blank;
     if (lab == a.blank) {
       const float mn = fmaxf(m, val);
       if (mn != kNegInf) {
         l = l * exp2_(m - mn) + exp2_(val - mn);
         m = mn;
       }
-    } else {
-      const int u = (s - 1) >> 1;
-      if (first[u]) {
-        float acc = val;
-        for (int q = chain[u]; q >= 0; q = chain[q])
-          acc = lse2_b2(acc, al[2 * q + 1] + be[2 * q + 1]);
-        if (lab >= 0 && lab < a.V) lcab[lab] = exr ? exact_grad(exr[1 + u], acc) : acc;
-      }
-    }
+    } else if (isfirst) {
+      float acc = val;
+      for (int q = q0; q >= 0; q = chain[q])
+        acc = lse2_b2(acc, al[2 * q + 1] + be[2 * q + 1]);
+      if (lab >= 0 && lab < a.V) lcab[lab] = exr ? exact_grad(exl, acc) : acc;
+    }
+  };
+#pragma unroll
+  for (int k = 0; k < kGradSP; ++k) {
+    const int s = lane + 64 * k;
+    if (s < Sb)
+      state(s, p.tgv[k], p.al[k] + p.be[k], p.firstv[k], p.chainv[k],
+            a.exbias ? p.exv[k] + p.exvb[k] : p.exv[k]);
+  }
+  for (int s = lane + 64 * kGradSP; s < Sb; s += 64) {
+    const int u = (s - 1) >> 1;
+    const bool odd = s & 1;
+    state(s, odd ? (int)tg[u] : 0, al[s] + be[s], odd ? first[u] : 0, odd ? chain[u] : -1,
+          (odd && exr) ? ex_ld(a, exr, b, 1 + u) : 0.0f);
   }
   {
     const float M = wave_max_dpp(m);
@@ -1126,26 +1252,20 @@
   }
   if (lane == 0 && a.blank >= 0 && a.blank < a.V) {
     const float ob = (m == kNegInf) ? kNegInf : m + log2_(l);
-    lcab[a.blank] = exr ? exact_grad(exr[0], ob) : ob;
+    lcab[a.blank] = exr ? exact_grad(a.exbias ? p.ex0 + p.ex0b : p.ex0, ob) : ob;
   }
   wave_lds_sync();
   const typename E::T* xr = (const typename E::T*)a.x + (int64_t)b * a.sb + (int64_t)t * a.stt;
-  if (gvec && ((uintptr_t)xr & 15) == 0) {
-    for (int c = lane; c < (a.V >> 3); c += 64) {
-      float xv[8], gv[8];
-      if constexpr (Vec16<DT>::N == 8) {
-        Vec16<DT>::ld(xr + 8 * c, xv);
-      } else {
-        Vec16<DT>::ld(xr + 8 * c, *(float(*)[4])&xv[0]);
-        Vec16<DT>::ld(xr + 8 * c + 4, *(float(*)[4])&xv[4]);
-      }
+  if (p.xvec) {
+    auto chunk = [&](int c, const float (&xv)[8], auto has_ex) __attribute__((always_inline)) {
+      float gv[8];
       const float4 l0 = *(const float4*)&lcab[8 * c], l1 = *(const float4*)&lcab[8 * c + 4];
       const float lc[8] = {l0.x, l0.y, l0.z, l0.w, l1.x, l1.y, l1.z, l1.w};
 #pragma unroll
       for (int k = 0; k < 8; ++k) {
         const float lp2 = ((xv[k] - lse) - lse_lo) * kLog2e;
-        gv[k] = (exp2_(lp2) - exp2_(lc[k] + koff - lp2)) * sc;
-        if (a.ex && lc[k] != kNegInf) gv[k] = lc[k];
+        if constexpr (decltype(has_ex)::value) gv[k] = lc[k] != kNegInf ? lc[k] : exp2_(lp2) * sc;
+        else gv[k] = (exp2_(lp2) - exp2_(lc[k] + koff - lp2)) * sc;
       }
       if constexpr (Vec16<GT>::N == 8) {
         Vec16<GT>::st(g + 8 * c, gv);
@@ -1153,7 +1273,30 @@
         Vec16<GT>::st(g + 8 * c, *(float(*)[4])&gv[0]);
         Vec16<GT>::st(g + 8 * c + 4, *(float(*)[4])&gv[4]);
       }
-    }
+    };
+    auto pass = [&](auto has_ex) __attribute__((always_inline)) {
+#pragma unroll
+      for (int j = 0; j < kGradXC; ++j) {
+        const int c = lane + 64 * j;
+        if (c < (a.V >> 3)) {
+          float xv[8];
+          grad_x8<DT>(p.x[j], xv);
+          chunk(c, xv, has_ex);
+        }
+      }
+      for (int c = lane + 64 * kGradXC; c < (a.V >> 3); c += 64) {
+        float xv[8];
+        if constexpr (Vec16<DT>::N == 8) {
+          Vec16<DT>::ld(xr + 8 * c, xv);
+        } else {
+          Vec16<DT>::ld(xr + 8 * c, *(float(*)[4])&xv[0]);
+          Vec16<DT>::ld(xr + 8 * c + 4, *(float(*)[4])&xv[4]);
+        }
+        chunk(c, xv, has_ex);
+      }
+    };
+    if (a.ex) pass(std::true_type{});
+    else pass(std::false_type{});
     return;
   }
   for (int v = lane; v < a.V; v += 64) {
@@ -1161,6 +1304,27 @@
     const float lc = lcab[v];
     const float gv = (a.ex && lc != kNegInf) ? lc : (exp2_(lp2) - exp2_(lc + koff - lp2)) * sc;
     g[v] = G::st(gv);
+  }
+}
+
+template <int DT, int GT>
+__global__ void __launch_bounds__(256) ctc_grad_kernel(CtcArgs a) {
+  extern __shared__ __attribute__((aligned(16))) float lcab_all[];
+  const int lane = threadIdx.x & 63, w = uniform(threadIdx.x >> 6);
+  const int64_t rows = (int64_t)a.B * a.T;
+  const int64_t row0 = ((int64_t)blockIdx.x * (blockDim.x >> 6) + w) * kGradRows;
+  if (row0 >= rows) return;
+  float* lcab = lcab_all + w * (a.V + 4);
+  GradPre<DT> cur, nxt;
+  grad_preload<DT, GT>(a, row0, lane, cur);
+#pragma unroll
+  for (int i = 0; i < kGradRows; ++i) {
+    const int64_t row = row0 + i;
+    if (row >= rows) break;
+    const bool more = i + 1 < kGradRows && row + 1 < rows;
+    if (more) grad_preload<DT, GT>(a, row + 1, lane, nxt);
+    grad_row<DT, GT>(a, row, lane, lcab, cur);
+    if (more) cur = nxt;
   }
 }
 
@@ -1208,7 +1372,8 @@
 template <int DT, int GT>
 static void launch_bwd(const CtcArgs& a, hipStream_t st) {
   const int R = 4 * (a.V + 4) * (int)sizeof(float) <= 65536 ? 4 : 1;
-  hipLaunchKernelGGL((ctc_grad_kernel<DT, GT>), dim3((unsigned)(((int64_t)a.B * a.T + R - 1) / R)),
+  const int64_t per = (int64_t)R * kGradRows;
+  hipLaunchKernelGGL((ctc_grad_kernel<DT, GT>), dim3((unsigned)(((int64_t)a.B * a.T + per - 1) / per)),
                      dim3(64 * R), R * (a.V + 4) * sizeof(float), st, a);
 }
 
@@ -1332,6 +1497,7 @@
   a.grad = grad;
   a.ex = nullptr;
   a.exb = a.ext = 0;
+  a.exbias = nullptr;
   return a;
 }
 
@@ -1344,12 +1510,12 @@
   return 0;
 }
 
-extern "C" int sc_ctc_fwd_ex(const void* x, int x_dtype, int is_logits, int B, int T, int V,
-                             int64_t stride_b, int64_t stride_t, const int64_t* targets,
-                             int64_t target_stride, int max_target_len, const int64_t* in_lens,
-                             const int64_t* tgt_lens, int blank, const float* ex,
-                             int64_t ex_stride_b, int64_t ex_stride_t, float* nll, void* workspace,
-                             size_t workspace_bytes, void* stream) {
+extern "C" int sc_ctc_fwd_exb(const void* x, int x_dtype, int is_logits, int B, int T, int V,
+                              int64_t stride_b, int64_t stride_t, const int64_t* targets,
+                              int64_t target_stride, int max_target_len, const int64_t* in_lens,
+                              const int64_t* tgt_lens, int blank, const float* ex,
+                              int64_t ex_stride_b, int64_t ex_stride_t, const float* ex_bias,
+                              float* nll, void* workspace, size_t workspace_bytes, void* stream) {
   clear_error();
   int rc = ctc_check(x, x_dtype, B, T, V, max_target_len, targets, in_lens, tgt_lens, blank,
                      workspace, workspace_bytes, "sc_ctc_fwd");
@@ -1361,9 +1527,11 @@
     return rc;
   CtcArgs a = make_args(x, is_logits, B, T, V, stride_b, stride_t, targets, target_stride,
                         max_target_len, in_lens, tgt_lens, blank, nll, workspace, nullptr, nullptr);
+  SC_REQUIRE(!ex_bias || ex, "sc_ctc_fwd_exb: ex_bias without ex");
   a.ex = ex;
   a.exb = ex_stride_b;
   a.ext = ex_stride_t;
+  a.exbias = ex_bias;
   hipStream_t st = (hipStream_t)stream;
   switch (x_dtype) {
     case SC_F32: launch_fwd<SC_F32>(a, st); break;
@@ -1371,6 +1539,17 @@
     default: launch_fwd<SC_F16>(a, st); break;
   }
   return launch_status("sc_ctc_fwd");
+}
+
+extern "C" int sc_ctc_fwd_ex(const void* x, int x_dtype, int is_logits, int B, int T, int V,
+                             int64_t stride_b, int64_t stride_t, const int64_t* targets,
+                             int64_t target_stride, int max_target_len, const int64_t* in_lens,
+                             const int64_t* tgt_lens, int blank, const float* ex,
+                             int64_t ex_stride_b, int64_t ex_stride_t, float* nll, void* workspace,
+                             size_t workspace_bytes, void* stream) {
+  return sc_ctc_fwd_exb(x, x_dtype, is_logits, B, T, V, stride_b, stride_t, targets, target_stride,
+                        max_target_len, in_lens, tgt_lens, blank, ex, ex_stride_b, ex_stride_t,
+                        nullptr, nll, workspace, workspace_bytes, stream);
 }
 
 extern "C" int sc_ctc_fwd(const void* x, int x_dtype, int is_logits, int B, int T, int V,
@@ -1383,13 +1562,13 @@
                        workspace_bytes, stream);
 }
 
-extern "C" int sc_ctc_bwd_ex(const void* x, int x_dtype, int is_logits, int B, int T, int V,
-                             int64_t stride_b, int64_t stride_t, const int64_t* targets,
-                             int64_t target_stride, int max_target_len, const int64_t* in_lens,
-                             const int64_t* tgt_lens, int blank, const float* ex,
-                             int64_t ex_stride_b, int64_t ex_stride_t, const float* nll,
-                             const float* scale, void* grad, int grad_dtype, const void* workspace,
-                             size_t workspace_bytes, void* stream) {
+extern "C" int sc_ctc_bwd_exb(const void* x, int x_dtype, int is_logits, int B, int T, int V,
+                              int64_t stride_b, int64_t stride_t, const int64_t* targets,
+                              int64_t target_stride, int max_target_len, const int64_t* in_lens,
+                              const int64_t* tgt_lens, int blank, const float* ex,
+                              int64_t ex_stride_b, int64_t ex_stride_t, const float* ex_bias,
+                              const float* nll, const float* scale, void* grad, int grad_dtype,
+                              const void* workspace, size_t workspace_bytes, void* stream) {
   clear_error();
   int rc = ctc_check(x, x_dtype, B, T, V, max_target_len, targets, in_lens, tgt_lens, blank,
                      workspace, workspace_bytes, "sc_ctc_bwd");
@@ -1403,9 +1582,11 @@
   CtcArgs a = make_args(x, is_logits, B, T, V, stride_b, stride_t, targets, target_stride,
                         max_target_len, in_lens, tgt_lens, blank, (float*)nll, workspace, scale,
                         grad);
+  SC_REQUIRE(!ex_bias || ex, "sc_ctc_bwd_exb: ex_bias without ex");
   a.ex = ex;
   a.exb = ex_stride_b;
   a.ext = ex_stride_t;
+  a.exbias = ex_bias;
   hipStream_t st = (hipStream_t)stream;
 #define SC_CTC_BWD(DT)                                               \
   switch (grad_dtype) {                                              \
@@ -1420,6 +1601,18 @@
   }
 #undef SC_CTC_BWD
   return launch_status("sc_ctc_bwd");
+}
+
+extern "C" int sc_ctc_bwd_ex(const void* x, int x_dtype, int is_logits, int B, int T, int V,
+                             int64_t stride_b, int64_t stride_t, const int64_t* targets,
+                             int64_t target_stride, int max_target_len, const int64_t* in_lens,
+                             const int64_t* tgt_lens, int blank, const float* ex,
+                             int64_t ex_stride_b, int64_t ex_stride_t, const float* nll,
+                             const float* scale, void* grad, int grad_dtype, const void* workspace,
+                             size_t workspace_bytes, void* stream) {
+  return sc_ctc_bwd_exb(x, x_dtype, is_logits, B, T, V, stride_b, stride_t, targets, target_stride,
+                        max_target_len, in_lens, tgt_lens, blank, ex, ex_stride_b, ex_stride_t,
+                        nullptr, nll, scale, grad, grad_dtype, workspace, workspace_bytes, stream);
 }
 
 extern "C" int sc_ctc_bwd(const void* x, int x_dtype, int is_logits, int B, int T, int V,
diff --git a/statecatcher_amd/csrc/tn_gemm.hip b/statecatcher_amd/csrc/tn_gemm.hip
--- a/statecatcher_amd/csrc/tn_gemm.hip
+++ b/statecatcher_amd/csrc/tn_gemm.hip
@@ -44,6 +44,12 @@
 
 __device__ __forceinline__ i4v lds_read16(uint32_t byte) {
   return *(const __attribute__((address_space(3))) i4v*)(size_t)byte;
+}
+
+__device__ __forceinline__ void wave_fence_lds() {
+  __builtin_amdgcn_fence(__ATOMIC_RELEASE, "wavefront", "local");
+  __builtin_amdgcn_wave_barrier();
+  __builtin_amdgcn_fence(__ATOMIC_ACQUIRE, "wavefront", "local");
 }
 
 template <int MF, int SPI>
@@ -1236,6 +1242,169 @@
 }
 #endif
 
+constexpr int kSkWBuf = 32 * 1024;
+constexpr int kSkStage = 8 * 1024;
+constexpr int kSkLds = 2 * kSkWBuf + 8 * kSkStage;
+constexpr int kSkStores = 8;
+
+template <int N>
+__device__ __forceinline__ void sk_wait_case(int n) {
+  if (n == N) dma_wait_younger<N>();
+}
+
+template <int NKS>
+__global__ void __launch_bounds__(512, 1) tnsk_kernel(TnArgs a) {
+  constexpr int NKT = NKS / 2;
+  constexpr int PPW = 2 * NKT;
+  extern __shared__ __attribute__((aligned(16))) unsigned char lds[];
+  const int lane = threadIdx.x & 63;
+  const int w = uniform(threadIdx.x >> 6);
+  const int l15 = lane & 15, l4 = lane >> 4;
+
+  const int G = gridDim.x, bid = blockIdx.x;
+  const int xcd = bid % 8, qq = G / 8, rr = G % 8;
+  const int lid = (xcd < rr ? xcd * (qq + 1) : rr * (qq + 1) + (xcd - rr) * qq) + bid / 8;
+  const int nct = a.N / 128;
+  const int64_t units = (int64_t)((a.M + 255) / 256) * nct;
+  const int u0 = (int)(units * lid / G), u1 = (int)(units * (lid + 1) / G);
+  const int n = u1 - u0;
+  if (n <= 0) return;
+  const uint32_t lds0 = lds_addr(lds);
+  const uint32_t stg = lds0 + 2u * kSkWBuf + (uint32_t)w * kSkStage;
+
+  auto dma_w = [&](int j) __attribute__((always_inline)) {
+    const int n0 = ((u0 + j) % nct) * 128;
+    const uint32_t dst = lds0 + (uint32_t)((j & 1) * kSkWBuf);
+#pragma unroll
+    for (int q = 0; q < PPW; ++q) {
+      const int g = PPW * w + q, kt = g / 16;
+      const int r = 8 * (g % 16) + (lane >> 3);
+      const uint32_t col = (uint32_t)kt * kBK + 8u * (uint32_t)((lane & 7) ^ swz(r));
+      dma_to_lds_s<16>(a.B, ((uint32_t)(n0 + r) * a.ldb + col) * 2u,
+                       dst + (uint32_t)(kt * 16 * 1024 + (g % 16) * 1024));
+    }
+  };
+  struct XFrag { i4v v[2][NKS]; };
+  auto load_x = [&](int rb, XFrag& f) __attribute__((always_inline)) {
+#pragma unroll
+    for (int mf = 0; mf < 2; ++mf) {
+      const uint32_t row = (uint32_t)min(rb * 256 + 32 * w + 16 * mf + l15, a.M - 1);
+      const __bf16* p = a.A + (size_t)row * a.lda + 8 * l4;
+#pragma unroll
+      for (int kk = 0; kk < NKS; ++kk) f.v[mf][kk] = *(const i4v*)(p + 32 * kk);
+    }
+  };
+  uint32_t offW[2][4];
+#pragma unroll
+  for (int h = 0; h < 2; ++h)
+#pragma unroll
+    for (int nf = 0; nf < 4; ++nf) {
+      const int r = 64 * h + (l15 >> 2) * 16 + nf * 4 + (l15 & 3);
+      offW[h][nf] = (uint32_t)(r * kRowB + 16 * (l4 ^ swz(r)));
+    }
+  const __amdgpu_buffer_rsrc_t crs = __builtin_amdgcn_make_buffer_rsrc(a.C, 0, a.cbytes, 0x00020000);
+  auto wait_landed = [&](int younger) __attribute__((always_inline)) {
+    sk_wait_case<0>(younger);
+    sk_wait_case<kSkStores>(younger);
+    sk_wait_case<2 * kSkStores>(younger);
+    sk_wait_case<PPW>(younger);
+    sk_wait_case<PPW + kSkStores>(younger);
+    sk_wait_case<PPW + 2 * kSkStores>(younger);
+  };
+
+  XFrag xf, xn;
+  int rb = (u0 / nct);
+  dma_w(0);
+  if (n > 1) dma_w(1);
+  load_x(rb, xf);
+  xn = xf;
+  for (int j = 0; j < n; ++j) {
+    const int u = u0 + j;
+    const int n0 = (u % nct) * 128;
+    wait_landed((j >= 2 ? kSkStores : 0) + (j >= 1 ? kSkStores : 0) + (j + 1 < n ? PPW : 0));
+    lds_barrier();
+    const bool turn = j + 1 < n && (u + 1) / nct != rb;
+    if (turn) load_x(rb + 1, xn);
+    const uint32_t wb = lds0 + (uint32_t)((j & 1) * kSkWBuf);
+    f4v acc[2][2][4];
+#pragma unroll
+    for (int mf = 0; mf < 2; ++mf)
+#pragma unroll
+      for (int h = 0; h < 2; ++h)
+#pragma unroll
+        for (int nf = 0; nf < 4; ++nf) acc[mf][h][nf] = f4v{0.f, 0.f, 0.f, 0.f};
+#pragma unroll
+    for (int kk = 0; kk < NKS; ++kk) {
+      i4v wf[2][4];
+#pragma unroll
+      for (int h = 0; h < 2; ++h)
+#pragma unroll
+        for (int nf = 0; nf < 4; ++nf)
+          wf[h][nf] = lds_read16(wb + (uint32_t)((kk >> 1) * 16 * 1024) + (offW[h][nf] ^ (64u * (kk & 1))));
+#pragma unroll
+      for (int mf = 0; mf < 2; ++mf)
+#pragma unroll
+        for (int h = 0; h < 2; ++h)
+#pragma unroll
+          for (int nf = 0; nf < 4; ++nf)
+            acc[mf][h][nf] = __builtin_amdgcn_mfma_f32_16x16x32_bf16(
+                __builtin_bit_cast(b8v, wf[h][nf]), __builtin_bit_cast(b8v, xf.v[mf][kk]),
+                acc[mf][h][nf], 0, 0, 0);
+    }
+    lds_read_wait();
+    lds_barrier();
+    if (j + 2 < n) dma_w(j + 2);
+#pragma unroll
+    for (int mf = 0; mf < 2; ++mf)
+#pragma unroll
+      for (int h = 0; h < 2; ++h)
+#pragma unroll
+        for (int s2 = 0; s2 < 2; ++s2) {
+          i4v v;
+#pragma unroll
+          for (int d = 0; d < 4; ++d) {
+            const int nf = 2 * s2 + (d >> 1), jj = 2 * (d & 1);
+            const b2v pk = {(__bf16)acc[mf][h][nf][jj], (__bf16)acc[mf][h][nf][jj + 1]};
+            v[d] = __builtin_bit_cast(int, pk);
+          }
+          const int chunk = 8 * h + 2 * l4 + s2;
+          *(__attribute__((address_space(3))) i4v*)(size_t)(stg + (uint32_t)(mf * 4096 + l15 * 256 +
+                                                                             16 * (chunk ^ l15))) = v;
+        }
+    wave_fence_lds();
+#pragma unroll
+    for (int i = 0; i < kSkStores; ++i) {
+      const int rl = 4 * i + l4;
+      const i4v v = lds_read16(stg + (uint32_t)(rl * 256 + 16 * (l15 ^ (rl & 15))));
+      const uint32_t row = (uint32_t)(rb * 256 + 32 * w + rl);
+      __builtin_amdgcn_raw_buffer_store_b128(v, crs, (row * a.ldc + (uint32_t)(n0 + 8 * l15)) * 2u, 0, 0);
+    }
+    if (turn) {
+      xf = xn;
+      ++rb;
+    }
+  }
+}
+
+int launch_tnsk(const TnArgs& a, hipStream_t st) {
+  const int64_t units = (int64_t)((a.M + 255) / 256) * (a.N / 128);
+  const int grid = units < 256 ? (int)units : 256;
+  if (a.K == 64) {
+    static const bool ok = hipFuncSetAttribute((const void*)tnsk_kernel<2>,
+                                               hipFuncAttributeMaxDynamicSharedMemorySize,
+                                               kSkLds) == hipSuccess;
+    (void)ok;
+    hipLaunchKernelGGL(tnsk_kernel<2>, dim3(grid), dim3(512), kSkLds, st, a);
+  } else {
+    static const bool ok = hipFuncSetAttribute((const void*)tnsk_kernel<4>,
+                                               hipFuncAttributeMaxDynamicSharedMemorySize,
+                                               kSkLds) == hipSuccess;
+    (void)ok;
+    hipLaunchKernelGGL(tnsk_kernel<4>, dim3(grid), dim3(512), kSkLds, st, a);
+  }
+  return 0;
+}
+
 int launch_tn256(const TnArgs& a, hipStream_t st) {
   constexpr size_t lds = 2 * 4 * (size_t)kHalfB;
   static const bool ok = hipFuncSetAttribute((const void*)tn256_kernel,
@@ -1284,9 +1453,10 @@
   SC_REQUIRE(K % kBK == 0, "sc_gemm_tn_bf16: K=%d must be a multiple of 64 (zero-pad it)", K);
   SC_REQUIRE(N % kTN == 0, "sc_gemm_tn_bf16: N=%d must be a multiple of 256", N);
   SC_REQUIRE(tile_m == 0 || (SC_TNW_AB && tile_m >= 1 && tile_m <= 3) || tile_m == 128 ||
-                 tile_m == 192 || tile_m == 256 || tile_m == 257,
-             "sc_gemm_tn_bf16: tile_m=%d must be 0 (default 192), 128, 192, 256 or 257 (256, "
-             "ping-pong schedule); 1 / 2 / 3 (one wave per SIMD) in SC_TNW_AB builds only",
+                 tile_m == 192 || tile_m == 256 || tile_m == 257 || tile_m == 258,
+             "sc_gemm_tn_bf16: tile_m=%d must be 0 (default 192), 128, 192, 256, 257 (256, "
+             "ping-pong schedule) or 258 (256, the four-phase kernel at every K: A/B of the "
+             "small-K kernel); 1 / 2 / 3 (one wave per SIMD) in SC_TNW_AB builds only",
              tile_m);
   SC_REQUIRE(lda >= K && ldb >= K && ldc >= N && lda % 8 == 0 && ldb % 8 == 0 && ldc % 8 == 0,
              "sc_gemm_tn_bf16: leading dimensions must cover the rows in 16-byte pieces");
@@ -1295,7 +1465,8 @@
   SC_REQUIRE((int64_t)M * lda * 2 < (1ll << 32) && (int64_t)N * ldb * 2 < (1ll << 32) &&
                  ((int64_t)M + 256) * ldc * 2 < (1ll << 32),
              "sc_gemm_tn_bf16: operands must be smaller than 4 GiB");
-  const int tm = (tile_m == 257 || (tile_m >= 1 && tile_m <= 3)) ? 256 : tile_m ? tile_m : 192;
+  const int tm = (tile_m == 257 || tile_m == 258 || (tile_m >= 1 && tile_m <= 3)) ? 256
+                 : tile_m ? tile_m : 192;
   const int ntn = N / kTN;
   const int64_t tiles = (int64_t)((M + tm - 1) / tm) * ntn;
   SC_REQUIRE(tiles < (1 << 30), "sc_gemm_tn_bf16: too many tiles");
@@ -1324,6 +1495,10 @@
 #endif
   if (tile_m == 257) {
     launch_tnpp(a, st);
+    return launch_status("sc_gemm_tn_bf16");
+  }
+  if (tile_m == 256 && K <= 128) {
+    launch_tnsk(a, st);
     return launch_status("sc_gemm_tn_bf16");
   }
   if (tm == 256) {
diff --git a/statecatcher_amd/ops.py b/statecatcher_amd/ops.py
--- a/statecatcher_amd/ops.py
+++ b/statecatcher_amd/ops.py
@@ -726,7 +726,7 @@
 class CTCFn(torch.autograd.Function):
 
     @staticmethod
-    def forward(ctx, x, targets, in_lens, tgt_lens, blank, is_logits, ex=None):
+    def forward(ctx, x, targets, in_lens, tgt_lens, blank, is_logits, ex=None, ex_bias=None):
         require_device(x, targets, in_lens, tgt_lens)
         if x.dim() != 3:
             raise ValueError(f"x must be [B,T,V], got {tuple(x.shape)}")
@@ -747,19 +747,28 @@
             if (ex.dtype != torch.float32 or ex.shape != (B, T, umax + 1) or ex.stride(2) != 1):
                 raise ValueError(f"ex must be fp32 [B, T, U_max + 1] = {(B, T, umax + 1)} with unit "
                                  f"column stride; got {ex.dtype} {tuple(ex.shape)}")
+        if ex_bias is not None:
+            if ex is None:
+                raise ValueError("ex_bias needs ex")
+            require_device(x, ex_bias)
+            if ex_bias.dtype != torch.float32 or ex_bias.shape != (B, umax + 1):
+                raise ValueError(f"ex_bias must be fp32 [B, U_max + 1] = {(B, umax + 1)}; got "
+                                 f"{ex_bias.dtype} {tuple(ex_bias.shape)}")
+            ex_bias = ex_bias.contiguous()
         if T == 0:
             nll = torch.where(tgt_lens == 0, 0.0, float("inf")).to(torch.float32)
         else:
-            rc = lib.sc_ctc_fwd_ex(ptr(x), dtype_code(x), int(is_logits), B, T, V, x.stride(0),
-                                   x.stride(1), ptr(targets), targets.stride(0) if umax else 0, umax,
-                                   ptr(in_lens), ptr(tgt_lens), blank, ptr(ex),
-                                   ex.stride(0) if ex is not None else 0,
-                                   ex.stride(1) if ex is not None else 0, ptr(nll), ptr(ws), wsb,
-                                   stream_of(x))
-            check(rc, "sc_ctc_fwd_ex")
+            rc = lib.sc_ctc_fwd_exb(ptr(x), dtype_code(x), int(is_logits), B, T, V, x.stride(0),
+                                    x.stride(1), ptr(targets), targets.stride(0) if umax else 0, umax,
+                                    ptr(in_lens), ptr(tgt_lens), blank, ptr(ex),
+                                    ex.stride(0) if ex is not None else 0,
+                                    ex.stride(1) if ex is not None else 0, ptr(ex_bias), ptr(nll),
+                                    ptr(ws), wsb, stream_of(x))
+            check(rc, "sc_ctc_fwd_exb")
         ctx.save_for_backward(x, targets, in_lens, tgt_lens, nll, ws)
         ctx.meta = (blank, int(is_logits), umax, wsb)
         ctx.ex = ex
+        ctx.ex_bias = ex_bias
         return nll
 
     @staticmethod
@@ -767,13 +776,14 @@
         blank, is_logits, umax, wsb = ctx.meta
         B, T, V = x.shape
         ex = ctx.ex
-        rc = _lib.load().sc_ctc_bwd_ex(ptr(x), dtype_code(x), is_logits, B, T, V, x.stride(0),
-                                       x.stride(1), ptr(targets), targets.stride(0) if umax else 0,
-                                       umax, ptr(in_lens), ptr(tgt_lens), blank, ptr(ex),
-                                       ex.stride(0) if ex is not None else 0,
-                                       ex.stride(1) if ex is not None else 0, ptr(nll), ptr(scale),
-                                       ptr(grad), dtype_code(grad), ptr(ws), wsb, stream_of(x))
-        check(rc, "sc_ctc_bwd_ex")
+        rc = _lib.load().sc_ctc_bwd_exb(ptr(x), dtype_code(x), is_logits, B, T, V, x.stride(0),
+                                        x.stride(1), ptr(targets), targets.stride(0) if umax else 0,
+                                        umax, ptr(in_lens), ptr(tgt_lens), blank, ptr(ex),
+                                        ex.stride(0) if ex is not None else 0,
+                                        ex.stride(1) if ex is not None else 0, ptr(ctx.ex_bias),
+                                        ptr(nll), ptr(scale), ptr(grad), dtype_code(grad), ptr(ws),
+                                        wsb, stream_of(x))
+        check(rc, "sc_ctc_bwd_exb")
 
     @staticmethod
     def backward(ctx, grad_nll):
@@ -784,14 +794,14 @@
         if T > 0:
             scale = grad_nll.to(torch.float32).contiguous()
             CTCFn._bwd(ctx, x, targets, in_lens, tgt_lens, nll, ws, scale, grad)
-        return grad, None, None, None, None, None, None
+        return grad, None, None, None, None, None, None, None
 
 
 class CTCMeanFn(torch.autograd.Function):
 
     @staticmethod
-    def forward(ctx, x, targets, in_lens, tgt_lens, blank, is_logits, ex=None):
-        nll = CTCFn.forward(ctx, x, targets, in_lens, tgt_lens, blank, is_logits, ex)
+    def forward(ctx, x, targets, in_lens, tgt_lens, blank, is_logits, ex=None, ex_bias=None):
+        nll = CTCFn.forward(ctx, x, targets, in_lens, tgt_lens, blank, is_logits, ex, ex_bias)
         B = nll.shape[0]
         loss = torch.empty((), dtype=torch.float32, device=x.device)
         factor = torch.empty(B, dtype=torch.float32, device=x.device)
@@ -820,7 +830,7 @@
     raise ValueError(f"SC_HEAD_SPLIT={HEAD_SPLIT!r}: expected 'emis', 'labels' or 'full'")
 
 
-def _emission_logits(wide, w, b, targets, blank, V):
+def _emission_logits_split(wide, w, b, targets, blank, V):
     B, T, K3 = wide.shape
     K = K3 // 3
     U1 = targets.shape[1] + 1
@@ -832,7 +842,11 @@
                                        ptr(tgc), tgc.stride(0) if U1 > 1 else 0, U1 - 1, blank,
                                        ptr(wg), ptr(bg), B, stream_of(wide))
     check(rc, "sc_ctc_split_rows")
-    ex = torch.bmm(wide, wg.transpose(1, 2), out_dtype=torch.float32)
+    return torch.bmm(wide, wg.transpose(1, 2), out_dtype=torch.float32), bg
+
+
+def _emission_logits(wide, w, b, targets, blank, V):
+    ex, bg = _emission_logits_split(wide, w, b, targets, blank, V)
     ex += bg.unsqueeze(1)
     return ex
 
@@ -872,17 +886,17 @@
         B, T, K = x.shape
         V = w.shape[0]
         x2 = x.reshape(-1, K)
-        ex = None
+        ex = bg = None
         if wide is not None and HEAD_SPLIT == "full":
             logits = _logits_fp32(wide.view(-1, 3 * K), split_weight_image(w), b).view(B, T, V)
         elif wide is not None and HEAD_SPLIT == "emis":
             logits = torch.addmm(b.to(torch.bfloat16), x2, wc.t()).view(B, T, V)
-            ex = _emission_logits(wide.view(B, T, 3 * K), w, b, targets, blank, V)
+            ex, bg = _emission_logits_split(wide.view(B, T, 3 * K), w, b, targets, blank, V)
         else:
             logits = _logits_fp32(x2, wc, b).view(B, T, V)
             if wide is not None:
                 _exact_emission_columns(logits, wide, w, b, targets, blank)
-        loss = CTCMeanFn.forward(ctx, logits, targets, in_lens, tgt_lens, blank, True, ex)
+        loss = CTCMeanFn.forward(ctx, logits, targets, in_lens, tgt_lens, blank, True, ex, bg)
         ctx.head = (x2, wt, x.shape, x.dtype)
         return loss, logits
 
```
